# TorchIO-project/torchio

Hardware: NVIDIA H100
Metric: augmented voxels/sec on 256^3 fp32 Compose pipeline (higher is better)
Workload: dtype f32

## Files before the change

### include/tio_b200.h

```cpp
#ifndef TIO_B200_H
#define TIO_B200_H

#include <stddef.h>
#include <stdint.h>

#ifdef __cplusplus
extern "C" {
#endif

#define TIO_ABI_VERSION 2

enum tio_dtype {
  TIO_F32 = 0,
  TIO_U8 = 1,
  TIO_I8 = 2,
  TIO_I16 = 3,
  TIO_I32 = 4,
  TIO_I64 = 5,
  TIO_F16 = 6,
  TIO_BF16 = 7,
  TIO_F64 = 8
};

enum tio_interp { TIO_NEAREST = 0, TIO_LINEAR = 1, TIO_LABEL_PV = 2 };
#define TIO_EXACT_COORDS 0x100

#define TIO_FLAG_PASSTHROUGH 1u
#define TIO_FLAG_ELASTIC 2u

const char* tio_last_error(void);
int tio_abi_version(void);

size_t tio_resample_workspace_bytes(int B, int OI, int OJ, int OK);
int tio_resample(const void* src, void* dst, int dtype,
                 int B, int C, int I, int J, int K,
                 int OI, int OJ, int OK,
                 const float* mat, const float* cp, const uint8_t* flags,
                 int ni, int nj, int nk,
                 const float* spacing_in, const float* spacing_out,
                 int affine_first, int mode, const float* fill, int box_hint,
                 void* workspace, size_t workspace_bytes, void* stream);

int tio_onehot(const void* src, int dtype, int B, int64_t vox, const void* labels, int n,
               float* dst, void* stream);
int tio_label_argmax(const float* sampled, int B, int n, int64_t vox, const void* labels,
                     float pad_label, void* dst, int dtype, void* stream);

int tio_crop_patches(const void* src, void* dst, int elem_bytes, int C, int I, int J, int K,
                     int n, const int32_t* corners, int pi, int pj, int pk, void* stream);

int tio_remap(const void* src, void* dst, int elem_bytes, int B, int C, int I, int J, int K,
              int OI, int OJ, int OK, int off_i, int off_j, int off_k, int mode,
              const void* fill, const uint8_t* flip, void* stream);

int tio_permute(const void* src, void* dst, int elem_bytes, int B, int C, int I, int J, int K,
                int perm0, int perm1, int perm2, int flip_bits, void* stream);

int tio_upload(const void* host_pinned, void* dst_device, size_t bytes, void* stream);

int tio_min_sample0(const float* src, int C, int64_t n, float* fill, void* stream);

int tio_blur(const float* src, float* dst, float* scratch,
             int B, int C, int I, int J, int K,
             const float* taps, const int32_t* radius, int R, int axes_mask,
             const uint8_t* identity, void* stream);

size_t tio_mt19937_table_bytes(void);
int tio_mt19937_build_table(void* host_blob, size_t bytes);
size_t tio_randn_mt19937_workspace_bytes(uint64_t offset, uint64_t n);
int tio_randn_mt19937(uint64_t seed, uint64_t offset, uint64_t n, float* z,
                      const void* table, void* workspace, size_t workspace_bytes,
                      void* stream);

int tio_moments(const float* src, const uint8_t* mask, int64_t n, double* out3, void* stream);
size_t tio_quantiles_workspace_bytes(void);
int tio_quantiles(const float* src, const uint8_t* mask, int64_t n, const double* q_host, int m,
                  float* values, double* weights, double* count, void* workspace,
                  size_t workspace_bytes, void* stream);
int tio_rescale(const float* src, float* dst, int B, int64_t per_elem, float lo, float hi,
                const float* sub, const float* div, const float* mul, const float* add,
                const uint8_t* keep, int flags, void* stream);

size_t tio_quantiles_batched_workspace_bytes(int B, int m);
int tio_quantiles_batched(const void* src, int dtype, const uint8_t* mask, int B, int64_t per_elem,
                          const double* q_host, int m, float* values, double* weights, double* count,
                          uint8_t* has_nan, void* workspace, size_t workspace_bytes, void* stream);
int tio_histogram_tables(const float* values, const double* weights, const uint8_t* has_nan,
                         const float* landmarks, int B, int m, float* tables, void* stream);
int tio_histogram_map(const void* src, void* dst, int dtype, int B, int64_t per_elem,
                      const float* tables, int m, void* stream);

int tio_intensity_fused(const float* src, float* dst, float* scratch,
                        int B, int C, int I, int J, int K,
                        const float* coarse, int si, int sj, int sk,
                        const uint8_t* bias_identity, int bias_divide,
                        const float* taps, const int32_t* radius, int R, int axes_mask,
                        const float* mean, const float* std, const uint8_t* keep,
                        const float* z, const float* z2,
                        uint64_t philox_seed, int noise_mode, int rician,
                        const float* gamma, void* stream);

int tio_labels_to_image(const void* labels, int dtype, int C, int B, int64_t vox,
                        const int64_t* label_values, int n, const float* mean, const float* std,
                        const uint64_t* draw_offset, uint64_t seed, int grid_x, float* dst,
                        void* stream);

int tio_label_lut(const void* src, void* dst, int dtype, int64_t count, const void* keys,
                  const void* values, int n, int identity, void* stream);
int tio_label_contour(const void* src, int dtype, int volumes, int I, int J, int K, float* dst,
                      void* stream);
int tio_onehot_classes(const void* src, int dtype, int B, int C, int64_t vox, int num_classes,
                       float* dst, void* stream);
int tio_label_range(const void* src, int dtype, int B, int C, int64_t vox, int64_t* range,
                    void* stream);
int tio_channel_argmax(const void* src, int dtype, int B, int C, int64_t vox, float* dst,
                       void* stream);

int tio_interpolate(const void* src, void* dst, int dtype, int volumes, int I, int J, int K, int OI,
                    int OJ, int OK, const int32_t* idx, const float* lam, int linear, void* stream);
int tio_axis_resample(const void* src, void* dst, int dtype, int B, int C, int I, int J, int K,
                      const int32_t* axis, const int32_t* lo, const int32_t* hi, const float* w, int L,
                      int linear, void* stream);

int tio_clamp(const void* src, void* dst, int dtype, int dst_dtype, int64_t count, const void* lo,
              const void* hi, void* stream);
int tio_mask(const void* mask, int mask_dtype, int mask_channels, const void* keys, int n_keys,
             const void* src, int dtype, void* dst, int dst_dtype, int B, int C, int64_t vox,
             const void* outside, void* stream);
int tio_swap_patches(void* data, int elem_size, int B, int C, int I, int J, int K, int pi, int pj,
                     int pk, const int32_t* swaps, int lists, int steps, int32_t* swaps_device,
                     void* stage, void* stream);

int tio_components(const void* src, int dtype, int B, int I, int J, int K, int mode, const void* keys,
                   int n_keys, int64_t background, int has_background, int fully_connected,
                   uint32_t* parent, uint32_t* count, uint32_t* flags, void* stream);
int tio_component_roots(const void* src, int dtype, int B, int64_t vox, const uint32_t* parent,
                        void* values, uint32_t* n_values, void* stream);
int tio_keep_largest(void* data, int dtype, int B, int64_t vox, int mode, const void* keys,
                     int n_keys, int64_t background, int has_background, const uint32_t* parent,
                     const uint32_t* count, uint64_t* winner, const void* fill, void* stream);

size_t tio_spike_stats_workspace_bytes(int rows);
int tio_spike_stats(const void* src, int dtype, int B, int C, int64_t vox, const float* intensity,
                    double* sum, uint32_t* flags, void* workspace, size_t workspace_bytes,
                    void* stream);
int tio_spectrum_peak(const void* src, int dtype, int B, int C, int I, int J, int K,
                      const float* intensity, const uint32_t* flags, float* peak, void* workspace,
                      size_t workspace_bytes, void* stream);
int tio_spike(void* data, int dtype, int B, int C, int I, int J, int K, const int32_t* spikes, int S,
              const float* intensity, const double* sum, const uint32_t* flags, const float* peak,
              void* tables, size_t tables_bytes, void* stream);

int tio_ghosting(void* data, int dtype, int B, int C, int I, int J, int K, const float* table, int n_max,
                 const int32_t* axis, const uint8_t* active, int axes, uint32_t* flags, void* stream);

#ifdef __cplusplus
}
#endif
#endif
```

### torchio_b200/_native.py

```python

from __future__ import annotations

import ctypes
from ctypes import c_char_p, c_float, c_int, c_int64, c_size_t, c_uint64, c_void_p
from pathlib import Path

LIB_PATH = Path(__file__).resolve().parent / "csrc" / "libtio_b200.so"

_SIGNATURES = {
    "tio_abi_version": [],
    "tio_resample": [c_void_p, c_void_p, c_int] + [c_int] * 8
    + [c_void_p, c_void_p, c_void_p] + [c_int] * 3
    + [c_void_p, c_void_p, c_int, c_int, c_void_p, c_int, c_void_p, c_size_t, c_void_p],
    "tio_resample_workspace_bytes": [c_int, c_int, c_int, c_int],
    "tio_min_sample0": [c_void_p, c_int, c_int64, c_void_p, c_void_p],
    "tio_upload": [c_void_p, c_void_p, c_size_t, c_void_p],
    "tio_remap": [c_void_p, c_void_p, c_int] + [c_int] * 8 + [c_int] * 3 + [c_int, c_void_p, c_void_p, c_void_p],
    "tio_crop_patches": [c_void_p, c_void_p, c_int] + [c_int] * 5 + [c_void_p, c_int, c_int, c_int, c_void_p],
    "tio_blur": [c_void_p, c_void_p, c_void_p] + [c_int] * 5
    + [c_void_p, c_void_p, c_int, c_int, c_void_p, c_void_p],
    "tio_moments": [c_void_p, c_void_p, c_int64, c_void_p, c_void_p],
    "tio_quantiles_workspace_bytes": [],
    "tio_quantiles": [c_void_p, c_void_p, c_int64, c_void_p, c_int, c_void_p, c_void_p, c_void_p, c_void_p,
                      c_size_t, c_void_p],
    "tio_quantiles_batched_workspace_bytes": [c_int, c_int],
    "tio_quantiles_batched": [c_void_p, c_int, c_void_p, c_int, c_int64, c_void_p, c_int, c_void_p, c_void_p,
                              c_void_p, c_void_p, c_void_p, c_size_t, c_void_p],
    "tio_histogram_tables": [c_void_p, c_void_p, c_void_p, c_void_p, c_int, c_int, c_void_p, c_void_p],
    "tio_histogram_map": [c_void_p, c_void_p, c_int, c_int, c_int64, c_void_p, c_int, c_void_p],
    "tio_rescale": [c_void_p, c_void_p, c_int, c_int64, c_float, c_float, c_void_p, c_void_p, c_void_p, c_void_p,
                    c_void_p, c_int, c_void_p],
    "tio_onehot": [c_void_p, c_int, c_int, c_int64, c_void_p, c_int, c_void_p, c_void_p],
    "tio_label_argmax": [c_void_p, c_int, c_int, c_int64, c_void_p, c_float, c_void_p, c_int, c_void_p],
    "tio_mt19937_table_bytes": [],
    "tio_mt19937_build_table": [c_void_p, c_size_t],
    "tio_randn_mt19937_workspace_bytes": [c_uint64, c_uint64],
    "tio_randn_mt19937": [c_uint64, c_uint64, c_uint64, c_void_p, c_void_p, c_void_p, c_size_t,
                          c_void_p],
    "tio_intensity_fused": [c_void_p, c_void_p, c_void_p] + [c_int] * 5
    + [c_void_p, c_int, c_int, c_int, c_void_p, c_int]
    + [c_void_p, c_void_p, c_int, c_int]
    + [c_void_p] * 5 + [c_uint64, c_int, c_int, c_void_p, c_void_p],
    "tio_labels_to_image": [c_void_p, c_int, c_int, c_int, c_int64, c_void_p, c_int, c_void_p, c_void_p, c_void_p,
                            c_uint64, c_int, c_void_p, c_void_p],
    "tio_label_lut": [c_void_p, c_void_p, c_int, c_int64, c_void_p, c_void_p, c_int, c_int, c_void_p],
    "tio_label_contour": [c_void_p, c_int, c_int, c_int, c_int, c_int, c_void_p, c_void_p],
    "tio_onehot_classes": [c_void_p, c_int, c_int, c_int, c_int64, c_int, c_void_p, c_void_p],
    "tio_label_range": [c_void_p, c_int, c_int, c_int, c_int64, c_void_p, c_void_p],
    "tio_channel_argmax": [c_void_p, c_int, c_int, c_int, c_int64, c_void_p, c_void_p],
    "tio_interpolate": [c_void_p, c_void_p, c_int, c_int, c_int, c_int, c_int, c_int, c_int, c_int, c_void_p,
                        c_void_p, c_int, c_void_p],
    "tio_axis_resample": [c_void_p, c_void_p, c_int, c_int, c_int, c_int, c_int, c_int, c_void_p, c_void_p,
                          c_void_p, c_void_p, c_int, c_int, c_void_p],
    "tio_clamp": [c_void_p, c_void_p, c_int, c_int, c_int64, c_void_p, c_void_p, c_void_p],
    "tio_mask": [c_void_p, c_int, c_int, c_void_p, c_int, c_void_p, c_int, c_void_p, c_int, c_int, c_int, c_int64,
                 c_void_p, c_void_p],
    "tio_swap_patches": [c_void_p] + [c_int] * 9 + [c_void_p, c_int, c_int, c_void_p, c_void_p, c_void_p],
    "tio_components": [c_void_p] + [c_int] * 6 + [c_void_p, c_int, c_int64, c_int, c_int] + [c_void_p] * 4,
    "tio_component_roots": [c_void_p, c_int, c_int, c_int64] + [c_void_p] * 4,
    "tio_keep_largest": [c_void_p, c_int, c_int, c_int64, c_int, c_void_p, c_int, c_int64, c_int] + [c_void_p] * 5,
    "tio_permute": [c_void_p, c_void_p] + [c_int] * 10 + [c_void_p],
    "tio_spike_stats_workspace_bytes": [c_int],
    "tio_spike_stats": [c_void_p, c_int, c_int, c_int, c_int64] + [c_void_p] * 4 + [c_size_t, c_void_p],
    "tio_spectrum_peak": [c_void_p] + [c_int] * 6 + [c_void_p] * 4 + [c_size_t, c_void_p],
    "tio_spike": [c_void_p] + [c_int] * 6 + [c_void_p, c_int] + [c_void_p] * 5 + [c_size_t, c_void_p],
    "tio_ghosting": [c_void_p] + [c_int] * 6 + [c_void_p, c_int, c_void_p, c_void_p, c_int, c_void_p, c_void_p],
}

_lib = None


def lib() -> ctypes.CDLL:
    global _lib
    if _lib is None:
        if not LIB_PATH.exists():
            raise RuntimeError(
                f"torchio_b200: CUDA library not built ({LIB_PATH} is missing)."
                " Run `python -c 'import __graft_entry__ as g; g.build()'` at the"
                " repo root (needs nvcc). There is no CPU fallback."
            )
        handle = ctypes.CDLL(str(LIB_PATH))
        handle.tio_last_error.restype = c_char_p
        handle.tio_last_error.argtypes = []
        for name, argtypes in _SIGNATURES.items():
            fn = getattr(handle, name)
            fn.argtypes = argtypes
            fn.restype = c_size_t if name.endswith("_bytes") else c_int
        _lib = handle
    return _lib


def exported_symbols() -> list[str]:
    return ["tio_last_error", *_SIGNATURES]


def call(name: str, *args) -> None:
    handle = lib()
    rc = getattr(handle, name)(*args)
    if rc != 0:
        msg = handle.tio_last_error().decode(errors="replace")
        raise RuntimeError(f"{name} failed (code {rc}): {msg}")
```

### torchio_b200/csrc/build.py

```python

from __future__ import annotations

import os
import subprocess
import sys
from concurrent.futures import ThreadPoolExecutor
from pathlib import Path

HERE = Path(__file__).resolve().parent
ROOT = HERE.parent.parent
SOURCES = ["error.cu", "resample.cu", "resample_tile.cu", "resample_fast.cu", "upload.cu", "fused_intensity.cu",
           "mt19937_jump.cpp", "mt19937.cu", "patches.cu", "stats.cu", "labels.cu", "labels_to_image.cu",
           "label_maps.cu", "interpolate.cu", "clamp_mask_swap.cu", "components.cu", "permute.cu", "spike.cu",
           "ghosting.cu"]
HEADERS = [HERE / "common.cuh", HERE / "resample_common.cuh", HERE / "resample_tile.cuh", HERE / "tma.cuh",
           HERE / "mt19937_layout.h", HERE / "label_lookup.cuh", HERE / "image_dtype.cuh",
           HERE / "fft_lines.cuh",
           ROOT / "include" / "tio_b200.h",
           Path(__file__).resolve()]
OBJ = HERE / "_obj"
OUT = HERE / "libtio_b200.so"

ARCH = ["-gencode", "arch=compute_90a,code=sm_90a"]
NVCC_FLAGS = [
    *ARCH,
    "-O3", "-std=c++17", "-lineinfo",
    "-Xcompiler", "-fPIC",
    "-Xptxas", "-v",
]


def needs_build() -> bool:
    if not OUT.exists():
        return True
    newest = max(p.stat().st_mtime for p in [*(HERE / s for s in SOURCES), *HEADERS])
    return OUT.stat().st_mtime < newest


def _compile(source: str) -> tuple[str, int, str]:
    src = HERE / source
    obj = OBJ / (Path(source).stem + ".o")
    newest = max(p.stat().st_mtime for p in [src, *HEADERS])
    if obj.exists() and obj.stat().st_mtime >= newest:
        return source, 0, ""
    proc = subprocess.run(["nvcc", *NVCC_FLAGS, "-c", str(src), "-o", str(obj)],
                          capture_output=True, text=True)
    return source, proc.returncode, proc.stdout + proc.stderr


def build(force: bool = False, verbose: bool = False) -> Path:
    if not force and not needs_build():
        return OUT
    OBJ.mkdir(exist_ok=True)
    if force:
        for stale in OBJ.glob("*.o"):
            stale.unlink()
    with ThreadPoolExecutor(max_workers=min(len(SOURCES), os.cpu_count() or 1)) as pool:
        results = list(pool.map(_compile, SOURCES))
    log = "".join(f"==== {name}\n{text}" for name, _, text in results)
    failed = [name for name, code, _ in results if code != 0]
    if verbose or failed:
        sys.stderr.write(log)
    if failed:
        raise RuntimeError(f"nvcc failed for {failed}")
    objects = [str(OBJ / (Path(s).stem + ".o")) for s in SOURCES]
    proc = subprocess.run(["nvcc", *ARCH, "-shared", "-o", str(OUT),
                           *objects], capture_output=True, text=True)
    if proc.returncode != 0:
        sys.stderr.write(proc.stdout + proc.stderr)
        raise RuntimeError(f"nvcc link failed with exit code {proc.returncode}")
    previous = (HERE / "ptxas.log").read_text() if (HERE / "ptxas.log").exists() and not force else ""
    (HERE / "ptxas.log").write_text(log if all(t for _, _, t in results) else previous + log)
    return OUT


if __name__ == "__main__":
    path = build(force="--force" in sys.argv, verbose="--verbose" in sys.argv)
    print(path)
```

### torchio_b200/csrc/fused_intensity.cu

```cuda
#include "common.cuh"
#include "tma.cuh"

namespace tio {

__device__ __forceinline__ float rician(float x, float n1, float n2) {
  float s = __fadd_rn(x, n1);
  return sqrtf(__fadd_rn(__fmul_rn(s, s), __fmul_rn(n2, n2)));
}


__device__ __forceinline__ uint4 philox4x32_10(uint4 ctr, uint2 key) {
  const uint32_t M0 = 0xD2511F53u, M1 = 0xCD9E8D57u, W0 = 0x9E3779B9u, W1 = 0xBB67AE85u;
#pragma unroll
  for (int r = 0; r < 7; ++r) {
    uint32_t hi0 = __umulhi(M0, ctr.x), lo0 = M0 * ctr.x;
    uint32_t hi1 = __umulhi(M1, ctr.z), lo1 = M1 * ctr.z;
    ctr = make_uint4(hi1 ^ ctr.y ^ key.x, lo1, hi0 ^ ctr.w ^ key.y, lo0);
    key.x += W0;
    key.y += W1;
  }
  return ctr;
}

__device__ __forceinline__ void box_muller(uint32_t a, uint32_t b, float& n0, float& n1) {
  float u1 = ((float)(a >> 8) + 0.5f) * (1.0f / 16777216.0f);
  float u2 = ((float)(b >> 8)) * (1.0f / 16777216.0f);
  float rad;
  asm("sqrt.approx.ftz.f32 %0, %1;" : "=f"(rad) : "f"(-2.0f * __logf(u1)));
  float s, c;
  __sincosf(6.283185307179586f * u2, &s, &c);
  n0 = rad * c;
  n1 = rad * s;
}


__device__ __forceinline__ float abs_pow(float ax, float g) {
  float l, p;
  asm("lg2.approx.f32 %0, %1;" : "=f"(l) : "f"(ax));
  asm("ex2.approx.f32 %0, %1;" : "=f"(p) : "f"(__fmul_rn(g, l)));
  return p;
}

__device__ __forceinline__ float signed_pow(float x, float gam) {
  if (gam == 1.0f) return x;
  float ax = fabsf(x);
  float p = abs_pow(ax, gam);
  p = ax == 0.0f ? 0.0f : p;
  return x < 0.0f ? -p : p;
}

constexpr int A_TJ = 32;
constexpr int A_TK = 64;
constexpr int A_PLANES = 16;

struct BiasArgs {
  const float* coarse;
  const uint8_t* identity;
  int si, sj, sk;
  float sc_i, sc_j, sc_k;
  int divide;
};

struct BlurArgs {
  const float* taps;
  const int32_t* radius;
  int R;
};

struct NoiseArgs {
  const float* mean;
  const float* std;
  const uint8_t* keep;
  const float* z;
  const float* z2;
  uint64_t philox_seed;
  int mode;
  int rician;
};

template <int RMAX, bool HAS_EPI>
__global__ void __launch_bounds__(256)
jk_kernel(const float* __restrict__ src, float* __restrict__ dst, int B, int C, int I, int J,
          int K, BlurArgs bl, NoiseArgs nz, const float* __restrict__ gamma) {
  constexpr int ROWS = A_TJ + 2 * RMAX;
  constexpr int COLS = A_TK + 2 * RMAX;
  constexpr int PITCH = (COLS + 3) / 4 * 4 + 4;
  extern __shared__ __align__(16) float smem[];
  float* A = smem;
  float* Bm = A + ROWS * PITCH;
  float* tapk = Bm + ROWS * A_TK;
  float* tapj = tapk + (2 * RMAX + 1);

  const int tiles_i = (I + A_PLANES - 1) / A_PLANES;
  const int bc = blockIdx.z / tiles_i;
  const int i_begin = (blockIdx.z % tiles_i) * A_PLANES;
  const int i_end = min(i_begin + A_PLANES, I);
  const int b = bc / C;
  const int j0 = blockIdx.y * A_TJ, k0 = blockIdx.x * A_TK;
  const int tid = threadIdx.x;
  const int64_t n = (int64_t)I * J * K;
  const float* x = src + (int64_t)bc * n;
  float* y = dst + (int64_t)bc * n;

  const int R = bl.taps ? bl.R : 0;
  const int rj = bl.taps ? bl.radius[1 * B + b] : 0;
  const int rk = bl.taps ? bl.radius[2 * B + b] : 0;
  const bool noise_on = HAS_EPI && nz.mode != 0 && (!nz.keep || nz.keep[b]);
  const float mu = (HAS_EPI && nz.mode) ? nz.mean[b] : 0.0f, sd = (HAS_EPI && nz.mode) ? nz.std[b] : 0.0f;
  const float gam = (HAS_EPI && gamma) ? gamma[b] : 1.0f;

  if (tid < 2 * (2 * RMAX + 1)) {
    const bool is_k = tid < (2 * RMAX + 1);
    const int sft = is_k ? tid : tid - (2 * RMAX + 1);
    const int rr = is_k ? rk : rj;
    float v = 0.0f;
    if (bl.taps && rr > 0 && sft <= 2 * rr)
      v = bl.taps[((int64_t)(is_k ? 2 : 1) * B + b) * (2 * R + 1) + R - rr + sft];
    (is_k ? tapk : tapj)[sft] = v;
  }
  __syncthreads();

  float tk[2 * RMAX + 1], tj[2 * RMAX + 1];
#pragma unroll
  for (int t = 0; t < 2 * RMAX + 1; ++t) { tk[t] = tapk[t]; tj[t] = tapj[t]; }

  const int rows = A_TJ + 2 * rj, cols = A_TK + 2 * rk;
  const int lx = tid & 31, ly = tid >> 5;

  for (int i = i_begin; i < i_end; ++i) {
    const float* xp = x + (int64_t)i * J * K;
    for (int r = ly; r < rows; r += 8) {
      const int jj = min(max(j0 - rj + r, 0), J - 1);
      const float* xr = xp + (int64_t)jj * K;
      for (int c = lx; c < cols; c += 32) {
        const int kk = min(max(k0 - rk + c, 0), K - 1);
        A[r * PITCH + c] = __ldg(xr + kk);
      }
    }
    __syncthreads();
    {
      const int k4 = (tid & 15) * 4;
      for (int r = tid >> 4; r < rows; r += 16) {
        const float* row = A + r * PITCH + k4;
        float acc[4];
        if (rk == 0) {
#pragma unroll
          for (int o = 0; o < 4; ++o) acc[o] = row[o];
        } else {
          float win[4 + 2 * RMAX];
#pragma unroll
          for (int m = 0; m < (4 + 2 * RMAX) / 4; ++m) {
            if (4 * m < 4 + 2 * rk) {
              float4 q = *(const float4*)(row + 4 * m);
              win[4 * m] = q.x; win[4 * m + 1] = q.y; win[4 * m + 2] = q.z; win[4 * m + 3] = q.w;
            } else {
              win[4 * m] = win[4 * m + 1] = win[4 * m + 2] = win[4 * m + 3] = 0.0f;
            }
          }
#pragma unroll
          for (int o = 0; o < 4; ++o) acc[o] = 0.0f;
#pragma unroll
          for (int s = 0; s < 2 * RMAX + 1; ++s) {
            if (s <= 2 * rk) {
#pragma unroll
              for (int o = 0; o < 4; ++o) acc[o] = __fmaf_rn(tk[s], win[o + s], acc[o]);
            }
          }
        }
        *(float4*)(Bm + r * A_TK + k4) = make_float4(acc[0], acc[1], acc[2], acc[3]);
      }
    }
    __syncthreads();
    {
      const int kx = tid & 63, jy = (tid >> 6) * 8;
      const int k = k0 + kx;
      float acc[8];
      if (rj == 0) {
#pragma unroll
        for (int o = 0; o < 8; ++o) acc[o] = Bm[(jy + o) * A_TK + kx];
      } else {
        float win[8 + 2 * RMAX];
#pragma unroll
        for (int w = 0; w < 8 + 2 * RMAX; ++w)
          win[w] = (w < 8 + 2 * rj) ? Bm[(jy + w) * A_TK + kx] : 0.0f;
#pragma unroll
        for (int o = 0; o < 8; ++o) acc[o] = 0.0f;
#pragma unroll
        for (int s = 0; s < 2 * RMAX + 1; ++s) {
          if (s <= 2 * rj) {
#pragma unroll
            for (int o = 0; o < 8; ++o) acc[o] = __fmaf_rn(tj[s], win[o + s], acc[o]);
          }
        }
      }
      if (k < K) {
        const int64_t plane_off = (int64_t)i * J * K + k;
        if (HAS_EPI && noise_on) {
          float z1[8], z2[8];
          if (nz.mode == 1) {
#pragma unroll
            for (int o = 0; o < 8; ++o)
              if (j0 + jy + o < J) {
                const int64_t flat = (int64_t)bc * n + plane_off + (int64_t)(j0 + jy + o) * K;
                z1[o] = __ldcs(nz.z + flat);
                if (nz.rician) z2[o] = __ldcs(nz.z2 + flat);
              }
          } else {
            const uint2 key = make_uint2((uint32_t)nz.philox_seed, (uint32_t)(nz.philox_seed >> 32));
            const uint64_t gidx = (uint64_t)((int64_t)bc * n + plane_off + (int64_t)(j0 + jy) * K);
#pragma unroll
            for (int h = 0; h < 2; ++h) {
              uint4 rr = philox4x32_10(make_uint4((uint32_t)gidx, (uint32_t)(gidx >> 32), (uint32_t)h, 0x6a6bu), key);
              box_muller(rr.x, rr.y, z1[4 * h], z1[4 * h + 1]);
              box_muller(rr.z, rr.w, z1[4 * h + 2], z1[4 * h + 3]);
              if (nz.rician) {
                uint4 r2 = philox4x32_10(make_uint4((uint32_t)gidx, (uint32_t)(gidx >> 32), (uint32_t)(2 + h), 0x6a6bu), key);
                box_muller(r2.x, r2.y, z2[4 * h], z2[4 * h + 1]);
                box_muller(r2.z, r2.w, z2[4 * h + 2], z2[4 * h + 3]);
              }
            }
          }
#pragma unroll
          for (int o = 0; o < 8; ++o) {
            const float n1 = __fadd_rn(mu, __fmul_rn(sd, z1[o]));
            if (nz.rician) acc[o] = rician(acc[o], n1, __fadd_rn(mu, __fmul_rn(sd, z2[o])));
            else acc[o] = __fadd_rn(acc[o], n1);
          }
        }
        if (HAS_EPI && gamma) {
#pragma unroll
          for (int o = 0; o < 8; ++o) acc[o] = signed_pow(acc[o], gam);
        }
        float* yp = y + plane_off;
#pragma unroll
        for (int o = 0; o < 8; ++o)
          if (j0 + jy + o < J) yp[(int64_t)(j0 + jy + o) * K] = acc[o];
      }
    }
    __syncthreads();
  }
}

constexpr int F_R = 6;
constexpr int F_HK = 8;
constexpr int F_ROWS = A_TJ + 2 * F_R;
constexpr int F_COLS = A_TK + 2 * F_HK;
constexpr int F_ABUF = F_ROWS * F_COLS;
constexpr int F_BBUF = F_ROWS * A_TK;
constexpr size_t F_SMEM = (size_t)(2 * F_ABUF + 2 * F_BBUF + 32) * sizeof(float) + 2 * sizeof(uint64_t);

template <int RK>
__device__ __forceinline__ float4 kconv4(const float* __restrict__ row, const int k4, const float* tk) {
  if (RK == 0) return *(const float4*)(row + F_HK + k4);
  constexpr int M0 = RK <= 4 ? 1 : 0, M1 = RK <= 4 ? 4 : 5;
  float win[20];
#pragma unroll
  for (int m = M0; m < M1; ++m) {
    const float4 q = *(const float4*)(row + k4 + 4 * m);
    win[4 * m] = q.x; win[4 * m + 1] = q.y; win[4 * m + 2] = q.z; win[4 * m + 3] = q.w;
  }
  float acc[4] = {0.0f, 0.0f, 0.0f, 0.0f};
#pragma unroll
  for (int t = -RK; t <= RK; ++t)
#pragma unroll
    for (int o = 0; o < 4; ++o) acc[o] = __fmaf_rn(tk[F_R + t], win[F_HK + o + t], acc[o]);
  return make_float4(acc[0], acc[1], acc[2], acc[3]);
}

template <int RJ>
__device__ __forceinline__ void jconv8(const float* __restrict__ Bw, const int jy, const int kx,
                                       const float* tj, float* acc) {
  float win[8 + 2 * RJ];
#pragma unroll
  for (int w = 0; w < 8 + 2 * RJ; ++w) win[w] = Bw[(F_R - RJ + jy + w) * A_TK + kx];
  if (RJ == 0) {
#pragma unroll
    for (int o = 0; o < 8; ++o) acc[o] = win[o];
    return;
  }
#pragma unroll
  for (int o = 0; o < 8; ++o) acc[o] = 0.0f;
#pragma unroll
  for (int t = -RJ; t <= RJ; ++t)
#pragma unroll
    for (int o = 0; o < 8; ++o) acc[o] = __fmaf_rn(tj[F_R + t], win[o + t + RJ], acc[o]);
}

__device__ __forceinline__ float signed_pow_pos(float x, float g) {
  const float p = abs_pow(fabsf(x), g);
  return x < 0.0f ? -p : p;
}

template <bool HAS_EPI>
__global__ void __launch_bounds__(256, 3)
jk6_kernel(const __grid_constant__ CUtensorMap tmap, float* __restrict__ dst, int B, int C, int I,
           int J, int K, BlurArgs bl, NoiseArgs nz, const float* __restrict__ gamma) {
  extern __shared__ __align__(128) float smem[];
  float* Abuf = smem;
  float* Bbuf = smem + 2 * F_ABUF;
  float* taps_s = Bbuf + 2 * F_BBUF;
  uint64_t* bars = reinterpret_cast<uint64_t*>(taps_s + 32);

  const int tiles_i = (I + A_PLANES - 1) / A_PLANES;
  const int bc = blockIdx.z / tiles_i;
  const int i_begin = (blockIdx.z % tiles_i) * A_PLANES;
  const int i_end = min(i_begin + A_PLANES, I);
  const int b = bc / C;
  const int j0 = blockIdx.y * A_TJ, k0 = blockIdx.x * A_TK;
  const int tid = threadIdx.x;
  const int64_t n = (int64_t)I * J * K;

  auto issue = [&](int i, int s) {
    const uint32_t bar = smem_u32(bars + s);
    mbar_expect_tx(bar, (uint32_t)(F_ABUF * sizeof(float)));
    tma_load_3d(smem_u32(Abuf + s * F_ABUF), &tmap, k0 - F_HK, j0 - F_R, bc * I + i, bar);
  };
  if (tid == 0) {
    mbar_init(smem_u32(bars + 0), 1);
    mbar_init(smem_u32(bars + 1), 1);
    mbar_fence_init();
    issue(i_begin, 0);
  }

  const int R = bl.R;
  const int rj = bl.radius[1 * B + b], rk = bl.radius[2 * B + b];
  const bool noise_on = HAS_EPI && nz.mode != 0 && (!nz.keep || nz.keep[b]);
  const float mu = (HAS_EPI && nz.mode) ? nz.mean[b] : 0.0f, sd = (HAS_EPI && nz.mode) ? nz.std[b] : 0.0f;
  const float gam = (HAS_EPI && gamma) ? gamma[b] : 1.0f;
  const int gamma_mode = !(HAS_EPI && gamma) || gam == 1.0f ? 0 : (gam > 0.0f ? 1 : 2);

  if (tid < 2 * (2 * F_R + 1)) {
    const int axis = tid < (2 * F_R + 1) ? 2 : 1;
    const int s = tid < (2 * F_R + 1) ? tid : tid - (2 * F_R + 1);
    const int off = s - F_R, rr = axis == 2 ? rk : rj;
    float v = 0.0f;
    if (rr > 0 && off >= -rr && off <= rr) v = bl.taps[((int64_t)axis * B + b) * (2 * R + 1) + R + off];
    taps_s[(axis == 2 ? 0 : 13) + s] = v;
  }
  __syncthreads();
  float tk[2 * F_R + 1], tj[2 * F_R + 1];
#pragma unroll
  for (int t = 0; t < 2 * F_R + 1; ++t) { tk[t] = taps_s[t]; tj[t] = taps_s[13 + t]; }

  const int row_lo = F_R - rj, row_hi = F_R + A_TJ + rj;
  const int rsrc_lo = max(0, F_R - j0), rsrc_hi = min(F_ROWS - 1, J - 1 - j0 + F_R);
  const int clo = max(0, F_HK - k0), chi = min(F_COLS - 1, K - 1 - k0 + F_HK);
  const bool kfix = (clo > F_HK - rk) || (chi < F_HK + A_TK + rk - 1);

  const int k4 = (tid & 15) * 4;
  const int kx = tid & 63, jy = (tid >> 6) * 8;
  const int k = k0 + kx;
  const int valid = (k < K) ? min(8, J - (j0 + jy)) : 0;
  const int plane_off = (j0 + jy) * K + k;

  auto kpass = [&](int i) {
    const int it = i - i_begin, s = it & 1;
    mbar_wait(smem_u32(bars + s), (uint32_t)((it >> 1) & 1));
    float* A = Abuf + s * F_ABUF;
    float* Bw = Bbuf + s * F_BBUF;
#pragma unroll 1
    for (int r = row_lo + (tid >> 4); r < row_hi; r += 16) {
      float* row = A + min(max(r, rsrc_lo), rsrc_hi) * F_COLS;
      if (kfix) {
        const int c_lo = (F_HK - F_R) + (tid & 15);
        if (c_lo < clo) row[c_lo] = row[clo];
#pragma unroll 1
        for (int c = chi + 1 + (tid & 15); c < F_HK + A_TK + F_R; c += 16) row[c] = row[chi];
        __syncwarp();
      }
      float4 o4;
      switch (rk) {
        case 0: o4 = kconv4<0>(row, k4, tk); break;
        case 1: o4 = kconv4<1>(row, k4, tk); break;
        case 2: o4 = kconv4<2>(row, k4, tk); break;
        case 3: o4 = kconv4<3>(row, k4, tk); break;
        case 4: o4 = kconv4<4>(row, k4, tk); break;
        case 5: o4 = kconv4<5>(row, k4, tk); break;
        default: o4 = kconv4<6>(row, k4, tk); break;
      }
      *(float4*)(Bw + r * A_TK + k4) = o4;
    }
  };

  if (tid == 0 && i_begin + 1 < i_end) issue(i_begin + 1, 1);
  kpass(i_begin);
  __syncthreads();
  for (int i = i_begin; i < i_end; ++i) {
    const int it = i - i_begin, s = it & 1;
    if (tid == 0 && i + 2 < i_end) issue(i + 2, s);
    float* Bw = Bbuf + s * F_BBUF;
    float z1[8], z2[8];
    const int64_t flat0 = (int64_t)bc * n + (int64_t)i * J * K + plane_off;
    if (HAS_EPI && noise_on && nz.mode == 1) {
      const float* zp = nz.z + flat0;
      if (valid == 8) {
#pragma unroll
        for (int o = 0; o < 8; ++o, zp += K) z1[o] = __ldcs(zp);
      } else {
#pragma unroll
        for (int o = 0; o < 8; ++o, zp += K)
          if (o < valid) z1[o] = __ldcs(zp);
      }
      if (nz.rician) {
        const float* zq = nz.z2 + flat0;
#pragma unroll
        for (int o = 0; o < 8; ++o, zq += K)
          if (o < valid) z2[o] = __ldcs(zq);
      }
    }
    if (i + 1 < i_end) kpass(i + 1);
    float acc[8];
    switch (rj) {
      case 0: jconv8<0>(Bw, jy, kx, tj, acc); break;
      case 1: jconv8<1>(Bw, jy, kx, tj, acc); break;
      case 2: jconv8<2>(Bw, jy, kx, tj, acc); break;
      case 3: jconv8<3>(Bw, jy, kx, tj, acc); break;
      case 4: jconv8<4>(Bw, jy, kx, tj, acc); break;
      case 5: jconv8<5>(Bw, jy, kx, tj, acc); break;
      default: jconv8<6>(Bw, jy, kx, tj, acc); break;
    }
    if (valid > 0) {
      if (HAS_EPI && noise_on) {
        if (nz.mode == 2) {
          const uint2 key = make_uint2((uint32_t)nz.philox_seed, (uint32_t)(nz.philox_seed >> 32));
#pragma unroll
          for (int h = 0; h < 2; ++h) {
            const uint64_t gidx = (uint64_t)(flat0 + (int64_t)(4 * h) * K);
            uint4 rr = philox4x32_10(make_uint4((uint32_t)gidx, (uint32_t)(gidx >> 32), 0u, 0x6a6bu), key);
            box_muller(rr.x, rr.y, z1[4 * h], z1[4 * h + 1]);
            box_muller(rr.z, rr.w, z1[4 * h + 2], z1[4 * h + 3]);
            if (nz.rician) {
              uint4 r2 = philox4x32_10(make_uint4((uint32_t)gidx, (uint32_t)(gidx >> 32), 1u, 0x6a6bu), key);
              box_muller(r2.x, r2.y, z2[4 * h], z2[4 * h + 1]);
              box_muller(r2.z, r2.w, z2[4 * h + 2], z2[4 * h + 3]);
            }
          }
        }
        if (nz.rician) {
#pragma unroll
          for (int o = 0; o < 8; ++o)
            acc[o] = rician(acc[o], __fadd_rn(mu, __fmul_rn(sd, z1[o])), __fadd_rn(mu, __fmul_rn(sd, z2[o])));
        } else {
#pragma unroll
          for (int o = 0; o < 8; ++o) acc[o] = __fadd_rn(acc[o], __fadd_rn(mu, __fmul_rn(sd, z1[o])));
        }
      }
      if (gamma_mode == 1) {
#pragma unroll
        for (int o = 0; o < 8; ++o) acc[o] = signed_pow_pos(acc[o], gam);
      } else if (gamma_mode == 2) {
#pragma unroll
        for (int o = 0; o < 8; ++o) acc[o] = signed_pow(acc[o], gam);
      }
      float* yp = dst + flat0;
      if (valid == 8) {
#pragma unroll
        for (int o = 0; o < 8; ++o, yp += K) *yp = acc[o];
      } else {
#pragma unroll
        for (int o = 0; o < 8; ++o, yp += K)
          if (o < valid) *yp = acc[o];
      }
    }
    __syncthreads();
  }
}

template <int V, bool HAS_BIAS>
__global__ void __launch_bounds__(256)
march_kernel(const float* __restrict__ src, float* __restrict__ dst, int B, int C, int I, int J,
             int K, BlurArgs bl, BiasArgs bi, NoiseArgs nz, const float* __restrict__ gamma) {
  extern __shared__ __align__(16) float smem[];
  const int bc = blockIdx.z;
  const int b = bc / C;
  const int tid = threadIdx.y * blockDim.x + threadIdx.x;
  const int k = (blockIdx.x * blockDim.x + threadIdx.x) * V;
  const int j = blockIdx.y * blockDim.y + threadIdx.y;
  const int64_t n = (int64_t)I * J * K;
  const float* x = src + (int64_t)bc * n;
  float* y = dst + (int64_t)bc * n;

  const int r = bl.taps ? bl.radius[0 * B + b] : 0;
  const int R = bl.taps ? bl.R : 0;
  const int W = 2 * r + 1;
  float* tapi = smem;
  float* g = smem + ((2 * R + 1 + 3) / 4) * 4;
  const int ns = HAS_BIAS ? bi.si * bi.sj * bi.sk : 0;
  float* ring = g + ((ns + 3) / 4) * 4;
  const bool bias_on = HAS_BIAS && !(bi.identity && bi.identity[b]);
  if (r > 0)
    for (int t = tid; t < 2 * R + 1; t += 256) tapi[t] = bl.taps[((int64_t)0 * B + b) * (2 * R + 1) + t];
  if (bias_on) {
    const float* gs = bi.coarse + (int64_t)bc * ns;
    for (int t = tid; t < ns; t += 256) g[t] = gs[t];
  }
  __syncthreads();
  if (k >= K || j >= J) return;

  const bool noise_on = nz.mode != 0 && (!nz.keep || nz.keep[b]);
  const float mu = nz.mode ? nz.mean[b] : 0.0f, sd = nz.mode ? nz.std[b] : 0.0f;
  const float gam = gamma ? gamma[b] : 1.0f;

  LerpAxis lj, lk[V];
  int cur0 = -1, cur1 = -1;
  float r_lo[V], r_hi[V];
  if (bias_on) {
    lj = lerp_axis(bi.sc_j, bi.sj, j);
#pragma unroll
    for (int v = 0; v < V; ++v) lk[v] = lerp_axis(bi.sc_k, bi.sk, k + v);
  }

  auto load_plane = [&](int i, float* out) {
    const int64_t o = ((int64_t)i * J + j) * K + k;
    if (V == 4) {
      float4 t = *(const float4*)(x + o);
      out[0] = t.x; out[1] = t.y; out[2] = t.z; out[3] = t.w;
    } else {
      out[0] = x[o];
    }
    if (bias_on) {
      const LerpAxis li = lerp_axis(bi.sc_i, bi.si, i);
      if (li.i0 != cur0 || li.i1 != cur1) {
        const float* p0 = g + (li.i0 * bi.sj) * bi.sk;
        const float* p1 = g + (li.i1 * bi.sj) * bi.sk;
#pragma unroll
        for (int v = 0; v < V; ++v) {
          float a0 = lerp2(lk[v].l0, p0[lj.i0 * bi.sk + lk[v].i0], lk[v].l1, p0[lj.i0 * bi.sk + lk[v].i1]);
          float a1 = lerp2(lk[v].l0, p0[lj.i1 * bi.sk + lk[v].i0], lk[v].l1, p0[lj.i1 * bi.sk + lk[v].i1]);
          r_lo[v] = lerp2(lj.l0, a0, lj.l1, a1);
          float b0 = lerp2(lk[v].l0, p1[lj.i0 * bi.sk + lk[v].i0], lk[v].l1, p1[lj.i0 * bi.sk + lk[v].i1]);
          float b1 = lerp2(lk[v].l0, p1[lj.i1 * bi.sk + lk[v].i0], lk[v].l1, p1[lj.i1 * bi.sk + lk[v].i1]);
          r_hi[v] = lerp2(lj.l0, b0, lj.l1, b1);
        }
        cur0 = li.i0; cur1 = li.i1;
      }
#pragma unroll
      for (int v = 0; v < V; ++v) {
        float f = expf(lerp2(li.l0, r_lo[v], li.l1, r_hi[v]));
        out[v] = bi.divide ? __fdiv_rn(out[v], f) : __fmul_rn(out[v], f);
      }
    }
  };

  auto finish = [&](int i, float* v) {
    const int64_t o = ((int64_t)i * J + j) * K + k;
    if (noise_on) {
      const int64_t flat = (int64_t)bc * n + o;
      float z1[V], z2[V];
      if (nz.mode == 1) {
        if (V == 4) {
          float4 t = __ldcs((const float4*)(nz.z + flat));
          z1[0] = t.x; z1[1] = t.y; z1[2] = t.z; z1[3] = t.w;
          if (nz.rician) {
            float4 u = __ldcs((const float4*)(nz.z2 + flat));
            z2[0] = u.x; z2[1] = u.y; z2[2] = u.z; z2[3] = u.w;
          }
        } else {
          z1[0] = nz.z[flat];
          if (nz.rician) z2[0] = nz.z2[flat];
        }
      } else {
        const uint2 key = make_uint2((uint32_t)nz.philox_seed, (uint32_t)(nz.philox_seed >> 32));
        const uint64_t gidx = (uint64_t)(flat / V);
        uint4 rr = philox4x32_10(make_uint4((uint32_t)gidx, (uint32_t)(gidx >> 32), 0u, 0x5eedu), key);
        float nn[4];
        box_muller(rr.x, rr.y, nn[0], nn[1]);
        box_muller(rr.z, rr.w, nn[2], nn[3]);
#pragma unroll
        for (int q = 0; q < V; ++q) z1[q] = nn[q];
        if (nz.rician) {
          uint4 r2 = philox4x32_10(make_uint4((uint32_t)gidx, (uint32_t)(gidx >> 32), 1u, 0x5eedu), key);
          box_muller(r2.x, r2.y, nn[0], nn[1]);
          box_muller(r2.z, r2.w, nn[2], nn[3]);
#pragma unroll
          for (int q = 0; q < V; ++q) z2[q] = nn[q];
        }
      }
#pragma unroll
      for (int q = 0; q < V; ++q) {
        float n1 = __fadd_rn(mu, __fmul_rn(sd, z1[q]));
        if (nz.rician) v[q] = rician(v[q], n1, __fadd_rn(mu, __fmul_rn(sd, z2[q])));
        else v[q] = __fadd_rn(v[q], n1);
      }
    }
    if (gamma) {
#pragma unroll
      for (int q = 0; q < V; ++q) v[q] = signed_pow(v[q], gam);
    }
    if (V == 4) *(float4*)(y + o) = make_float4(v[0], v[1], v[2], v[3]);
    else y[o] = v[0];
  };

  if (r == 0) {
    for (int i = 0; i < I; ++i) {
      float v[V];
      load_plane(i, v);
      finish(i, v);
    }
    return;
  }

  float* mine = ring + tid * V;
  const int slot_stride = 256 * V;
  auto put = [&](int pos, const float* v) {
    int s = pos % W; if (s < 0) s += W;
    if (V == 4) *(float4*)(mine + s * slot_stride) = make_float4(v[0], v[1], v[2], v[3]);
    else mine[s * slot_stride] = v[0];
  };
  float first[V];
  load_plane(0, first);
  for (int p = -r; p <= 0; ++p) put(p, first);
  float last[V];
#pragma unroll
  for (int q = 0; q < V; ++q) last[q] = first[q];
  for (int p = 1; p < I + r; ++p) {
    if (p < I) load_plane(p, last);
    put(p, last);
    const int o = p - r;
    if (o < 0) continue;
    float acc[V];
#pragma unroll
    for (int q = 0; q < V; ++q) acc[q] = 0.0f;
    int s = (o - r) % W; if (s < 0) s += W;
    for (int t = 0; t < W; ++t) {
      const float tp = tapi[R - r + t];
      if (V == 4) {
        float4 w4 = *(const float4*)(mine + s * slot_stride);
        acc[0] = __fmaf_rn(tp, w4.x, acc[0]); acc[1] = __fmaf_rn(tp, w4.y, acc[1]);
        acc[2] = __fmaf_rn(tp, w4.z, acc[2]); acc[3] = __fmaf_rn(tp, w4.w, acc[3]);
      } else {
        acc[0] = __fmaf_rn(tp, mine[s * slot_stride], acc[0]);
      }
      if (++s == W) s = 0;
    }
    finish(o, acc);
  }
}

constexpr int M6_PF = 8;

template <bool HAS_BIAS, bool EPI>
__global__ void __launch_bounds__(256, EPI ? 1 : 2)
march6_kernel(const float* __restrict__ src, float* __restrict__ dst, int B, int C, int I, int J,
              int K, BlurArgs bl, BiasArgs bi, NoiseArgs nz, const float* __restrict__ gamma) {
  extern __shared__ __align__(16) float smem[];
  constexpr int W = 2 * F_R + 1;
  const int bc = blockIdx.z;
  const int b = bc / C;
  const int tid = threadIdx.y * blockDim.x + threadIdx.x;
  const int k = (blockIdx.x * blockDim.x + threadIdx.x) * 4;
  const int j = blockIdx.y * blockDim.y + threadIdx.y;
  const int64_t n = (int64_t)I * J * K;
  const float* x = src + (int64_t)bc * n;
  float* y = dst + (int64_t)bc * n;

  const int r = bl.taps ? bl.radius[0 * B + b] : 0;
  float* tapi = smem;
  float* g = smem + 16;
  const int ns = HAS_BIAS ? bi.si * bi.sj * bi.sk : 0;
  const bool bias_on = HAS_BIAS && !(bi.identity && bi.identity[b]);
  if (tid < W) {
    const int off = tid - F_R;
    tapi[tid] = (r > 0 && off >= -r && off <= r) ? bl.taps[((int64_t)0 * B + b) * (2 * bl.R + 1) + bl.R + off] : 0.0f;
  }
  if (bias_on) {
    const float* gs = bi.coarse + (int64_t)bc * ns;
    for (int t = tid; t < ns; t += 256) g[t] = gs[t];
  }
  __syncthreads();
  if (k >= K || j >= J) return;

  const bool noise_on = EPI && nz.mode != 0 && (!nz.keep || nz.keep[b]);
  const float mu = (EPI && nz.mode) ? nz.mean[b] : 0.0f, sd = (EPI && nz.mode) ? nz.std[b] : 0.0f;
  const float gam = (EPI && gamma) ? gamma[b] : 1.0f;
  const int gamma_mode = !(EPI && gamma) || gam == 1.0f ? 0 : (gam > 0.0f ? 1 : 2);

  LerpAxis lj, lk[4];
  int o00[4], o01[4], o10[4], o11[4];
  int cur0 = -1, cur1 = -1;
  float r_lo[4], r_hi[4];
  if (bias_on) {
    lj = lerp_axis(bi.sc_j, bi.sj, j);
#pragma unroll
    for (int v = 0; v < 4; ++v) {
      lk[v] = lerp_axis(bi.sc_k, bi.sk, k + v);
      o00[v] = lj.i0 * bi.sk + lk[v].i0; o01[v] = lj.i0 * bi.sk + lk[v].i1;
      o10[v] = lj.i1 * bi.sk + lk[v].i0; o11[v] = lj.i1 * bi.sk + lk[v].i1;
    }
  }
  const int col = j * K + k;
  const int plane = J * K;

  float4* fifo = reinterpret_cast<float4*>(g + ((ns + 3) / 4) * 4) + tid;
  auto fifo_issue = [&](int pl) {
    if (pl < I) {
      const uint32_t sa = (uint32_t)__cvta_generic_to_shared(fifo + (pl & (M6_PF - 1)) * 256);
      asm volatile("cp.async.cg.shared.global [%0], [%1], 16;" ::"r"(sa), "l"(x + (int64_t)pl * plane + col) : "memory");
    }
    asm volatile("cp.async.commit_group;" ::: "memory");
  };
#pragma unroll
  for (int pl = 0; pl < M6_PF - 1; ++pl) fifo_issue(pl);

  auto load_plane = [&](int i, float* out) {
    fifo_issue(i + M6_PF - 1);
    asm volatile("cp.async.wait_group %0;" ::"n"(M6_PF - 1) : "memory");
    const float4 t = fifo[(i & (M6_PF - 1)) * 256];
    out[0] = t.x; out[1] = t.y; out[2] = t.z; out[3] = t.w;
    if (bias_on) {
      const LerpAxis li = lerp_axis(bi.sc_i, bi.si, i);
      if (li.i0 != cur0 || li.i1 != cur1) {
        const float* p0 = g + (li.i0 * bi.sj) * bi.sk;
        const float* p1 = g + (li.i1 * bi.sj) * bi.sk;
#pragma unroll
        for (int v = 0; v < 4; ++v) {
          const float a0 = lerp2(lk[v].l0, p0[o00[v]], lk[v].l1, p0[o01[v]]);
          const float a1 = lerp2(lk[v].l0, p0[o10[v]], lk[v].l1, p0[o11[v]]);
          r_lo[v] = lerp2(lj.l0, a0, lj.l1, a1);
          const float b0 = lerp2(lk[v].l0, p1[o00[v]], lk[v].l1, p1[o01[v]]);
          const float b1 = lerp2(lk[v].l0, p1[o10[v]], lk[v].l1, p1[o11[v]]);
          r_hi[v] = lerp2(lj.l0, b0, lj.l1, b1);
        }
        cur0 = li.i0; cur1 = li.i1;
      }
#pragma unroll
      for (int v = 0; v < 4; ++v) {
        const float f = expf(lerp2(li.l0, r_lo[v], li.l1, r_hi[v]));
        out[v] = bi.divide ? __fdiv_rn(out[v], f) : __fmul_rn(out[v], f);
      }
    }
  };

  auto finish = [&](int i, float* v) {
    const int64_t o = (int64_t)i * plane + col;
    if (EPI) {
      if (noise_on) {
        const int64_t flat = (int64_t)bc * n + o;
        float z1[4], z2[4];
        if (nz.mode == 1) {
          const float4 t = __ldcs((const float4*)(nz.z + flat));
          z1[0] = t.x; z1[1] = t.y; z1[2] = t.z; z1[3] = t.w;
          if (nz.rician) {
            const float4 u = __ldcs((const float4*)(nz.z2 + flat));
            z2[0] = u.x; z2[1] = u.y; z2[2] = u.z; z2[3] = u.w;
          }
        } else {
          const uint2 key = make_uint2((uint32_t)nz.philox_seed, (uint32_t)(nz.philox_seed >> 32));
          const uint64_t gidx = (uint64_t)(flat / 4);
          uint4 rr = philox4x32_10(make_uint4((uint32_t)gidx, (uint32_t)(gidx >> 32), 0u, 0x5eedu), key);
          box_muller(rr.x, rr.y, z1[0], z1[1]);
          box_muller(rr.z, rr.w, z1[2], z1[3]);
          if (nz.rician) {
            uint4 r2 = philox4x32_10(make_uint4((uint32_t)gidx, (uint32_t)(gidx >> 32), 1u, 0x5eedu), key);
            box_muller(r2.x, r2.y, z2[0], z2[1]);
            box_muller(r2.z, r2.w, z2[2], z2[3]);
          }
        }
#pragma unroll
        for (int q = 0; q < 4; ++q) {
          const float n1 = __fadd_rn(mu, __fmul_rn(sd, z1[q]));
          if (nz.rician) v[q] = rician(v[q], n1, __fadd_rn(mu, __fmul_rn(sd, z2[q])));
          else v[q] = __fadd_rn(v[q], n1);
        }
      }
      if (gamma_mode == 1) {
#pragma unroll
        for (int q = 0; q < 4; ++q) v[q] = signed_pow_pos(v[q], gam);
      } else if (gamma_mode == 2) {
#pragma unroll
        for (int q = 0; q < 4; ++q) v[q] = signed_pow(v[q], gam);
      }
    }
    *(float4*)(y + o) = make_float4(v[0], v[1], v[2], v[3]);
  };

  if (r == 0) {
    for (int i = 0; i < I; ++i) {
      float v[4];
      load_plane(i, v);
      finish(i, v);
    }
    return;
  }

  float tp[W];
#pragma unroll
  for (int t = 0; t < W; ++t) tp[t] = tapi[t];
  float ring[W][4];
  {
    float first[4];
    load_plane(0, first);
#pragma unroll
    for (int sl = 0; sl < W; ++sl)
#pragma unroll
      for (int q = 0; q < 4; ++q) ring[sl][q] = first[q];
  }
  for (int base = 0; base < I + F_R; base += W) {
#pragma unroll
    for (int ph = 0; ph < W; ++ph) {
      const int p = base + ph;
      if (p >= I + F_R) break;
      if (p > 0 && p < I) load_plane(p, ring[ph]);
      else if (p >= I) {
#pragma unroll
        for (int q = 0; q < 4; ++q) ring[ph][q] = ring[(ph + W - 1) % W][q];
      }
      const int o = p - F_R;
      if (o >= 0) {
        float acc[4] = {0.0f, 0.0f, 0.0f, 0.0f};
#pragma unroll
        for (int t = 0; t < W; ++t) {
          if (t < F_R - r || t > F_R + r) continue;
          const int sl = (ph + 1 + t) % W;
#pragma unroll
          for (int q = 0; q < 4; ++q) acc[q] = __fmaf_rn(tp[t], ring[sl][q], acc[q]);
        }
        finish(o, acc);
      }
    }
  }
}

constexpr int WIDE_RMAX = 6143;

template <bool HAS_EPI>
__global__ void __launch_bounds__(256)
axis_kernel(const float* __restrict__ src, float* __restrict__ dst, int B, int C, int I, int J,
            int K, int axis, BlurArgs bl, NoiseArgs nz, const float* __restrict__ gamma) {
  extern __shared__ float taps_s[];
  const int bc = blockIdx.y;
  const int b = bc / C;
  const int tid = threadIdx.x;
  const int64_t n = (int64_t)I * J * K;
  const int r = bl.radius[axis * B + b];
  for (int t = tid; t < 2 * r + 1; t += 256)
    taps_s[t] = bl.taps[((int64_t)axis * B + b) * (2 * bl.R + 1) + bl.R - r + t];
  __syncthreads();
  const int64_t e = (int64_t)blockIdx.x * 256 + tid;
  if (e >= n) return;
  const int L = axis == 0 ? I : (axis == 1 ? J : K);
  const int64_t s = axis == 0 ? (int64_t)J * K : (axis == 1 ? K : 1);
  const int pos = (int)((e / s) % L);
  const float* x = src + (int64_t)bc * n + (e - pos * s);
  float acc;
  if (r == 0) {
    acc = x[pos * s];
  } else {
    acc = 0.0f;
    for (int t = 0; t <= 2 * r; ++t) {
      const int q = min(max(pos - r + t, 0), L - 1);
      acc = __fmaf_rn(taps_s[t], __ldg(x + q * s), acc);
    }
  }
  const int64_t flat = (int64_t)bc * n + e;
  if (HAS_EPI) {
    if (nz.mode != 0 && (!nz.keep || nz.keep[b])) {
      const float mu = nz.mean[b], sd = nz.std[b];
      float z1, z2 = 0.0f;
      if (nz.mode == 1) {
        z1 = nz.z[flat];
        if (nz.rician) z2 = nz.z2[flat];
      } else {
        const uint2 key = make_uint2((uint32_t)nz.philox_seed, (uint32_t)(nz.philox_seed >> 32));
        float unused;
        uint4 rr = philox4x32_10(make_uint4((uint32_t)flat, (uint32_t)((uint64_t)flat >> 32), 0u, 0x77ffu), key);
        box_muller(rr.x, rr.y, z1, unused);
        if (nz.rician) box_muller(rr.z, rr.w, z2, unused);
      }
      const float n1 = __fadd_rn(mu, __fmul_rn(sd, z1));
      acc = nz.rician ? rician(acc, n1, __fadd_rn(mu, __fmul_rn(sd, z2))) : __fadd_rn(acc, n1);
    }
    if (gamma) acc = signed_pow(acc, gamma[b]);
  }
  dst[flat] = acc;
}

static inline bool aligned16f(const void* p) { return ((uintptr_t)p & 15) == 0; }

static float up_scale(int n_in, int n_out) {
  if (n_in == n_out) return 1.0f;
  return n_out > 1 ? (float)(n_in - 1) / (float)(n_out - 1) : 0.0f;
}

template <int RMAX>
static int launch_jk(const float* src, float* dst, int B, int C, int I, int J, int K,
                     const BlurArgs& bl, const NoiseArgs& nz, const float* gamma, cudaStream_t st) {
  constexpr int ROWS = A_TJ + 2 * RMAX, COLS = A_TK + 2 * RMAX, PITCH = (COLS + 3) / 4 * 4 + 4;
  const size_t smem = (size_t)(ROWS * PITCH + ROWS * A_TK + 2 * (2 * RMAX + 1)) * sizeof(float);
  const int tiles_i = (I + A_PLANES - 1) / A_PLANES;
  dim3 grid((K + A_TK - 1) / A_TK, (J + A_TJ - 1) / A_TJ, B * C * tiles_i);
  if (nz.mode != 0 || gamma) {
    if (smem > 48 * 1024)
      cudaFuncSetAttribute(jk_kernel<RMAX, true>, cudaFuncAttributeMaxDynamicSharedMemorySize, (int)smem);
    jk_kernel<RMAX, true><<<grid, 256, smem, st>>>(src, dst, B, C, I, J, K, bl, nz, gamma);
  } else {
    if (smem > 48 * 1024)
      cudaFuncSetAttribute(jk_kernel<RMAX, false>, cudaFuncAttributeMaxDynamicSharedMemorySize, (int)smem);
    jk_kernel<RMAX, false><<<grid, 256, smem, st>>>(src, dst, B, C, I, J, K, bl, nz, gamma);
  }
  return 0;
}

static int launch_march(const float* cur, float* out, int B, int C, int I, int J, int K,
                        const BiasArgs& bi, const BlurArgs& ib, const NoiseArgs& nz1,
                        const float* gamma1, cudaStream_t st, const char* who) {
  {
    const bool vec = (K % 4 == 0) && aligned16f(cur) && aligned16f(out) &&
                     (nz1.mode != 1 || (aligned16f(nz1.z) && (!nz1.z2 || aligned16f(nz1.z2))));
    const int V = vec ? 4 : 1;
    dim3 block(64, 4);
    dim3 grid((K + 64 * V - 1) / (64 * V), (J + 3) / 4, B * C);
    TIO_CHECK_ARG(grid.y <= 65535, "%s: J too large", who);
    const int R = ib.taps ? ib.R : 0;
    const int ns = bi.coarse ? bi.si * bi.sj * bi.sk : 0;
    const size_t smem = ((size_t)((2 * R + 1 + 3) / 4 * 4) + (size_t)((ns + 3) / 4 * 4) +
                         (ib.taps ? (size_t)(2 * R + 1) * 256 * V : 0)) * sizeof(float);
#define TIO_LAUNCH_MARCH(VV, BB)                                                              \
  do {                                                                                        \
    if (smem > 48 * 1024)                                                                     \
      cudaFuncSetAttribute(march_kernel<VV, BB>, cudaFuncAttributeMaxDynamicSharedMemorySize, \
                           (int)smem);                                                        \
    march_kernel<VV, BB><<<grid, block, smem, st>>>(cur, out, B, C, I, J, K, ib, bi, nz1, gamma1); \
  } while (0)
    if (vec && R <= F_R) {
      const size_t smem6 = (size_t)(16 + (ns + 3) / 4 * 4) * sizeof(float) + (size_t)M6_PF * 256 * 16;
#define TIO_LAUNCH_MARCH6(BB, EE)                                                              \
  do {                                                                                         \
    if (smem6 > 48 * 1024)                                                                     \
      cudaFuncSetAttribute(march6_kernel<BB, EE>, cudaFuncAttributeMaxDynamicSharedMemorySize, \
                           (int)smem6);                                                        \
    march6_kernel<BB, EE><<<grid, block, smem6, st>>>(cur, out, B, C, I, J, K, ib, bi, nz1, gamma1); \
  } while (0)
      const bool epi = nz1.mode != 0 || gamma1 != nullptr;
      if (bi.coarse) { if (epi) TIO_LAUNCH_MARCH6(true, true); else TIO_LAUNCH_MARCH6(true, false); }
      else { if (epi) TIO_LAUNCH_MARCH6(false, true); else TIO_LAUNCH_MARCH6(false, false); }
#undef TIO_LAUNCH_MARCH6
    } else if (vec) { if (bi.coarse) TIO_LAUNCH_MARCH(4, true); else TIO_LAUNCH_MARCH(4, false); }
    else { if (bi.coarse) TIO_LAUNCH_MARCH(1, true); else TIO_LAUNCH_MARCH(1, false); }
#undef TIO_LAUNCH_MARCH
  }
  return 0;
}

static int wide_impl(const float* src, float* dst, float* scratch, int B, int C, int I, int J,
                     int K, const BiasArgs& bi, const BlurArgs& bl, int axes_mask,
                     const NoiseArgs& nz, const float* gamma, cudaStream_t st, const char* who) {
  TIO_CHECK_ARG(bl.R <= WIDE_RMAX, "%s: blur radius R=%d > %d unsupported", who, bl.R, WIDE_RMAX);
  int axes[3], na = 0;
  for (int a : {0, 2, 1})
    if (axes_mask & (1 << a)) axes[na++] = a;
  const int steps = na + (bi.coarse ? 1 : 0);
  TIO_CHECK_ARG(src != dst && (steps < 2 || (scratch && scratch != src && scratch != dst)),
                "%s: blur radius R=%d > 16 needs src != dst and a scratch buffer", who, bl.R);
  const int64_t n = (int64_t)I * J * K;
  TIO_CHECK_ARG((n + 255) / 256 <= 0x7fffffff, "%s: volume too large", who);
  const float* cur = src;
  int left = steps;
  auto next_out = [&]() { return (--left % 2 == 0) ? dst : scratch; };
  if (bi.coarse) {
    BlurArgs none = bl;
    none.taps = nullptr;
    float* out = next_out();
    if (launch_march(cur, out, B, C, I, J, K, bi, none, NoiseArgs{}, nullptr, st, who)) return 1;
    cur = out;
  }
  const size_t smem = (size_t)(2 * bl.R + 1) * sizeof(float);
  dim3 grid((unsigned)((n + 255) / 256), B * C);
  for (int s = 0; s < na; ++s) {
    float* out = next_out();
    if (s == na - 1 && (nz.mode != 0 || gamma))
      axis_kernel<true><<<grid, 256, smem, st>>>(cur, out, B, C, I, J, K, axes[s], bl, nz, gamma);
    else
      axis_kernel<false><<<grid, 256, smem, st>>>(cur, out, B, C, I, J, K, axes[s], bl, nz, gamma);
    cur = out;
  }
  TIO_CHECK_LAUNCH();
  return 0;
}

static int fused_impl(const float* src, float* dst, float* scratch, int B, int C, int I, int J,
                      int K, BiasArgs bi, BlurArgs bl, int axes_mask, NoiseArgs nz,
                      const float* gamma, cudaStream_t st, const char* who) {
  TIO_CHECK_ARG(src && dst, "%s: null src/dst", who);
  TIO_CHECK_ARG(B > 0 && C > 0 && I > 0 && J > 0 && K > 0, "%s: bad shape", who);
  TIO_CHECK_ARG((int64_t)B * C <= 65535, "%s: B*C must be <= 65535", who);
  if (!bl.taps) axes_mask = 0;
  TIO_CHECK_ARG(!bl.taps || (bl.radius && bl.R >= 0), "%s: blur radius table missing or R=%d < 0", who, bl.R);
  if (bi.coarse) {
    bi.sc_i = up_scale(bi.si, I); bi.sc_j = up_scale(bi.sj, J); bi.sc_k = up_scale(bi.sk, K);
    TIO_CHECK_ARG((size_t)bi.si * bi.sj * bi.sk * 4 <= 64 * 1024, "%s: coarse bias grid too large", who);
  }
  if (axes_mask != 0 && bl.R > 16)
    return wide_impl(src, dst, scratch, B, C, I, J, K, bi, bl, axes_mask, nz, gamma, st, who);
  const bool need_jk = (axes_mask & 6) != 0;
  TIO_CHECK_ARG(!need_jk || (scratch && src != dst && scratch != src && scratch != dst),
                "%s: blur along J/K needs a scratch buffer and src != dst", who);
  TIO_CHECK_ARG(!((axes_mask & 1) && src == dst && !need_jk), "%s: blur along I needs src != dst", who);
  const bool need_i = (axes_mask & 1) != 0;
  const bool need_march = !need_jk || need_i || bi.coarse != nullptr;
  const float* cur = src;
  if (need_jk) {
    const int64_t tiles = (int64_t)B * C * ((I + A_PLANES - 1) / A_PLANES);
    TIO_CHECK_ARG(tiles <= 65535, "%s: batch too large for the blur grid", who);
  }
  if (need_march) {
    BlurArgs ib = bl;
    if (!need_i) ib.taps = nullptr;
    float* out = need_jk ? scratch : dst;
    if (launch_march(cur, out, B, C, I, J, K, bi, ib, need_jk ? NoiseArgs{} : nz,
                     need_jk ? nullptr : gamma, st, who))
      return 1;
    cur = out;
  }
  if (need_jk) {
    const bool tma_ok = bl.R <= F_R && (K % 4 == 0) && aligned16f(cur) && (int64_t)B * C * I < (1ll << 31);
    EncodeTiledFn encode = tma_ok ? encode_tiled_fn() : nullptr;
    CUtensorMap tm;
    bool have_map = false;
    if (encode) {
      const cuuint64_t gdim[3] = {(cuuint64_t)K, (cuuint64_t)J, (cuuint64_t)B * C * I};
      const cuuint64_t gstride[2] = {(cuuint64_t)K * 4, (cuuint64_t)J * K * 4};
      const cuuint32_t bdim[3] = {(cuuint32_t)F_COLS, (cuuint32_t)F_ROWS, 1};
      const cuuint32_t estr[3] = {1, 1, 1};
      have_map = encode(&tm, CU_TENSOR_MAP_DATA_TYPE_FLOAT32, 3, const_cast<float*>(cur), gdim, gstride,
                        bdim, estr, CU_TENSOR_MAP_INTERLEAVE_NONE, CU_TENSOR_MAP_SWIZZLE_NONE,
                        CU_TENSOR_MAP_L2_PROMOTION_L2_128B, CU_TENSOR_MAP_FLOAT_OOB_FILL_NONE) == CUDA_SUCCESS;
    }
    if (have_map) {
      const int tiles_i = (I + A_PLANES - 1) / A_PLANES;
      dim3 grid((K + A_TK - 1) / A_TK, (J + A_TJ - 1) / A_TJ, B * C * tiles_i);
      if (nz.mode != 0 || gamma) {
        cudaFuncSetAttribute(jk6_kernel<true>, cudaFuncAttributeMaxDynamicSharedMemorySize, (int)F_SMEM);
        jk6_kernel<true><<<grid, 256, F_SMEM, st>>>(tm, dst, B, C, I, J, K, bl, nz, gamma);
      } else {
        cudaFuncSetAttribute(jk6_kernel<false>, cudaFuncAttributeMaxDynamicSharedMemorySize, (int)F_SMEM);
        jk6_kernel<false><<<grid, 256, F_SMEM, st>>>(tm, dst, B, C, I, J, K, bl, nz, gamma);
      }
    } else if (bl.R <= F_R) {
      launch_jk<6>(cur, dst, B, C, I, J, K, bl, nz, gamma, st);
    } else {
      launch_jk<16>(cur, dst, B, C, I, J, K, bl, nz, gamma, st);
    }
  }
  TIO_CHECK_LAUNCH();
  return 0;
}

}

using namespace tio;

extern "C" int tio_blur(const float* src, float* dst, float* scratch, int B, int C, int I, int J,
                        int K, const float* taps, const int32_t* radius, int R, int axes_mask,
                        const uint8_t* identity, void* stream) {
  (void)identity;
  TIO_CHECK_ARG(taps && radius, "tio_blur: null taps/radius");
  TIO_CHECK_ARG(src != dst, "tio_blur: src and dst must not alias");
  BiasArgs bi{};
  BlurArgs bl{taps, radius, R};
  NoiseArgs nz{};
  return fused_impl(src, dst, scratch, B, C, I, J, K, bi, bl, axes_mask & 7, nz, nullptr,
                    (cudaStream_t)stream, "tio_blur");
}

extern "C" int tio_intensity_fused(const float* src, float* dst, float* scratch, int B, int C,
                                   int I, int J, int K, const float* coarse, int si, int sj,
                                   int sk, const uint8_t* bias_identity, int bias_divide,
                                   const float* taps, const int32_t* radius, int R,
                                   int axes_mask, const float* mean, const float* std,
                                   const uint8_t* keep, const float* z, const float* z2,
                                   uint64_t philox_seed, int noise_mode, int rician_flag,
                                   const float* gamma, void* stream) {
  BiasArgs bi{};
  bi.coarse = coarse; bi.identity = bias_identity; bi.si = si; bi.sj = sj; bi.sk = sk;
  bi.divide = bias_divide;
  BlurArgs bl{taps, radius, R};
  NoiseArgs nz{};
  nz.mode = noise_mode;
  TIO_CHECK_ARG(noise_mode >= 0 && noise_mode <= 2, "tio_intensity_fused: bad noise_mode");
  if (noise_mode) {
    TIO_CHECK_ARG(mean && std, "tio_intensity_fused: noise needs mean/std");
    TIO_CHECK_ARG(noise_mode != 1 || (z && (!rician_flag || z2)), "tio_intensity_fused: normals missing");
    nz.mean = mean; nz.std = std; nz.keep = keep; nz.z = z; nz.z2 = z2;
    nz.philox_seed = philox_seed; nz.rician = rician_flag;
  }
  return fused_impl(src, dst, scratch, B, C, I, J, K, bi, bl, taps ? (axes_mask & 7) : 0, nz,
                    gamma, (cudaStream_t)stream, "tio_intensity_fused");
}
```

### torchio_b200/csrc/mt19937.cu

```cuda
#include "common.cuh"
#include "mt19937_layout.h"

namespace tio {

constexpr int MT_N = 624, MT_M = 397, MT_DEG = 19937;
constexpr int MT_SEQ = MT_DEG + MT_N;
constexpr int MT_OFFS = (MT_SEQ + 7) / 4 * 4;

__device__ __forceinline__ uint32_t mt_twist(uint32_t a, uint32_t b, uint32_t c) {
  const uint32_t y = (a & 0x80000000u) | (b & 0x7fffffffu);
  return c ^ (y >> 1) ^ ((y & 1u) ? 0x9908b0dfu : 0u);
}

__device__ __forceinline__ uint32_t mt_temper(uint32_t y) {
  y ^= y >> 11;
  y ^= (y << 7) & 0x9d2c5680u;
  y ^= (y << 15) & 0xefc60000u;
  y ^= y >> 18;
  return y;
}

__global__ void mt_seed_kernel(uint32_t seed, uint32_t* __restrict__ states) {
  if (threadIdx.x == 0) {
    uint32_t v = seed;
    states[0] = v;
    for (int j = 1; j < MT_N; ++j) {
      v = 1812433253u * (v ^ (v >> 30)) + (uint32_t)j;
      states[j] = v;
    }
  }
}

struct MtJob { int src, dst, slot; };

__global__ void __launch_bounds__(640)
mt_jump_kernel(uint32_t* __restrict__ states, const uint16_t* __restrict__ polys, int stride,
               int first, int S2, int fine, int parts) {
  extern __shared__ __align__(16) uint32_t seq[];
  uint32_t* offs = seq + MT_OFFS;
  const int job_idx = (int)blockIdx.x / parts, part = (int)blockIdx.x % parts;
  MtJob job;
  if (fine) {
    const int q = first + job_idx, r = q % S2;
    if (r == 0) return;
    job = MtJob{q - r, q, r - 1};
  } else {
    const int m = first + job_idx;
    job = MtJob{0, m * S2, (S2 - 1) + (m - 1)};
  }
  const int tid = threadIdx.x;
  const uint32_t* src = states + (size_t)job.src * MT_N;
  for (int t = tid; t < MT_N; t += blockDim.x) seq[t] = src[t];
  __syncthreads();
  for (int base = 0; base + MT_N < MT_SEQ; base += MT_N - MT_M) {
    const int k = base + tid;
    if (tid < MT_N - MT_M && k + MT_N < MT_SEQ)
      seq[k + MT_N] = mt_twist(seq[k], seq[k + 1], seq[k + MT_M]);
    __syncthreads();
  }
  const uint16_t* p = polys + (size_t)job.slot * stride;
  const uint32_t count = p[0] | ((uint32_t)p[1] << 16);
  const uint32_t t_begin = (uint32_t)((uint64_t)count * part / parts);
  const uint32_t t_end = (uint32_t)((uint64_t)count * (part + 1) / parts);
  const char* mine = reinterpret_cast<const char*>(seq + (tid < MT_N ? tid : 0));
  uint32_t acc = 0;
  for (uint32_t c0 = t_begin; c0 < t_end; c0 += 2048) {
    const uint32_t chunk = min(2048u, t_end - c0);
    for (uint32_t t = tid; t < chunk; t += blockDim.x) offs[t] = (uint32_t)p[2 + c0 + t] << 2;
    __syncthreads();
    if (tid < MT_N) {
      const uint4* o4 = reinterpret_cast<const uint4*>(offs);
      const uint32_t quads = chunk >> 2;
#pragma unroll 4
      for (uint32_t t = 0; t < quads; ++t) {
        const uint4 o = o4[t];
        acc ^= *reinterpret_cast<const uint32_t*>(mine + o.x) ^ *reinterpret_cast<const uint32_t*>(mine + o.y);
        acc ^= *reinterpret_cast<const uint32_t*>(mine + o.z) ^ *reinterpret_cast<const uint32_t*>(mine + o.w);
      }
      for (uint32_t t = quads << 2; t < chunk; ++t) acc ^= *reinterpret_cast<const uint32_t*>(mine + offs[t]);
    }
    __syncthreads();
  }
  if (tid < MT_N) {
    uint32_t* dst = states + (size_t)job.dst * MT_N + tid;
    if (parts == 1) *dst = acc;
    else atomicXor(dst, acc);
  }
}

__device__ __forceinline__ void sincos_0_2pi(float theta, float& sn, float& cs) {
  const float t = __fmaf_rn(theta, 0.6366197723675814f, 12582912.0f);
  const int j = __float_as_int(t);
  const float jf = __fsub_rn(t, 12582912.0f);
  float r = __fmaf_rn(jf, -1.5707962512969971f, theta);
  r = __fmaf_rn(jf, -7.549789415861596e-08f, r);
  const float r2 = __fmul_rn(r, r);
  float ps = __fmaf_rn(r2, -1.9515295891e-4f, 8.3321608736e-3f);
  ps = __fmaf_rn(ps, r2, -1.6666654611e-1f);
  const float s = __fmaf_rn(__fmul_rn(ps, r2), r, r);
  float pc = __fmaf_rn(r2, 2.443315711809948e-5f, -1.388731625493765e-3f);
  pc = __fmaf_rn(pc, r2, 4.166664568298827e-2f);
  const float c = __fmaf_rn(__fmul_rn(pc, r2), r2, __fmaf_rn(r2, -0.5f, 1.0f));
  const bool swap = j & 1;
  const float a = swap ? c : s, b = swap ? s : c;
  sn = (j & 2) ? -a : a;
  cs = ((j + 1) & 2) ? -b : b;
}

__device__ __forceinline__ void mt_box_muller(uint32_t a, uint32_t b, float& zc, float& zs) {
  const float u1 = (float)(mt_temper(a) & 0xffffffu) * (1.0f / 16777216.0f);
  const float u2 = (float)(mt_temper(b) & 0xffffffu) * (1.0f / 16777216.0f);
  float radius;
  asm("sqrt.approx.ftz.f32 %0, %1;" : "=f"(radius) : "f"(-2.0f * logf(1.0f - u1)));
  const float theta = (float)(6.283185307179586 * (double)u2);
  float sn, cs;
  sincos_0_2pi(theta, sn, cs);
  zc = radius * cs;
  zs = radius * sn;
}

template <int ID, int COUNT>
__device__ __forceinline__ void mt_bar_sync() {
  asm volatile("bar.sync %0, %1;" ::"n"(ID), "n"(COUNT) : "memory");
}
template <int ID, int COUNT>
__device__ __forceinline__ void mt_bar_arrive() {
  asm volatile("bar.arrive %0, %1;" ::"n"(ID), "n"(COUNT) : "memory");
}

constexpr int MT_ROUND = 4;
constexpr int MT_RING = 2 * MT_ROUND;
constexpr int MT_ITEMS = MT_ROUND * MT_N / 8;
constexpr int MT_PRODUCERS = 256;
constexpr int MT_CONSUMERS = (MT_ITEMS + 31) / 32 * 32;
constexpr int MT_THREADS = MT_PRODUCERS + MT_CONSUMERS;
constexpr int MT_BAR_PROD = 1, MT_BAR_FULL = 2, MT_BAR_EMPTY = 4;

__global__ void __launch_bounds__(MT_THREADS, 2)
mt_normal_kernel(const uint32_t* __restrict__ states, int q_first, unsigned long long L,
                 unsigned long long offset, unsigned long long n, float* __restrict__ z) {
  __shared__ __align__(16) uint32_t ring[MT_RING * MT_N];
  const int tid = threadIdx.x;
  const int q = q_first + blockIdx.x;
  const unsigned long long seg_begin = (unsigned long long)q * L;
  const unsigned long long lo = max(seg_begin, offset);
  const unsigned long long hi = min(seg_begin + L, offset + n);
  if (lo >= hi) return;
  const int lo_rel = (int)(lo - seg_begin), hi_rel = (int)(hi - seg_begin);
  const int rounds = ((hi_rel + MT_N - 1) / MT_N + MT_ROUND - 1) / MT_ROUND;
  if (tid < MT_PRODUCERS) {
    constexpr int W = MT_N - MT_M;
    const uint32_t* w = states + (size_t)q * MT_N;
    uint32_t* start = ring + (MT_RING - 1) * MT_N;
    for (int t = tid; t < MT_N; t += MT_PRODUCERS) start[t] = w[t];
    mt_bar_sync<MT_BAR_PROD, MT_PRODUCERS>();
    for (int r = 0; r < rounds; ++r) {
      if (r >= 2) {
        if (r & 1) mt_bar_sync<MT_BAR_EMPTY + 1, MT_THREADS>();
        else mt_bar_sync<MT_BAR_EMPTY, MT_THREADS>();
      }
      for (int i = 0; i < MT_ROUND; ++i) {
        const int b = r * MT_ROUND + i;
        const uint32_t* cur = ring + ((b + MT_RING - 1) % MT_RING) * MT_N;
        uint32_t* nxt = ring + (b % MT_RING) * MT_N;
        if (tid < W) nxt[tid] = mt_twist(cur[tid], cur[tid + 1], cur[tid + MT_M]);
        mt_bar_sync<MT_BAR_PROD, MT_PRODUCERS>();
        if (tid < W) nxt[W + tid] = mt_twist(cur[W + tid], cur[W + tid + 1], nxt[tid]);
        mt_bar_sync<MT_BAR_PROD, MT_PRODUCERS>();
        if (tid < MT_N - 2 * W) {
          const int k = 2 * W + tid;
          const uint32_t c = (k + 1 < MT_N) ? cur[k + 1] : nxt[0];
          nxt[k] = mt_twist(cur[k], c, nxt[k - W]);
        }
        mt_bar_sync<MT_BAR_PROD, MT_PRODUCERS>();
      }
      if (r & 1) mt_bar_arrive<MT_BAR_FULL + 1, MT_THREADS>();
      else mt_bar_arrive<MT_BAR_FULL, MT_THREADS>();
    }
  } else {
    const int c = tid - MT_PRODUCERS;
    const int blk = c / (MT_N / 8), item = c % (MT_N / 8);
    const int word = 16 * (item >> 1) + 4 * (item & 1);
    const long long seg_to_z = (long long)seg_begin - (long long)offset;
    const bool vec = ((reinterpret_cast<uintptr_t>(z) & 15) == 0);
    for (int r = 0; r < rounds; ++r) {
      if (r & 1) mt_bar_sync<MT_BAR_FULL + 1, MT_THREADS>();
      else mt_bar_sync<MT_BAR_FULL, MT_THREADS>();
      const int b = r * MT_ROUND + blk;
      const int group = b * MT_N + (word & ~15);
      if (c < MT_ITEMS && group >= lo_rel && group < hi_rel) {
        const uint32_t* x = ring + (b % MT_RING) * MT_N + word;
        const uint4 a = *reinterpret_cast<const uint4*>(x);
        const uint4 s = *reinterpret_cast<const uint4*>(x + 8);
        float4 zc, zs;
        mt_box_muller(a.x, s.x, zc.x, zs.x);
        mt_box_muller(a.y, s.y, zc.y, zs.y);
        mt_box_muller(a.z, s.z, zc.z, zs.z);
        mt_box_muller(a.w, s.w, zc.w, zs.w);
        float* zp = z + (seg_to_z + b * MT_N + word);
        if (vec) {
          *reinterpret_cast<float4*>(zp) = zc;
          *reinterpret_cast<float4*>(zp + 8) = zs;
        } else {
          zp[0] = zc.x; zp[1] = zc.y; zp[2] = zc.z; zp[3] = zc.w;
          zp[8] = zs.x; zp[9] = zs.y; zp[10] = zs.z; zp[11] = zs.w;
        }
      }
      if (r + 2 < rounds) {
        if (r & 1) mt_bar_arrive<MT_BAR_EMPTY + 1, MT_THREADS>();
        else mt_bar_arrive<MT_BAR_EMPTY, MT_THREADS>();
      }
    }
  }
}

}

using namespace tio;

constexpr uint64_t MT_L = 1ull << tio_mt::kLog2L;

extern "C" size_t tio_randn_mt19937_workspace_bytes(uint64_t offset, uint64_t n) {
  const uint64_t q_hi = (offset + n + MT_L - 1) / MT_L;
  return (size_t)(q_hi + tio_mt::kS1) * MT_N * 4;
}

extern "C" int tio_randn_mt19937(uint64_t seed, uint64_t offset, uint64_t n, float* z,
                                 const void* table, void* workspace, size_t workspace_bytes,
                                 void* stream) {
  TIO_CHECK_ARG(z && table && workspace, "tio_randn_mt19937: null pointer");
  TIO_CHECK_ARG(n >= 16 && (n % 16) == 0 && (offset % 16) == 0,
                "tio_randn_mt19937: n and offset must be multiples of 16 (n >= 16)");
  const int S2 = tio_mt::kS2, S1 = tio_mt::kS1, stride = tio_mt::kStride;
  const uint64_t q_lo = offset / MT_L, q_hi = (offset + n + MT_L - 1) / MT_L;
  TIO_CHECK_ARG(q_hi <= (uint64_t)S1 * S2, "tio_randn_mt19937: stream position beyond %d segments", S1 * S2);
  TIO_CHECK_ARG(workspace_bytes >= tio_randn_mt19937_workspace_bytes(offset, n),
                "tio_randn_mt19937: workspace too small");
  cudaStream_t st = (cudaStream_t)stream;
  uint32_t* states = (uint32_t*)workspace;
  const uint16_t* polys = (const uint16_t*)((const char*)table + tio_mt::kHeaderBytes);
  mt_seed_kernel<<<1, 32, 0, st>>>((uint32_t)seed, states);
  const size_t jump_smem = (size_t)(MT_OFFS + 2048) * 4;
  cudaFuncSetAttribute(mt_jump_kernel, cudaFuncAttributeMaxDynamicSharedMemorySize, (int)jump_smem);
  const int m_lo = (int)(q_lo / S2), m_hi = (int)((q_hi - 1) / S2);
  const int m_first = m_lo > 1 ? m_lo : 1;
  if (m_hi >= m_first) {
    constexpr int kCoarseParts = 8;
    const size_t pitch = (size_t)S2 * MT_N * 4;
    cudaMemset2DAsync(states + (size_t)m_first * S2 * MT_N, pitch, 0, MT_N * 4, m_hi - m_first + 1, st);
    mt_jump_kernel<<<(m_hi - m_first + 1) * kCoarseParts, 640, jump_smem, st>>>(states, polys, stride, m_first,
                                                                             S2, 0, kCoarseParts);
  }
  mt_jump_kernel<<<(unsigned)(q_hi - q_lo), 640, jump_smem, st>>>(states, polys, stride, (int)q_lo, S2, 1, 1);
  mt_normal_kernel<<<(unsigned)(q_hi - q_lo), MT_THREADS, 0, st>>>(states, (int)q_lo, MT_L, offset, n, z);
  TIO_CHECK_LAUNCH();
  return 0;
}
```

### torchio_b200/ops.py

```python

from __future__ import annotations

import os
import threading

import numpy as np
import torch
from torch import Tensor

from . import _native, tables

DTYPE_CODES = {
    torch.float32: 0, torch.uint8: 1, torch.int8: 2,
    torch.int16: 3, torch.int32: 4, torch.int64: 5,
}
NEAREST, LINEAR, LABEL_PV = 0, 1, 2
FLAG_PASSTHROUGH, FLAG_ELASTIC = 1, 2

_counter = threading.local()


def launches() -> int:
    return getattr(_counter, "n", 0)


def _count(n: int) -> None:
    _counter.n = getattr(_counter, "n", 0) + n


def _stream(t: Tensor) -> int:
    return torch.cuda.current_stream(t.device).cuda_stream


def _ptr(t: Tensor | None):
    return None if t is None else t.data_ptr()


def _require_cuda(t: Tensor, name: str) -> None:
    if not t.is_cuda:
        raise RuntimeError(
            f"torchio_b200.ops.{name}: expected a CUDA tensor (got {t.device});"
            " the kernels have no CPU fallback"
        )
    if t.requires_grad:
        raise NotImplementedError(
            f"torchio_b200.ops.{name}: kernels are forward-only; detach() the input"
        )


class _StagingRing:

    SLOTS = 64
    SLOT_BYTES = 1 << 20

    def __init__(self) -> None:
        self.buffers = [torch.empty(self.SLOT_BYTES, dtype=torch.uint8, pin_memory=True)
                        for _ in range(self.SLOTS)]
        self.events: list = [None] * self.SLOTS
        self.index = 0
        self.lock = threading.Lock()

    def take(self):
        with self.lock:
            i = self.index
            self.index = (i + 1) % self.SLOTS
            pending, self.events[i] = self.events[i], None
        if pending is not None:
            pending.synchronize()
        return i, self.buffers[i]

    def release(self, i: int, device: torch.device) -> None:
        ev = torch.cuda.Event()
        ev.record(torch.cuda.current_stream(device))
        with self.lock:
            self.events[i] = ev


_ring: _StagingRing | None = None
_init_lock = threading.Lock()


def upload(device: torch.device, *arrays):
    global _ring
    specs, offset = [], 0
    for a in arrays:
        if a is None:
            specs.append(None)
            continue
        t = torch.as_tensor(a)
        t = t.contiguous()
        nbytes = t.numel() * t.element_size()
        specs.append((t, offset, nbytes))
        offset += (nbytes + 15) // 16 * 16
    if offset == 0:
        return [None] * len(arrays)
    slot = None
    if torch.cuda.is_available() and offset <= _StagingRing.SLOT_BYTES:
        if _ring is None:
            with _init_lock:
                if _ring is None:
                    _ring = _StagingRing()
        slot, stage = _ring.take()
        stage = stage[:offset]
    else:
        stage = torch.empty(offset, dtype=torch.uint8, pin_memory=torch.cuda.is_available())
    stage_np = stage.numpy()
    for s in specs:
        if s is None:
            continue
        t, off, nbytes = s
        stage_np[off:off + nbytes] = t.reshape(-1).numpy().view(np.uint8)
    if slot is not None:
        dev = torch.empty(offset, dtype=torch.uint8, device=device)
        _native.call("tio_upload", stage.data_ptr(), dev.data_ptr(), offset,
                     torch.cuda.current_stream(dev.device).cuda_stream)
        _count(1)
        _ring.release(slot, torch.device(device))
    else:
        dev = stage.to(device, non_blocking=True)
    out = []
    for s in specs:
        if s is None:
            out.append(None)
            continue
        t, off, nbytes = s
        out.append(dev[off:off + nbytes].view(t.dtype).reshape(t.shape))
    return out


EXACT_COORDS = 0x100
_exact_default = os.environ.get("TIO_B200_EXACT_COORDS", "0") not in ("", "0")


def set_exact_coords(enabled: bool) -> bool:
    global _exact_default
    previous, _exact_default = _exact_default, bool(enabled)
    return previous


def exact_coords_default() -> bool:
    return _exact_default


def resample(
    src: Tensor, mat: Tensor, cp: Tensor | None, flags: Tensor | None,
    spacing_in, spacing_out, *, affine_first: bool, mode: int,
    fill: Tensor | None, out_shape=None, box_hint: int = 0, exact_coords: bool | None = None,
) -> Tensor:
    _require_cuda(src, "resample")
    if src.dtype not in DTYPE_CODES:
        raise TypeError(f"resample: unsupported dtype {src.dtype}")
    src = src.contiguous()
    b, c, i, j, k = src.shape
    oi, oj, ok = (i, j, k) if out_shape is None else out_shape
    dst = torch.empty((b, c, oi, oj, ok), dtype=src.dtype, device=src.device)
    ni = nj = nk = 0
    if cp is not None:
        ni, nj, nk = cp.shape[1:4]
    sp_in = np.asarray(spacing_in, dtype=np.float32)
    sp_out = np.asarray(spacing_out, dtype=np.float32)
    workspace, ws_bytes = None, 0
    tiled = (src.dtype == torch.float32 and mode == LINEAR) or (
        mode in (NEAREST, LABEL_PV) and src.dtype in (torch.uint8, torch.int16, torch.int32))
    if box_hint >= 0 and tiled:
        ws_bytes = _native.lib().tio_resample_workspace_bytes(b, oi, oj, ok)
        workspace = torch.empty(ws_bytes, dtype=torch.uint8, device=src.device)
    with torch.cuda.device(src.device):
        _native.call(
            "tio_resample", _ptr(src), _ptr(dst), DTYPE_CODES[src.dtype],
            b, c, i, j, k, oi, oj, ok, _ptr(mat), _ptr(cp), _ptr(flags), ni, nj, nk,
            sp_in.ctypes.data, sp_out.ctypes.data, int(bool(affine_first)),
            int(mode) | (EXACT_COORDS if (_exact_default if exact_coords is None else exact_coords) else 0),
            _ptr(fill), int(box_hint), _ptr(workspace), ws_bytes, _stream(src),
        )
    _count(2 if workspace is not None else 1)
    return dst


def _label_table(labels: Tensor, dtype: torch.dtype) -> Tensor:
    return labels.to(torch.float32 if dtype == torch.float32 else torch.int64).contiguous()


def onehot(src: Tensor, labels: Tensor) -> Tensor:
    _require_cuda(src, "onehot")
    if src.dtype not in DTYPE_CODES:
        raise TypeError(f"onehot: unsupported dtype {src.dtype}")
    src = src.contiguous()
    b, n = src.shape[0], int(labels.numel())
    vox = src[0].numel()
    table = _label_table(labels, src.dtype)
    dst = torch.empty((b, n, *src.shape[2:]), dtype=torch.float32, device=src.device)
    with torch.cuda.device(src.device):
        _native.call("tio_onehot", _ptr(src), DTYPE_CODES[src.dtype], b, vox, _ptr(table), n, _ptr(dst),
                     _stream(src))
    _count(1)
    return dst


def label_argmax(sampled: Tensor, labels: Tensor, pad_label: float, dtype: torch.dtype) -> Tensor:
    _require_cuda(sampled, "label_argmax")
    if dtype not in DTYPE_CODES:
        raise TypeError(f"label_argmax: unsupported dtype {dtype}")
    sampled = sampled.contiguous()
    b, n = sampled.shape[:2]
    vox = sampled[0, 0].numel()
    table = _label_table(labels, dtype)
    dst = torch.empty((b, 1, *sampled.shape[2:]), dtype=dtype, device=sampled.device)
    with torch.cuda.device(sampled.device):
        _native.call("tio_label_argmax", _ptr(sampled), b, n, vox, _ptr(table), float(pad_label), _ptr(dst),
                     DTYPE_CODES[dtype], _stream(sampled))
    _count(1)
    return dst


def min_sample0(src: Tensor) -> Tensor:
    _require_cuda(src, "min_sample0")
    src = src.contiguous()
    c = src.shape[1]
    n = src[0, 0].numel()
    fill = torch.empty(c, dtype=torch.float32, device=src.device)
    with torch.cuda.device(src.device):
        _native.call("tio_min_sample0", _ptr(src), c, n, _ptr(fill), _stream(src))
    _count(2)
    return fill


def crop_patches(volume: Tensor, corners, size, out: Tensor | None = None) -> Tensor:
    _require_cuda(volume, "crop_patches")
    if volume.ndim != 4:
        raise ValueError(f"crop_patches expects a (C, I, J, K) volume, got {tuple(volume.shape)}")
    volume = volume.contiguous()
    corners = np.ascontiguousarray(np.asarray(corners, dtype=np.int32).reshape(-1, 3))
    n = corners.shape[0]
    c, i, j, k = (int(v) for v in volume.shape)
    pi, pj, pk = (int(v) for v in size)
    if n == 0:
        return volume.new_empty((0, c, pi, pj, pk))
    if corners.min() < 0 or np.any(corners + np.asarray([pi, pj, pk]) > np.asarray([i, j, k])):
        raise ValueError("crop_patches: a patch extends beyond the volume")
    (corners_d,) = upload(volume.device, corners)
    if out is None:
        dst = torch.empty((n, c, pi, pj, pk), dtype=volume.dtype, device=volume.device)
    else:
        dst = out
        if (tuple(dst.shape) != (n, c, pi, pj, pk) or dst.dtype != volume.dtype or dst.device != volume.device
                or not dst.is_contiguous()):
            raise ValueError("crop_patches: `out` must be a contiguous (n, C, *size) block of the volume's dtype/device")
    with torch.cuda.device(volume.device):
        _native.call(
            "tio_crop_patches", _ptr(volume), _ptr(dst), volume.element_size(), c, i, j, k, n,
            _ptr(corners_d), pi, pj, pk, _stream(volume),
        )
    _count(1)
    return dst


PAD_MODES = {"constant": 0, "replicate": 1, "reflect": 2, "circular": 3}


def remap(src: Tensor, out_shape, offsets, *, mode: str = "constant", fill=0, flip: Tensor | None = None,
          out: Tensor | None = None) -> Tensor:
    _require_cuda(src, "remap")
    if src.ndim != 5:
        raise ValueError(f"remap expects (B, C, I, J, K), got {tuple(src.shape)}")
    src = src.contiguous()
    b, c, i, j, k = (int(v) for v in src.shape)
    oi, oj, ok = (int(v) for v in out_shape)
    if out is None:
        dst = torch.empty((b, c, oi, oj, ok), dtype=src.dtype, device=src.device)
    else:
        dst = out
        if (tuple(dst.shape) != (b, c, oi, oj, ok) or dst.dtype != src.dtype or dst.device != src.device
                or not dst.is_contiguous()):
            raise ValueError("remap: `out` must be a contiguous (B, C, *out_shape) block of the source's dtype/device")
    fill_host = torch.tensor([fill]).to(src.dtype)
    with torch.cuda.device(src.device):
        _native.call(
            "tio_remap", _ptr(src), _ptr(dst), src.element_size(), b, c, i, j, k, oi, oj, ok,
            int(offsets[0]), int(offsets[1]), int(offsets[2]), PAD_MODES[mode],
            fill_host.data_ptr(), _ptr(flip), _stream(src),
        )
    _count(1)
    return dst


def permute(src: Tensor, perm, flip_bits: int = 0) -> Tensor:
    _require_cuda(src, "permute")
    if src.ndim != 5:
        raise ValueError(f"permute expects (B, C, I, J, K), got {tuple(src.shape)}")
    perm = tuple(int(p) for p in perm)
    if sorted(perm) != [0, 1, 2]:
        raise ValueError(f"permute: {perm} is not a permutation of (0, 1, 2)")
    flip_bits = int(flip_bits)
    if perm == (0, 1, 2):
        if flip_bits == 0:
            return src
        (flags,) = upload(src.device, np.full(src.shape[0], flip_bits, dtype=np.uint8))
        return remap(src, src.shape[2:], (0, 0, 0), flip=flags)
    src = src.contiguous()
    b, c, i, j, k = (int(v) for v in src.shape)
    n = (i, j, k)
    dst = torch.empty((b, c, *(n[p] for p in perm)), dtype=src.dtype, device=src.device)
    with torch.cuda.device(src.device):
        _native.call("tio_permute", _ptr(src), _ptr(dst), src.element_size(), b, c, i, j, k, *perm, flip_bits,
                     _stream(src))
    _count(1)
    return dst


def blur(src: Tensor, taps: Tensor, radius: Tensor, big_r: int, axes_mask: int,
         identity: Tensor | None) -> Tensor:
    _require_cuda(src, "blur")
    src = src.contiguous()
    b, c, i, j, k = src.shape
    dst = torch.empty_like(src)
    scratch = torch.empty_like(src) if (axes_mask & 6) or big_r > WIDE_R else None
    with torch.cuda.device(src.device):
        _native.call(
            "tio_blur", _ptr(src), _ptr(dst), _ptr(scratch), b, c, i, j, k, _ptr(taps),
            _ptr(radius), int(big_r), int(axes_mask), _ptr(identity), _stream(src),
        )
    _count(_fused_launches(axes_mask, False, big_r))
    return dst


WIDE_R = 16


def _fused_launches(axes_mask: int, has_bias: bool, big_r: int = 0) -> int:
    if axes_mask & 7 and big_r > WIDE_R:
        return bin(axes_mask & 7).count("1") + int(has_bias)
    jk = bool(axes_mask & 6)
    march = (not jk) or bool(axes_mask & 1) or has_bias
    return int(jk) + int(march)


def moments(values: Tensor, mask: Tensor | None = None) -> tuple[float, float, float]:
    _require_cuda(values, "moments")
    values = values.contiguous()
    m8 = None if mask is None else mask.expand_as(values).contiguous().to(torch.uint8)
    out = torch.empty(3, dtype=torch.float64, device=values.device)
    with torch.cuda.device(values.device):
        _native.call("tio_moments", _ptr(values), _ptr(m8), values.numel(), _ptr(out), _stream(values))
    _count(1)
    s, ss, n = out.tolist()
    return s, ss, n


def quantile_neighbours(values: Tensor, qs, mask: Tensor | None = None):
    _require_cuda(values, "quantile_neighbours")
    values = values.contiguous()
    m8 = None if mask is None else mask.expand_as(values).contiguous().to(torch.uint8)
    qs = np.ascontiguousarray(np.asarray(qs, dtype=np.float64).reshape(-1))
    m = int(qs.shape[0])
    dev = values.device
    vals = torch.empty(2 * m, dtype=torch.float32, device=dev)
    out = torch.empty(m + 1, dtype=torch.float64, device=dev)
    ws_bytes = _native.lib().tio_quantiles_workspace_bytes()
    ws = torch.empty(ws_bytes, dtype=torch.uint8, device=dev)
    with torch.cuda.device(dev):
        _native.call("tio_quantiles", _ptr(values), _ptr(m8), values.numel(), qs.ctypes.data, m, _ptr(vals),
                     _ptr(out), out[m:].data_ptr(), _ptr(ws), ws_bytes, _stream(values))
    _count(7)
    host = out.tolist()
    return vals.tolist(), host[:m], int(host[m])


def quantiles_batched(values: Tensor, qs, mask: Tensor | None = None):
    _require_cuda(values, "quantiles_batched")
    if values.dtype not in RESOLUTION_DTYPE_CODES:
        raise TypeError(f"quantiles_batched: unsupported dtype {values.dtype}")
    values = values.contiguous()
    b = values.shape[0]
    per_elem = values[0].numel()
    m8 = None if mask is None else mask.expand_as(values).contiguous().to(torch.uint8)
    qs = np.ascontiguousarray(np.asarray(qs, dtype=np.float64).reshape(-1))
    m = int(qs.shape[0])
    dev = values.device
    vals = torch.empty((b, 2 * m), dtype=torch.float32, device=dev)
    weights = torch.empty((b, m), dtype=torch.float64, device=dev)
    count = torch.empty(b, dtype=torch.float64, device=dev)
    has_nan = torch.empty(b, dtype=torch.uint8, device=dev)
    ws_bytes = _native.lib().tio_quantiles_batched_workspace_bytes(b, m)
    ws = torch.empty(ws_bytes, dtype=torch.uint8, device=dev)
    with torch.cuda.device(dev):
        _native.call("tio_quantiles_batched", _ptr(values), RESOLUTION_DTYPE_CODES[values.dtype], _ptr(m8), b,
                     per_elem, qs.ctypes.data, m, _ptr(vals), _ptr(weights), _ptr(count), _ptr(has_nan), _ptr(ws),
                     ws_bytes, _stream(values))
    _count(2 + 5 * ((m + 12) // 13))
    return vals, weights, count, has_nan


def histogram_tables(values: Tensor, weights: Tensor, has_nan: Tensor, landmarks: Tensor) -> Tensor:
    b, m = weights.shape
    landmarks = landmarks.to(device=values.device, dtype=torch.float32).contiguous()
    tables = torch.empty((b, 3 * (m - 1)), dtype=torch.float32, device=values.device)
    with torch.cuda.device(values.device):
        _native.call("tio_histogram_tables", _ptr(values), _ptr(weights), _ptr(has_nan), _ptr(landmarks), b, m,
                     _ptr(tables), _stream(values))
    _count(1)
    return tables


def histogram_map(data: Tensor, tables: Tensor, m: int) -> None:
    _require_cuda(data, "histogram_map")
    if data.dtype not in RESOLUTION_DTYPE_CODES:
        raise TypeError(f"histogram_map: unsupported dtype {data.dtype}")
    if not data.is_contiguous():
        raise ValueError("histogram_map: data must be contiguous")
    if data.numel() == 0:
        return
    with torch.cuda.device(data.device):
        _native.call("tio_histogram_map", _ptr(data), _ptr(data), RESOLUTION_DTYPE_CODES[data.dtype], data.shape[0],
                     data[0].numel(), _ptr(tables), int(m), _stream(data))
    _count(1)


def rescale(src: Tensor, *, lo: float | None = None, hi: float | None = None, sub=None, div=None, mul=None,
            add=None, keep=None) -> Tensor:
    _require_cuda(src, "rescale")
    src = src.contiguous()
    b = src.shape[0]
    flags = (1 if lo is not None else 0)
    tabs = []
    for bit, table in ((2, sub), (4, div), (8, mul), (16, add)):
        if table is None:
            tabs.append(None)
            continue
        flags |= bit
        arr = np.asarray(table, dtype=np.float32).reshape(-1)
        tabs.append(np.ascontiguousarray(np.broadcast_to(arr, (b,)) if arr.size == 1 else arr))
    keep_np = None if keep is None else np.ascontiguousarray(np.asarray(keep, dtype=np.uint8))
    sub_d, div_d, mul_d, add_d, keep_d = upload(src.device, *tabs, keep_np)
    dst = torch.empty_like(src)
    with torch.cuda.device(src.device):
        _native.call("tio_rescale", _ptr(src), _ptr(dst), b, src[0].numel(),
                     float(lo if lo is not None else 0.0), float(hi if hi is not None else 0.0),
                     _ptr(sub_d), _ptr(div_d), _ptr(mul_d), _ptr(add_d), _ptr(keep_d), flags, _stream(src))
    _count(2)
    return dst


def intensity_fused(
    src: Tensor, *, coarse: Tensor | None = None, bias_identity: Tensor | None = None,
    bias_divide: bool = False, taps: Tensor | None = None, radius: Tensor | None = None,
    big_r: int = 0, axes_mask: int = 0, mean: Tensor | None = None, std: Tensor | None = None,
    keep: Tensor | None = None, z: Tensor | None = None, z2: Tensor | None = None,
    philox_seed: int = 0, noise_mode: int = 0, rician: bool = False,
    gamma: Tensor | None = None,
) -> Tensor:
    _require_cuda(src, "intensity_fused")
    src = src.contiguous()
    b, c, i, j, k = src.shape
    dst = torch.empty_like(src)
    jk = taps is not None and ((axes_mask & 6) or (axes_mask & 7 and big_r > WIDE_R))
    scratch = torch.empty_like(src) if jk else None
    si = sj = sk = 0
    if coarse is not None:
        si, sj, sk = coarse.shape[2:]
    with torch.cuda.device(src.device):
        _native.call(
            "tio_intensity_fused", _ptr(src), _ptr(dst), _ptr(scratch), b, c, i, j, k,
            _ptr(coarse), si, sj, sk, _ptr(bias_identity), int(bool(bias_divide)),
            _ptr(taps), _ptr(radius), int(big_r), int(axes_mask),
            _ptr(mean), _ptr(std), _ptr(keep), _ptr(z), _ptr(z2),
            int(philox_seed) & (2**64 - 1), int(noise_mode), int(bool(rician)),
            _ptr(gamma), _stream(src),
        )
    _count(_fused_launches(axes_mask if taps is not None else 0, coarse is not None, big_r))
    return dst



_MT_TABLE_FILE = _native.LIB_PATH.parent / "mt19937_jump.bin"
_mt_host_table: Tensor | None = None
_mt_device_tables: dict = {}
_mt_lock = threading.Lock()
MT_MAX_WORDS = 1 << 31
MT_TABLE_HEADER = (0x4D544A31, 21, 16, 64, 78, 10496)


def mt19937_host_table() -> Tensor:
    global _mt_host_table
    with _mt_lock:
        if _mt_host_table is None:
            lib = _native.lib()
            nbytes = lib.tio_mt19937_table_bytes()
            blob = None
            if _MT_TABLE_FILE.exists() and _MT_TABLE_FILE.stat().st_size == nbytes:
                cached = np.fromfile(_MT_TABLE_FILE, dtype=np.uint8)
                if tuple(int(v) for v in cached[:24].view(np.uint32)) == MT_TABLE_HEADER:
                    blob = torch.from_numpy(cached)
            if blob is None:
                blob = torch.zeros(nbytes, dtype=torch.uint8)
                _native.call("tio_mt19937_build_table", blob.data_ptr(), nbytes)
                try:
                    blob.numpy().tofile(_MT_TABLE_FILE)
                except OSError:
                    pass
            _mt_host_table = blob
        return _mt_host_table


def _mt_table(device: torch.device) -> Tensor:
    key = (device.type, device.index)
    table = _mt_device_tables.get(key)
    if table is None:
        with _init_lock:
            table = _mt_device_tables.get(key)
            if table is None:
                table = mt19937_host_table().to(device)
                torch.cuda.synchronize(device)
                _mt_device_tables[key] = table
    return table


def randn_mt19937(seed: int, offset: int, n: int, device, out: Tensor | None = None) -> Tensor:
    device = torch.device(device)
    if n < 16 or n % 16 or offset % 16 or offset + n > MT_MAX_WORDS:
        raise ValueError("randn_mt19937: offset and n must be multiples of 16, n >= 16,"
                         " offset + n <= 2**31")
    z = torch.empty(n, dtype=torch.float32, device=device) if out is None else out
    lib = _native.lib()
    ws_bytes = lib.tio_randn_mt19937_workspace_bytes(offset, n)
    workspace = torch.empty(ws_bytes, dtype=torch.uint8, device=device)
    table = _mt_table(device)
    with torch.cuda.device(device):
        _native.call("tio_randn_mt19937", int(seed) & 0xFFFFFFFF, offset, n, _ptr(z), _ptr(table),
                     _ptr(workspace), ws_bytes, torch.cuda.current_stream(device).cuda_stream)
    _count(4)
    return z



_cuda_rng_lock = threading.Lock()


def labels_to_image(labels: Tensor, label_values, means, stds, draw=None) -> Tensor:
    if labels.dtype not in DTYPE_CODES:
        raise TypeError(f"labels_to_image: unsupported label dtype {labels.dtype}")
    if labels.ndim != 5:
        raise ValueError(f"labels_to_image expects (B, C, I, J, K), got {tuple(labels.shape)}")
    b, c = int(labels.shape[0]), int(labels.shape[1])
    vox = int(np.prod(labels.shape[2:]))
    numel = b * vox
    tables.check_randn_numel(numel)
    _require_cuda(labels, "labels_to_image")
    if torch.cuda.is_current_stream_capturing():
        raise RuntimeError("labels_to_image: CUDA-graph capture is not supported (the generator offsets are"
                           " reserved on the host)")
    values = np.ascontiguousarray(np.asarray(label_values, dtype=np.int64).reshape(-1))
    n = int(values.shape[0])
    if n and np.any(np.diff(values) <= 0):
        raise ValueError("labels_to_image: label_values must be strictly ascending")
    mean = np.array(np.broadcast_to(np.asarray(means, dtype=np.float32).reshape(-1, n), (b, n)))
    std = np.array(np.broadcast_to(np.asarray(stds, dtype=np.float32).reshape(-1, n), (b, n)))
    if draw is None:
        active = np.any(mean != 0, axis=0) | np.any(std != 0, axis=0)
        draw = np.where(active, np.cumsum(active) - 1, -1)
    draw = np.asarray(draw, dtype=np.int64).reshape(n)
    n_draws = int((draw >= 0).sum())
    out = torch.empty((b, 1, *labels.shape[2:]), dtype=torch.float32, device=labels.device)
    if numel == 0:
        return out
    device = labels.device
    props = torch.cuda.get_device_properties(device)
    grid_x, counter_offset = tables.randn_cuda_layout(numel, props.multi_processor_count,
                                                      props.max_threads_per_multi_processor)
    gen = torch.cuda.default_generators[device.index]
    with _cuda_rng_lock:
        seed = int(gen.initial_seed())
        base = int(gen.get_offset())
        if n_draws:
            gen.set_offset(base + n_draws * counter_offset)
    offsets = np.where(draw >= 0, base + draw * counter_offset, -1).astype(np.int64)
    labels = labels.contiguous()
    values_d, mean_d, std_d, offsets_d = upload(device, values, mean, std, offsets) if n else (None,) * 4
    with torch.cuda.device(device):
        _native.call("tio_labels_to_image", _ptr(labels), DTYPE_CODES[labels.dtype], c, b, vox, _ptr(values_d), n,
                     _ptr(mean_d), _ptr(std_d), _ptr(offsets_d), seed & (2**64 - 1), grid_x, _ptr(out),
                     _stream(labels))
    _count(2 if n else 1)
    return out




def _label_map(src: Tensor, name: str) -> Tensor:
    _require_cuda(src, name)
    if src.dtype not in DTYPE_CODES:
        raise TypeError(f"{name}: unsupported label dtype {src.dtype}")
    if src.ndim != 5:
        raise ValueError(f"{name} expects (B, C, I, J, K), got {tuple(src.shape)}")
    return src.contiguous()


def label_lut(src: Tensor, keys: np.ndarray, values: np.ndarray, *, identity: bool) -> Tensor:
    src = _label_map(src, "label_lut")
    dst = torch.empty_like(src)
    n = int(keys.shape[0])
    keys_d, values_d = upload(src.device, keys, values) if n else (None, None)
    with torch.cuda.device(src.device):
        _native.call("tio_label_lut", _ptr(src), _ptr(dst), DTYPE_CODES[src.dtype], src.numel(), _ptr(keys_d),
                     _ptr(values_d), n, int(bool(identity)), _stream(src))
    _count(2 if n else 1)
    return dst


def label_contour(src: Tensor) -> Tensor:
    src = _label_map(src, "label_contour")
    dst = torch.empty(src.shape, dtype=torch.float32, device=src.device)
    if src.numel():
        b, c, i, j, k = src.shape
        with torch.cuda.device(src.device):
            _native.call("tio_label_contour", _ptr(src), DTYPE_CODES[src.dtype], b * c, i, j, k, _ptr(dst),
                         _stream(src))
        _count(1)
    return dst


def label_range(src: Tensor) -> tuple[int, int]:
    src = _label_map(src, "label_range")
    b, c = src.shape[:2]
    out = torch.empty(2, dtype=torch.int64, device=src.device)
    with torch.cuda.device(src.device):
        _native.call("tio_label_range", _ptr(src), DTYPE_CODES[src.dtype], b, c, src[0, 0].numel(), _ptr(out),
                     _stream(src))
    _count(2)
    lo, hi = out.tolist()
    return lo, hi


def onehot_classes(src: Tensor, num_classes: int) -> Tensor:
    src = _label_map(src, "onehot_classes")
    b, c = src.shape[:2]
    dst = torch.empty((b, num_classes, *src.shape[2:]), dtype=torch.float32, device=src.device)
    with torch.cuda.device(src.device):
        _native.call("tio_onehot_classes", _ptr(src), DTYPE_CODES[src.dtype], b, c, src[0, 0].numel(),
                     int(num_classes), _ptr(dst), _stream(src))
    _count(1)
    return dst


def channel_argmax(src: Tensor) -> Tensor:
    src = _label_map(src, "channel_argmax")
    b, c = src.shape[:2]
    dst = torch.empty((b, 1, *src.shape[2:]), dtype=torch.float32, device=src.device)
    with torch.cuda.device(src.device):
        _native.call("tio_channel_argmax", _ptr(src), DTYPE_CODES[src.dtype], b, c, src[0, 0].numel(), _ptr(dst),
                     _stream(src))
    _count(1)
    return dst



RESOLUTION_DTYPE_CODES = {**DTYPE_CODES, torch.float16: 6, torch.bfloat16: 7, torch.float64: 8}


def _volume_batch(src: Tensor, name: str) -> Tensor:
    _require_cuda(src, name)
    if src.dtype not in RESOLUTION_DTYPE_CODES:
        raise TypeError(f"{name}: unsupported dtype {src.dtype}")
    if src.ndim != 5:
        raise ValueError(f"{name} expects (B, C, I, J, K), got {tuple(src.shape)}")
    return src.contiguous()


def interpolate(src: Tensor, out_shape, idx: np.ndarray, lam: np.ndarray | None) -> Tensor:
    src = _volume_batch(src, "interpolate")
    b, c, i, j, k = src.shape
    oi, oj, ok = (int(s) for s in out_shape)
    dst = torch.empty((b, c, oi, oj, ok), dtype=src.dtype, device=src.device)
    if src.numel() and dst.numel():
        idx_d, lam_d = upload(src.device, idx, lam)
        with torch.cuda.device(src.device):
            _native.call("tio_interpolate", _ptr(src), _ptr(dst), RESOLUTION_DTYPE_CODES[src.dtype], b * c, i, j, k, oi, oj,
                         ok, _ptr(idx_d), _ptr(lam_d), int(lam is not None), _stream(src))
        _count(1)
    return dst


def axis_resample(src: Tensor, axis: np.ndarray, lo: np.ndarray, hi: np.ndarray, w: np.ndarray, *,
                  linear: bool) -> Tensor:
    src = _volume_batch(src, "axis_resample")
    b, c, i, j, k = src.shape
    dst = torch.empty_like(src)
    if src.numel():
        if linear:
            axis_d, lo_d, hi_d, w_d = upload(src.device, axis, lo, hi, w)
        else:
            (axis_d, lo_d), hi_d, w_d = upload(src.device, axis, lo), None, None
        with torch.cuda.device(src.device):
            _native.call("tio_axis_resample", _ptr(src), _ptr(dst), RESOLUTION_DTYPE_CODES[src.dtype], b, c, i, j, k,
                         _ptr(axis_d), _ptr(lo_d), _ptr(hi_d), _ptr(w_d), int(lo.shape[1]), int(bool(linear)),
                         _stream(src))
        _count(1)
    return dst




def _scalar_bytes(value: Tensor | None):
    if value is None:
        return None, None
    raw = value.reshape(1).contiguous().view(torch.uint8).numpy()
    return raw, raw.ctypes.data


def clamp(src: Tensor, lo: Tensor | None, hi: Tensor | None) -> Tensor:
    _require_cuda(src, "clamp")
    if src.dtype not in RESOLUTION_DTYPE_CODES:
        raise TypeError(f"clamp: unsupported dtype {src.dtype}")
    bound = lo if lo is not None else hi
    if bound is None:
        raise ValueError("clamp: no bound")
    src = src.contiguous()
    dst = torch.empty(src.shape, dtype=bound.dtype, device=src.device)
    (lo_keep, lo_ptr), (hi_keep, hi_ptr) = _scalar_bytes(lo), _scalar_bytes(hi)
    with torch.cuda.device(src.device):
        _native.call("tio_clamp", _ptr(src), _ptr(dst), RESOLUTION_DTYPE_CODES[src.dtype],
                     RESOLUTION_DTYPE_CODES[dst.dtype], src.numel(), lo_ptr, hi_ptr, _stream(src))
    _count(1)
    del lo_keep, hi_keep
    return dst


def mask(data: Tensor, mask: Tensor, keys: np.ndarray | None, outside: Tensor) -> Tensor:
    _require_cuda(data, "mask")
    _require_cuda(mask, "mask")
    if data.dtype not in RESOLUTION_DTYPE_CODES:
        raise TypeError(f"mask: unsupported dtype {data.dtype}")
    if mask.dtype == torch.bool:
        mask = mask.view(torch.uint8)
    if mask.dtype not in DTYPE_CODES:
        raise TypeError(f"mask: unsupported mask dtype {mask.dtype}")
    if data.ndim != 5 or mask.ndim != 4 or mask.shape[0] not in (1, data.shape[1]) or mask.shape[1:] != data.shape[2:]:
        raise ValueError(f"mask: a {tuple(mask.shape)} mask for a {tuple(data.shape)} batch")
    if not data.is_contiguous():
        raise ValueError("mask: data must be contiguous")
    mask = mask.contiguous()
    b, c = data.shape[:2]
    promote = outside.dtype != data.dtype
    dst = torch.empty(data.shape, dtype=outside.dtype, device=data.device) if promote else data
    n = -1 if keys is None else int(keys.shape[0])
    (keys_d,) = upload(data.device, keys) if n > 0 else (None,)
    keep, outside_ptr = _scalar_bytes(outside)
    if data.numel():
        with torch.cuda.device(data.device):
            _native.call("tio_mask", _ptr(mask), DTYPE_CODES[mask.dtype], mask.shape[0], _ptr(keys_d), n,
                         _ptr(data), RESOLUTION_DTYPE_CODES[data.dtype], _ptr(dst), RESOLUTION_DTYPE_CODES[dst.dtype],
                         b, c, data[0, 0].numel(), outside_ptr, _stream(data))
        _count(2 if n > 0 else 1)
    del keep
    return dst


SWAP_EXCHANGE, SWAP_STAGED, SWAP_NOOP = 0, 1, 2


def swap_patches(data: Tensor, swaps: np.ndarray, patch_size) -> None:
    _require_cuda(data, "swap_patches")
    if data.ndim != 5 or not data.is_contiguous():
        raise ValueError(f"swap_patches expects a contiguous (B, C, I, J, K) batch, got {tuple(data.shape)}")
    swaps = np.ascontiguousarray(swaps, dtype=np.int32)
    lists, steps = swaps.shape[:2]
    if steps == 0 or data.numel() == 0:
        return
    b, c, i, j, k = data.shape
    pi, pj, pk = (int(p) for p in patch_size)
    device_list = torch.empty(swaps.size, dtype=torch.int32, device=data.device)
    stage = None
    if bool((swaps[..., 6] == SWAP_STAGED).any()):
        stage = torch.empty(b * 2 * c * pi * pj * pk * data.element_size(), dtype=torch.uint8, device=data.device)
    with torch.cuda.device(data.device):
        _native.call("tio_swap_patches", _ptr(data), data.element_size(), b, c, i, j, k, pi, pj, pk,
                     swaps.ctypes.data, lists, steps, _ptr(device_list), _ptr(stage), _stream(data))
    _count(2)



KEEP_KEYS, KEEP_VALUE, KEEP_SEARCH = 0, 1, 2
KEEP_PRESENT, KEEP_NAN, KEEP_INF = 1, 2, 4


def _background_key(background_label, dtype: torch.dtype) -> tuple[int, int]:
    if isinstance(background_label, float) and not background_label.is_integer():
        return 0, 0
    key = int(background_label)
    if not -2**63 <= key < 2**63:
        return 0, 0
    if dtype == torch.float32 and int(np.float32(key)) != key:
        return 0, 0
    return key, 1


def keep_largest(data: Tensor, labels, background_label, fully_connected: bool) -> tuple[Tensor, Tensor]:
    if data.ndim != 5:
        raise ValueError(f"keep_largest expects (B, 1, I, J, K), got {tuple(data.shape)}")
    b, c, i, j, k = (int(s) for s in data.shape)
    if c != 1:
        raise ValueError(f"keep_largest expects single-channel label maps, got {c} channels")
    vox = i * j * k
    if vox >= 2**32:
        raise ValueError(f"keep_largest: {vox} voxels per element; component roots are 32-bit (at most 2**32 - 1)")
    if b > 65535:
        raise ValueError(f"keep_largest: {b} elements, at most 65535")
    data = _label_map(data, "keep_largest")
    dtype, dev = data.dtype, data.device
    fill, fill_error = None, None
    try:
        _, fill = tables.label_lut([(0, background_label)], dtype, dev)
    except (RuntimeError, ValueError, OverflowError, TypeError) as exc:
        fill_error = exc
    key, has_key = _background_key(background_label, dtype)
    if labels is not None:
        mode = KEEP_KEYS
        keys, _ = tables.label_lut([(label, 0) for label in labels], dtype, dev)
        n = int(keys.shape[0])
        (keys_d,) = upload(dev, keys) if n else (None,)
    else:
        mode = KEEP_VALUE if data.element_size() <= 2 else KEEP_SEARCH
        keys_d, n = None, 0
    roots = torch.empty((b, i, j, k), dtype=torch.int32, device=dev)
    count = torch.empty_like(roots)
    flags = torch.empty(b, dtype=torch.int32, device=dev)
    code = DTYPE_CODES[dtype]
    with torch.cuda.device(dev):
        _native.call("tio_components", _ptr(data), code, b, i, j, k, mode, _ptr(keys_d), n, key, has_key,
                     int(bool(fully_connected)), _ptr(roots), _ptr(count), _ptr(flags), _stream(data))
        _count(3)
        if mode == KEEP_SEARCH and b * vox:
            values = torch.empty(b * vox, dtype=dtype, device=dev)
            n_values = torch.empty(1, dtype=torch.int32, device=dev)
            _native.call("tio_component_roots", _ptr(data), code, b, vox, _ptr(roots), _ptr(values),
                         _ptr(n_values), _stream(data))
            _count(1)
            found = values[:int(n_values.item())]
            keys_d = torch.unique(found).to(torch.float32 if dtype == torch.float32 else torch.int64).contiguous()
            n = int(keys_d.numel())
            del values
    if (labels is None and dtype == torch.float32) or fill_error is not None:
        for bits in flags.tolist():
            if labels is None and bits & KEEP_INF:
                raise OverflowError("cannot convert float infinity to integer")
            if labels is None and bits & KEEP_NAN:
                raise ValueError("cannot convert float NaN to integer")
            if fill_error is not None and bits & KEEP_PRESENT:
                raise fill_error
    if fill_error is not None or not b * vox or (mode != KEEP_VALUE and n == 0):
        return data, roots
    slots = n if mode != KEEP_VALUE else (65536 if data.element_size() == 2 else 256)
    winner = torch.empty(b * slots, dtype=torch.int64, device=dev)
    keep, fill_ptr = _scalar_bytes(torch.from_numpy(np.ascontiguousarray(fill[:1])))
    with torch.cuda.device(dev):
        _native.call("tio_keep_largest", _ptr(data), code, b, vox, mode, _ptr(keys_d), n, key, has_key, _ptr(roots),
                     _ptr(count), _ptr(winner), fill_ptr, _stream(data))
    _count(2)
    del keep
    return data, roots



SPIKE_MAX_AXIS = 4096
SPECTRUM_WORKSPACE_BYTES = 512 << 20


def spike(data: Tensor, spikes: np.ndarray, intensity: np.ndarray) -> Tensor:
    _require_cuda(data, "spike")
    if data.dtype not in RESOLUTION_DTYPE_CODES:
        raise TypeError(f"spike: unsupported dtype {data.dtype}")
    if data.ndim != 5 or not data.is_contiguous():
        raise ValueError(f"spike expects a contiguous (B, C, I, J, K) batch, got {tuple(data.shape)}")
    b, c, i, j, k = (int(s) for s in data.shape)
    if max(i, j, k) > SPIKE_MAX_AXIS:
        raise NotImplementedError(
            f"Spike: spatial shape {(i, j, k)} has an axis longer than {SPIKE_MAX_AXIS} points, the"
            f" longest the spectrum peak supports")
    spikes = np.ascontiguousarray(spikes, dtype=np.int32)
    intensity = np.ascontiguousarray(intensity, dtype=np.float32)
    if spikes.ndim != 3 or spikes.shape[0] != b or spikes.shape[2] != 4 or intensity.shape != (b,):
        raise ValueError(f"spike: tables {spikes.shape} / {intensity.shape} for a batch of {b}")
    if data.numel() == 0 or spikes.shape[1] == 0:
        return data
    s = int(spikes.shape[1])
    spikes_d, intensity_d = upload(data.device, spikes, intensity)
    total, flags = spike_stats(data, intensity_d)
    peak = spectrum_peak(data, intensity_d, flags)
    tables_bytes = b * s * (i + j + k) * 8
    tables = torch.empty(tables_bytes, dtype=torch.uint8, device=data.device)
    with torch.cuda.device(data.device):
        _native.call("tio_spike", _ptr(data), RESOLUTION_DTYPE_CODES[data.dtype], b, c, i, j, k, _ptr(spikes_d), s,
                     _ptr(intensity_d), _ptr(total), _ptr(flags), _ptr(peak), _ptr(tables), tables_bytes,
                     _stream(data))
    _count(2)
    return data


def spike_stats(data: Tensor, intensity: Tensor) -> tuple[Tensor, Tensor]:
    b, c = int(data.shape[0]), int(data.shape[1])
    total = torch.empty(b * c, dtype=torch.float64, device=data.device)
    flags = torch.empty(b * c, dtype=torch.int32, device=data.device)
    ws_bytes = _native.lib().tio_spike_stats_workspace_bytes(b * c)
    ws = torch.empty(ws_bytes, dtype=torch.uint8, device=data.device)
    with torch.cuda.device(data.device):
        _native.call("tio_spike_stats", _ptr(data), RESOLUTION_DTYPE_CODES[data.dtype], b, c, data[0, 0].numel(),
                     _ptr(intensity), _ptr(total), _ptr(flags), _ptr(ws), ws_bytes, _stream(data))
    _count(2)
    return total, flags


def spectrum_peak(data: Tensor, intensity: Tensor, flags: Tensor, workspace_bytes: int | None = None) -> Tensor:
    b, c, i, j, k = (int(s) for s in data.shape)
    row_bytes = i * j * (k // 2 + 1) * 8
    if workspace_bytes is None:
        workspace_bytes = min(b * c, max(1, SPECTRUM_WORKSPACE_BYTES // row_bytes)) * row_bytes
    peak = torch.empty(b * c, dtype=torch.float32, device=data.device)
    ws = torch.empty(workspace_bytes, dtype=torch.uint8, device=data.device)
    with torch.cuda.device(data.device):
        _native.call("tio_spectrum_peak", _ptr(data), RESOLUTION_DTYPE_CODES[data.dtype], b, c, i, j, k,
                     _ptr(intensity), _ptr(flags), _ptr(peak), _ptr(ws), workspace_bytes, _stream(data))
    _count(1 + 3 * -(-(b * c) // (workspace_bytes // row_bytes)))
    return peak



GHOSTING_MAX_AXIS = 4096


def ghosting(data: Tensor, table: np.ndarray, axis: np.ndarray, active: np.ndarray) -> Tensor:
    _require_cuda(data, "ghosting")
    if data.dtype not in RESOLUTION_DTYPE_CODES:
        raise TypeError(f"ghosting: unsupported dtype {data.dtype}")
    if data.ndim != 5 or not data.is_contiguous():
        raise ValueError(f"ghosting expects a contiguous (B, C, I, J, K) batch, got {tuple(data.shape)}")
    b, c, i, j, k = (int(s) for s in data.shape)
    table = np.ascontiguousarray(table, dtype=np.float32)
    axis = np.ascontiguousarray(axis, dtype=np.int32)
    active = np.ascontiguousarray(active, dtype=np.uint8)
    if table.ndim != 2 or table.shape[0] != b or axis.shape != (b,) or active.shape != (b,):
        raise ValueError(f"ghosting: tables {table.shape} / {axis.shape} / {active.shape} for a batch of {b}")
    ghosted = sorted({int(a) for a, on in zip(axis, active, strict=True) if on})
    if not ghosted or data.numel() == 0:
        return data
    if ghosted[0] < 0 or ghosted[-1] > 2:
        raise ValueError(f"ghosting: axis {ghosted[0] if ghosted[0] < 0 else ghosted[-1]} outside 0..2")
    longest = max(data.shape[2 + a] for a in ghosted)
    if longest > GHOSTING_MAX_AXIS:
        raise NotImplementedError(
            f"Ghosting: spatial shape {(i, j, k)} is ghosted along an axis longer than {GHOSTING_MAX_AXIS} points,"
            f" the longest the line FFT supports")
    if table.shape[1] < longest:
        raise ValueError(f"ghosting: table rows of {table.shape[1]} entries for an axis of {longest} points")
    table_d, axis_d, active_d = upload(data.device, table, axis, active)
    flags = torch.empty(b * c, dtype=torch.int32, device=data.device)
    with torch.cuda.device(data.device):
        _native.call("tio_ghosting", _ptr(data), RESOLUTION_DTYPE_CODES[data.dtype], b, c, i, j, k, _ptr(table_d),
                     int(table.shape[1]), _ptr(axis_d), _ptr(active_d), sum(1 << a for a in ghosted), _ptr(flags),
                     _stream(data))
    _count(2 + len(ghosted))
    return data
```

### torchio_b200/transforms/intensity.py

```python

from __future__ import annotations

import os
import warnings
from typing import Any

import numpy as np
import torch
from torch import Tensor

from .. import ops, tables
from ..data import ImagesBatch, LabelMap, ScalarImage, SubjectsBatch
from ..params import to_nonneg_range, to_range
from .base import IntensityTransform, Transform, chunk_info, staged_derived


def _as_f32(data: Tensor) -> Tensor:
    return data if data.dtype == torch.float32 else data.float()




class BiasField(IntensityTransform):
    def __init__(self, *, std=0.5, scale: float = 0.025, **kwargs: Any) -> None:
        super().__init__(**kwargs)
        self.std = to_nonneg_range(std)
        if scale <= 0 or scale > 1:
            raise ValueError(f"scale must be in (0, 1], got {scale}")
        self.scale = scale

    @property
    def supports_per_instance_params(self) -> bool:
        return True

    @property
    def supports_per_instance_p(self) -> bool:
        return True

    def supports_chunks(self, batch: SubjectsBatch) -> bool:
        return True

    def make_params(self, batch: SubjectsBatch) -> dict[str, Any]:
        n = self._resolve_n(batch)
        if n is None:
            std = self.std.sample_1d()
            seed = int(torch.randint(0, 2**31, (1,)).item())
            return {"std": std, "seed": seed, "scale": self.scale}
        keep = self._keep_mask(batch, n)
        std = self._mask_identity(self.std.sample_1d(n), keep, identity=0.0)
        seeds = [int(torch.randint(0, 2**31, (1,)).item()) for _ in range(n)]
        params = {"std": self._serialize_param(std), "seed": seeds, "scale": self.scale}
        self._tag_batched(params, batch, n, keep, ["std", "seed"])
        return params

    def apply_transform(self, batch: SubjectsBatch, params: dict[str, Any]) -> SubjectsBatch:
        _apply_bias(self, batch, params["std"], params["seed"], params["scale"], divide=False)
        return batch

    @property
    def invertible(self) -> bool:
        return True

    def inverse(self, params: dict[str, Any]) -> _BiasFieldInverse:
        return _BiasFieldInverse(std=params["std"], seed=params["seed"], scale=params["scale"],
                                 copy=False)


def _bias_stage(data_shape, affines, std, seed, scale, *, divide: bool):
    per_element = isinstance(std, list)
    if (not per_element and std == 0) or (per_element and all(s == 0 for s in std)):
        return None
    b = data_shape[0]
    if per_element and len(std) != b:
        raise RuntimeError(
            f"Per-instance parameters were recorded for {len(std)} elements"
            f" but the batch has {b}"
        )
    info = chunk_info()
    if info is not None and not per_element:
        full = tables.coarse_bias_fields((info.total, *data_shape[1:]), std, seed, scale)
        coarse = full[info.b0:info.b1].contiguous()
    else:
        coarse = tables.coarse_bias_fields(data_shape, std, seed, scale)
    return {
        "coarse": coarse,
        "bias_identity": np.asarray([s == 0 for s in std], dtype=np.uint8) if per_element else None,
        "bias_divide": divide,
    }


def _apply_bias(transform, batch, std, seed, scale, *, divide: bool) -> None:
    run_stages(transform._get_images(batch),
               [lambda ib, index: _bias_stage(ib.data.shape, ib.affines, std, seed, scale,
                                              divide=divide)])


class _BiasFieldInverse(IntensityTransform):
    def __init__(self, *, std, seed, scale: float, **kwargs: Any) -> None:
        super().__init__(**kwargs)
        self._std, self._seed, self._scale = std, seed, scale

    def apply_transform(self, batch: SubjectsBatch, params: dict[str, Any]) -> SubjectsBatch:
        _apply_bias(self, batch, self._std, self._seed, self._scale, divide=True)
        return batch




class Blur(IntensityTransform):
    def __init__(self, *, std=0.0, **kwargs: Any) -> None:
        super().__init__(**kwargs)
        self.std = to_nonneg_range(std)
        self._warn_if_noop(is_noop=self.std.is_constant(0.0), hint="std=(0, 2)")

    @property
    def supports_per_instance_params(self) -> bool:
        return True

    @property
    def supports_per_instance_p(self) -> bool:
        return True

    def supports_chunks(self, batch: SubjectsBatch) -> bool:
        return True

    def make_params(self, batch: SubjectsBatch) -> dict[str, Any]:
        n = self._resolve_n(batch)
        if n is None:
            return {"std": self.std.sample()}
        keep = self._keep_mask(batch, n)
        std = self.std.sample(n)
        if keep is not None:
            std[~keep] = 0.0
        params = {"std": self._serialize_param(std)}
        self._tag_batched(params, batch, n, keep, ["std"])
        return params

    def apply_transform(self, batch: SubjectsBatch, params: dict[str, Any]) -> SubjectsBatch:
        run_stages(self._get_images(batch), [lambda ib, index: _blur_stage(ib, params, index)])
        return batch

    def prepare_stream(self, batch: SubjectsBatch, params: dict[str, Any], cache: dict, step: int) -> None:
        for index, ib in enumerate(self._get_images(batch).values()):
            cache[("blur", step, index)] = {"tables": _blur_stage(ib, params, index, whole=True)}


def _blur_stage(ib, params, index: int = 0, whole: bool = False):
    info = None if whole else chunk_info()
    if info is not None:
        cached = info.cache.get(("blur", info.step, index))
        if cached is not None:
            full = cached["tables"]
            if full is None:
                return None
            return {"taps": full["taps"][:, info.b0:info.b1].contiguous(),
                    "radius": full["radius"][:, info.b0:info.b1].contiguous(),
                    "big_r": full["big_r"], "axes_mask": full["axes_mask"]}
    if "_batched_keys" in params:
        mm = np.asarray(params["std"], dtype=np.float64)
        sp = np.asarray([a.spacing for a in ib.affines], dtype=np.float64)
        vox = np.divide(mm, sp, out=np.zeros_like(mm), where=sp > 0)
    else:
        sp = np.asarray(ib.affines[0].spacing, dtype=np.float64)
        vox = [s / q if q > 0 else 0.0 for s, q in zip(params["std"], sp, strict=True)]
    t = tables.blur_tables(vox, ib.data.shape[0])
    if t is None:
        return None
    return {"taps": t.taps, "radius": t.radius, "big_r": t.big_r, "axes_mask": t.axes_mask}




def _noise_mode() -> str:
    mode = os.environ.get("TIO_B200_NOISE", "exact").lower()
    if mode not in ("exact", "philox"):
        raise ValueError(f"TIO_B200_NOISE must be 'exact' or 'philox', got {mode!r}")
    return mode


class Noise(IntensityTransform):
    def __init__(self, *, mean=0.0, std=0.25, rician: bool = False, **kwargs: Any) -> None:
        super().__init__(**kwargs)
        self.mean = to_range(mean)
        self.std = to_nonneg_range(std)
        self.rician = rician

    @property
    def supports_per_instance_params(self) -> bool:
        return True

    @property
    def supports_per_instance_p(self) -> bool:
        return True

    def supports_chunks(self, batch: SubjectsBatch) -> bool:
        if _noise_mode() != "exact":
            return False
        images = self._get_images(batch).values()
        words = sum(int(np.prod(ib.data.shape)) for ib in images) * (2 if self.rician else 1)
        if words > ops.MT_MAX_WORDS:
            return False
        return all(int(np.prod(ib.data.shape[1:])) % 16 == 0 for ib in images)

    def make_params(self, batch: SubjectsBatch) -> dict[str, Any]:
        seed = int(torch.randint(0, 2**31, (1,)).item())
        n = self._resolve_n(batch)
        keep = self._keep_mask(batch, n)
        mean = self._mask_identity(self.mean.sample_1d(n), keep, identity=0.0)
        std = self._mask_identity(self.std.sample_1d(n), keep, identity=0.0)
        params = {
            "mean": self._serialize_param(mean), "std": self._serialize_param(std),
            "seed": seed, "rician": self.rician,
        }
        self._tag_batched(params, batch, n, keep, ["mean", "std"])
        return params

    def apply_transform(self, batch: SubjectsBatch, params: dict[str, Any]) -> SubjectsBatch:
        run_stages(self._get_images(batch), [_noise_stage_factory(params)])
        return batch


def _noise_stage_factory(params):
    mode = _noise_mode()
    generator = torch.Generator(device="cpu")
    generator.manual_seed(params["seed"])
    rician = bool(params.get("rician", False))
    keep = params.get("_keep")

    consumed = [0]

    def draw(shape, device):
        n = int(np.prod(shape))
        info = chunk_info()
        if info is None:
            start, n_full = consumed[0], n
        else:
            per = n // shape[0]
            start, n_full = consumed[0] + per * info.b0, per * info.total
        on_device = (not ragged[0] and n >= 16 and n % 16 == 0 and start % 16 == 0
                     and n_full % 16 == 0 and start + n <= ops.MT_MAX_WORDS
                     and device.type == "cuda")
        if info is not None and not on_device:
            raise RuntimeError("Noise: this batch cannot be streamed in slices (ragged normal stream)")
        if n_full < 16 or n_full % 16:
            ragged[0] = True
        consumed[0] += n_full + (16 if (n_full >= 16 and n_full % 16) else 0)
        if on_device:
            return ops.randn_mt19937(params["seed"], start, n, device).view(shape), None
        if host_state[0] != start:
            skip = start - host_state[0]
            if skip % 16 == 0 and skip >= 16:
                torch.randn(skip, generator=generator)
            else:
                raise RuntimeError("Noise: cannot realign the host generator (ragged stream)")
        pin = torch.cuda.is_available()
        z = torch.empty(shape, dtype=torch.float32, pin_memory=pin)
        torch.randn(shape, generator=generator, out=z)
        host_state[0] = consumed[0]
        return None, z

    host_state = [0]
    ragged = [False]

    def stage(ib, index):
        shape = ib.data.shape
        b = shape[0]
        out = {
            "mean": tables.per_element_vector(params["mean"], b),
            "std": tables.per_element_vector(params["std"], b),
            "keep": None if keep is None else np.asarray(keep, dtype=np.uint8),
            "rician": rician,
        }
        if mode == "philox":
            out["noise_mode"] = 2
            out["philox_seed"] = (int(params["seed"]) << 8) | (index & 0xFF)
            return out
        out["noise_mode"] = 1
        z_dev, z_host = draw(shape, ib.data.device)
        out["z" if z_dev is not None else "z_host"] = z_dev if z_dev is not None else z_host
        if rician:
            z_dev, z_host = draw(shape, ib.data.device)
            out["z2" if z_dev is not None else "z2_host"] = z_dev if z_dev is not None else z_host
        return out

    return stage




class Gamma(IntensityTransform):
    def __init__(self, *, log_gamma=0.0, **kwargs: Any) -> None:
        super().__init__(**kwargs)
        self.log_gamma = to_range(log_gamma)
        self._warn_if_noop(is_noop=self.log_gamma.is_constant(0.0), hint="log_gamma=(-0.3, 0.3)")

    @property
    def supports_per_instance_params(self) -> bool:
        return True

    @property
    def supports_per_instance_p(self) -> bool:
        return True

    def supports_chunks(self, batch: SubjectsBatch) -> bool:
        return True

    def make_params(self, batch: SubjectsBatch) -> dict[str, Any]:
        n = self._resolve_n(batch)
        keep = self._keep_mask(batch, n)
        log_gamma = self._mask_identity(self.log_gamma.sample_1d(n), keep, identity=0.0)
        params = {"log_gamma": self._serialize_param(log_gamma)}
        self._tag_batched(params, batch, n, keep, ["log_gamma"])
        return params

    def apply_transform(self, batch: SubjectsBatch, params: dict[str, Any]) -> SubjectsBatch:
        _apply_gamma(self, batch, params["log_gamma"])
        return batch

    @property
    def invertible(self) -> bool:
        return True

    def inverse(self, params: dict[str, Any]) -> _GammaInverse:
        return _GammaInverse(log_gamma=params["log_gamma"], copy=False)


def _apply_gamma(transform, batch, log_gamma) -> None:
    run_stages(transform._get_images(batch),
               [lambda ib, index: {"gamma": tables.gamma_values(log_gamma, ib.data.shape[0])}])


class _GammaInverse(IntensityTransform):
    def __init__(self, *, log_gamma, **kwargs: Any) -> None:
        super().__init__(**kwargs)
        self._log_gamma = log_gamma

    def apply_transform(self, batch: SubjectsBatch, params: dict[str, Any]) -> SubjectsBatch:
        lg = self._log_gamma
        _apply_gamma(self, batch, [-v for v in lg] if isinstance(lg, list) else -lg)
        return batch




class LabelsToImage(Transform):

    def __init__(self, label_key: str | None = None, *, image_key: str = "image_from_labels", mean=None,
                 std=None, default_mean=(0.1, 0.9), default_std=(0.01, 0.1), ignore_background: bool = False,
                 **kwargs: Any) -> None:
        super().__init__(**kwargs)
        self.label_key = label_key
        self.image_key = image_key
        self.mean_ranges = [to_range(m) for m in mean] if mean is not None else None
        self.std_ranges = [to_range(s) for s in std] if std is not None else None
        self.default_mean = to_range(default_mean)
        self.default_std = to_range(default_std)
        self.ignore_background = ignore_background

    @property
    def supports_per_instance_params(self) -> bool:
        return True

    def make_params(self, batch: SubjectsBatch) -> dict[str, Any]:
        _, label_batch = self._find_label_batch(batch)
        unique = sorted(int(v) for v in label_batch.data[0].unique().tolist())
        n = self._resolve_n(batch)
        if n is None:
            means, stds = self._sample_label_values(unique)
            return {"means": means, "stds": stds}
        means_list, stds_list = [], []
        for _ in range(n):
            means, stds = self._sample_label_values(unique)
            means_list.append(means)
            stds_list.append(stds)
        params = {"means": means_list, "stds": stds_list}
        self._tag_batched(params, batch, n, None, ["means", "stds"])
        return params

    def _sample_label_values(self, unique: list[int]) -> tuple[dict[int, float], dict[int, float]]:
        means: dict[int, float] = {}
        stds: dict[int, float] = {}
        for idx, label in enumerate(unique):
            if self.ignore_background and label == 0:
                means[label] = 0.0
                stds[label] = 0.0
                continue
            if self.mean_ranges is not None and idx < len(self.mean_ranges):
                means[label] = self.mean_ranges[idx].sample_1d()
            else:
                means[label] = self.default_mean.sample_1d()
            if self.std_ranges is not None and idx < len(self.std_ranges):
                stds[label] = self.std_ranges[idx].sample_1d()
            else:
                stds[label] = abs(self.default_std.sample_1d())
        return means, stds

    def apply_transform(self, batch: SubjectsBatch, params: dict[str, Any]) -> SubjectsBatch:
        name, label_batch = self._find_label_batch(batch)
        data = label_batch.data
        if not data.is_cuda:
            from .base import execution_device

            data = data.to(execution_device())
        values, draw, mean, std = tables.label_synthesis_tables(params["means"], params["stds"], data.shape[0])
        generated = ops.labels_to_image(data, values, mean, std, draw)
        batch.images[self.image_key] = ImagesBatch(generated, label_batch.affines, image_class=ScalarImage)
        staged_derived(self.image_key, name)
        return batch

    def _find_label_batch(self, batch: SubjectsBatch):
        if self.label_key is not None:
            if self.label_key not in batch.images:
                raise KeyError(f"Label key '{self.label_key}' not found. Available: {list(batch.images.keys())}")
            return self.label_key, batch.images[self.label_key]
        for name, img_batch in batch.images.items():
            if issubclass(img_batch._image_class, LabelMap):
                return name, img_batch
        raise KeyError("No LabelMap found in the subject")




def _resolve_mask(masking_method, img_batch, batch) -> Tensor | None:
    if masking_method is None:
        return None
    if callable(masking_method) and not isinstance(masking_method, str):
        return masking_method(img_batch.data[0]).bool()
    if isinstance(masking_method, str):
        return label_map_element0(masking_method, batch).bool()
    raise TypeError(f"masking_method must be None, str, or callable, got {type(masking_method)}")


def label_map_element0(key: str, batch) -> Tensor:
    if key not in batch.images:
        raise KeyError(f'Masking method "{key}" not found in batch images.'
                       f" Available: {list(batch.images.keys())}")
    mask_batch = batch.images[key]
    from ..data import LabelMap

    if not issubclass(mask_batch._image_class, LabelMap):
        raise TypeError(f'Masking method "{key}" must refer to a LabelMap.')
    return mask_batch.data[0]


def _sample0(img_batch, mask, warn_empty: str) -> tuple[Tensor, Tensor | None]:
    tensor = _as_f32(img_batch.data[0]).contiguous()
    if mask is not None:
        mask = mask.to(tensor.device).expand_as(tensor)
        if not bool(mask.any()):
            warnings.warn(warn_empty, RuntimeWarning, stacklevel=4)
            mask = None
    return tensor, mask


class Standardize(IntensityTransform):

    def __init__(self, *, masking_method=None, **kwargs: Any) -> None:
        super().__init__(**kwargs)
        self.masking_method = masking_method

    def make_params(self, batch: SubjectsBatch) -> dict[str, Any]:
        stats: dict[str, tuple[float, float]] = {}
        for name, img_batch in self._get_images(batch).items():
            mask = _resolve_mask(self.masking_method, img_batch, batch)
            with _Staged(img_batch) as staged:
                tensor, mask = _sample0(staged, mask, f'Mask is empty for "{name}". Using all voxels.')
                s, ss, n = ops.moments(tensor, mask)
            mean = s / n
            var = (ss - s * s / n) / (n - 1) if n > 1 else float("nan")
            stats[name] = (float(np.float32(mean)), float(np.float32(np.sqrt(max(var, 0.0)))))
        return {"stats": stats}

    def apply_transform(self, batch: SubjectsBatch, params: dict[str, Any]) -> SubjectsBatch:
        stats = params["stats"]
        for name, img_batch in self._get_images(batch).items():
            if name not in stats:
                continue
            mean, std = stats[name]
            if std == 0:
                raise RuntimeError(f'Standard deviation is zero for masked values in "{name}".'
                                   " Cannot standardize.")
            img_batch.data = ops.rescale(_as_f32(img_batch.data), sub=mean, div=std)
        return batch

    @property
    def invertible(self) -> bool:
        return True

    def inverse(self, params: dict[str, Any]) -> _StandardizeInverse:
        return _StandardizeInverse(stats=params["stats"], copy=False)


class _StandardizeInverse(IntensityTransform):
    def __init__(self, *, stats, **kwargs: Any) -> None:
        super().__init__(**kwargs)
        self._stats = stats

    def make_params(self, batch: SubjectsBatch) -> dict[str, Any]:
        return {}

    def apply_transform(self, batch: SubjectsBatch, params: dict[str, Any]) -> SubjectsBatch:
        for name, img_batch in self._get_images(batch).items():
            if name not in self._stats:
                continue
            mean, std = self._stats[name]
            if std == 0:
                continue
            img_batch.data = ops.rescale(_as_f32(img_batch.data), mul=std, add=mean)
        return batch


def _lerp_f32(a: float, b: float, weight: float) -> float:
    a32, b32, w32 = np.float32(a), np.float32(b), np.float32(weight)
    diff = np.float32(b32 - a32)
    if w32 < np.float32(0.5):
        return float(np.float32(a32 + np.float32(w32 * diff)))
    return float(np.float32(b32 - np.float32(diff * np.float32(np.float32(1.0) - w32))))


class Normalize(IntensityTransform):

    def __init__(self, *, out_min=-1.0, out_max=1.0, in_min=None, in_max=None, percentile_low=0.0,
                 percentile_high=100.0, masking_method=None, **kwargs: Any) -> None:
        super().__init__(**kwargs)
        self.out_min = _value_range(out_min)
        self.out_max = _value_range(out_max)
        self.in_min = _value_range(in_min) if in_min is not None else None
        self.in_max = _value_range(in_max) if in_max is not None else None
        self.percentile_low = _value_range(percentile_low)
        self.percentile_high = _value_range(percentile_high)
        self.masking_method = masking_method

    @property
    def supports_per_instance_params(self) -> bool:
        return True

    def make_params(self, batch: SubjectsBatch) -> dict[str, Any]:
        n = self._resolve_n(batch)
        out_min = self.out_min.sample_1d(n)
        out_max = self.out_max.sample_1d(n)
        pct_low = self.percentile_low.sample_1d()
        pct_high = self.percentile_high.sample_1d()
        params: dict[str, Any] = {"out_min": self._serialize_param(out_min),
                                  "out_max": self._serialize_param(out_max)}
        if self.in_min is not None and self.in_max is not None:
            params["in_min"] = self.in_min.sample_1d()
            params["in_max"] = self.in_max.sample_1d()
        else:
            in_ranges: dict[str, tuple[float, float]] = {}
            for name, img_batch in self._get_images(batch).items():
                mask = _resolve_mask(self.masking_method, img_batch, batch)
                with _Staged(img_batch) as staged:
                    tensor, mask = _sample0(staged, mask, f'Cannot compute percentiles for "{name}": mask is'
                                                          " empty. Using full range.")
                    values, weights, _ = ops.quantile_neighbours(tensor, [pct_low / 100.0, pct_high / 100.0], mask)
                low = values[0] if weights[0] == 0 else _lerp_f32(values[0], values[1], weights[0])
                high = values[2] if weights[1] == 0 else _lerp_f32(values[2], values[3], weights[1])
                in_ranges[name] = (low, high)
            params["in_ranges"] = in_ranges
        if n is not None:
            self._tag_batched(params, batch, n, None, ["out_min", "out_max"])
        return params

    def apply_transform(self, batch: SubjectsBatch, params: dict[str, Any]) -> SubjectsBatch:
        for name, img_batch in self._get_images(batch).items():
            if "in_min" in params:
                in_min, in_max = params["in_min"], params["in_max"]
            else:
                in_ranges = params.get("in_ranges", {})
                if name not in in_ranges:
                    continue
                in_min, in_max = in_ranges[name]
            in_range = in_max - in_min
            if in_range == 0:
                warnings.warn(f'Cannot rescale "{name}": input range is zero.', RuntimeWarning, stacklevel=2)
                continue
            out_min, out_range = _out_min_and_range(params["out_min"], params["out_max"])
            img_batch.data = ops.rescale(_as_f32(img_batch.data), lo=in_min, hi=in_max, sub=in_min, div=in_range,
                                         mul=out_range, add=out_min)
        return batch

    @property
    def invertible(self) -> bool:
        return True

    def inverse(self, params: dict[str, Any]) -> _RescaleInverse:
        return _RescaleInverse(out_min=params["out_min"], out_max=params["out_max"], in_min=params.get("in_min"),
                               in_max=params.get("in_max"), in_ranges=params.get("in_ranges"), copy=False)


RescaleIntensity = Normalize
ZNormalization = Standardize


def _value_range(value):
    if isinstance(value, (int, float)):
        return to_range(float(value))
    if isinstance(value, (tuple, list)):
        return to_range(tuple(float(v) for v in value))
    return to_range(value)


def _out_min_and_range(out_min, out_max):
    if isinstance(out_min, list):
        lo = np.asarray(out_min, dtype=np.float32)
        return lo, (np.asarray(out_max, dtype=np.float32) - lo).astype(np.float32)
    return out_min, out_max - out_min


class _RescaleInverse(IntensityTransform):
    def __init__(self, *, out_min, out_max, in_min, in_max, in_ranges, **kwargs: Any) -> None:
        super().__init__(**kwargs)
        self._out_min, self._out_max = out_min, out_max
        self._in_min, self._in_max, self._in_ranges = in_min, in_max, in_ranges

    def make_params(self, batch: SubjectsBatch) -> dict[str, Any]:
        return {}

    def apply_transform(self, batch: SubjectsBatch, params: dict[str, Any]) -> SubjectsBatch:
        for name, img_batch in self._get_images(batch).items():
            if self._in_min is not None and self._in_max is not None:
                in_min, in_max = self._in_min, self._in_max
            elif self._in_ranges is not None and name in self._in_ranges:
                in_min, in_max = self._in_ranges[name]
            else:
                continue
            in_range = in_max - in_min
            if in_range == 0:
                continue
            out_min, out_range = _out_min_and_range(self._out_min, self._out_max)
            keep = None
            if isinstance(out_range, float):
                if out_range == 0:
                    continue
            else:
                keep = (out_range != 0).astype(np.uint8)
                out_range = np.where(out_range == 0, np.float32(1.0), out_range)
            data = _as_f32(img_batch.data)
            img_batch.data = ops.rescale(data, sub=out_min, div=out_range, mul=in_range, add=in_min, keep=keep)
        return batch


class _Staged:

    def __init__(self, img_batch) -> None:
        self.img_batch = img_batch

    def __enter__(self):
        data = self.img_batch.data
        if data.is_cuda:
            return self.img_batch
        from .base import execution_device

        class _View:
            pass

        view = _View()
        view.data = data[:1].to(execution_device(), non_blocking=True)
        return view

    def __exit__(self, *exc) -> None:
        return None



_TABLE_KEYS = ("coarse", "bias_identity", "taps", "radius", "mean", "std", "keep", "gamma")


def run_stages(images, stage_builders) -> None:
    for index, ib in enumerate(images.values()):
        kwargs: dict[str, Any] = {}
        for build in stage_builders:
            stage = build(ib, index)
            if stage:
                kwargs.update(stage)
        if not kwargs:
            continue
        data = ib.data
        device = data.device
        uploaded = ops.upload(device, *[kwargs.get(k) for k in _TABLE_KEYS])
        for key, value in zip(_TABLE_KEYS, uploaded, strict=True):
            if key in kwargs:
                kwargs[key] = value
        z_host, z2_host = kwargs.pop("z_host", None), kwargs.pop("z2_host", None)
        if z_host is not None:
            kwargs["z"] = z_host.to(device, non_blocking=True)
        if z2_host is not None:
            kwargs["z2"] = z2_host.to(device, non_blocking=True)
        out = ops.intensity_fused(_as_f32(data), **kwargs)
        promotes = ("gamma" in kwargs or "mean" in kwargs) and data.dtype != torch.float64
        ib.data = out if promotes or out.dtype == data.dtype else out.to(data.dtype)
```

Measured before the change: 49.95 billion.

## Co-schedule MT19937 normal generation with first intensity pass via warp-specialized kernel

Adds a persistent kernel that runs the bias/I-blur march in 256 threads while the extra warps generate MT19937 normals concurrently, using named barriers and setmaxnreg to split registers between the two roles. The noise stage now defers normal generation (passing seed/offset as z_replay), and intensity_fused routes eligible cases through this combined pass before the J/K blur+noise pass. The goal is to hide the standalone RNG kernel's cost behind the memory-bound march. It also relaxes the scratch requirement when only J/K blur is needed. This adds complexity and contention for SM resources, and it relies on a dynamic tile counter.

```diff
diff --git a/include/tio_b200.h b/include/tio_b200.h
--- a/include/tio_b200.h
+++ b/include/tio_b200.h
@@ -100,6 +100,16 @@
                         uint64_t philox_seed, int noise_mode, int rician,
                         const float* gamma, void* stream);
 
+size_t tio_intensity_pass1_with_normals_workspace_bytes(uint64_t offset, uint64_t n);
+int tio_intensity_pass1_with_normals(const float* src, float* dst,
+                                     int B, int C, int I, int J, int K,
+                                     const float* coarse, int si, int sj, int sk,
+                                     const uint8_t* bias_identity, int bias_divide,
+                                     const float* taps, const int32_t* radius, int R, int axes_mask,
+                                     uint64_t seed, uint64_t offset, uint64_t n, float* z,
+                                     const void* table, void* workspace, size_t workspace_bytes,
+                                     void* stream);
+
 int tio_labels_to_image(const void* labels, int dtype, int C, int B, int64_t vox,
                         const int64_t* label_values, int n, const float* mean, const float* std,
                         const uint64_t* draw_offset, uint64_t seed, int grid_x, float* dst,
diff --git a/torchio_b200/_native.py b/torchio_b200/_native.py
--- a/torchio_b200/_native.py
+++ b/torchio_b200/_native.py
@@ -41,6 +41,11 @@
     + [c_void_p, c_int, c_int, c_int, c_void_p, c_int]
     + [c_void_p, c_void_p, c_int, c_int]
     + [c_void_p] * 5 + [c_uint64, c_int, c_int, c_void_p, c_void_p],
+    "tio_intensity_pass1_with_normals_workspace_bytes": [c_uint64, c_uint64],
+    "tio_intensity_pass1_with_normals": [c_void_p, c_void_p] + [c_int] * 5
+    + [c_void_p, c_int, c_int, c_int, c_void_p, c_int]
+    + [c_void_p, c_void_p, c_int, c_int]
+    + [c_uint64, c_uint64, c_uint64, c_void_p, c_void_p, c_void_p, c_size_t, c_void_p],
     "tio_labels_to_image": [c_void_p, c_int, c_int, c_int, c_int64, c_void_p, c_int, c_void_p, c_void_p, c_void_p,
                             c_uint64, c_int, c_void_p, c_void_p],
     "tio_label_lut": [c_void_p, c_void_p, c_int, c_int64, c_void_p, c_void_p, c_int, c_int, c_void_p],
diff --git a/torchio_b200/csrc/build.py b/torchio_b200/csrc/build.py
--- a/torchio_b200/csrc/build.py
+++ b/torchio_b200/csrc/build.py
@@ -14,7 +14,7 @@
            "label_maps.cu", "interpolate.cu", "clamp_mask_swap.cu", "components.cu", "permute.cu", "spike.cu",
            "ghosting.cu"]
 HEADERS = [HERE / "common.cuh", HERE / "resample_common.cuh", HERE / "resample_tile.cuh", HERE / "tma.cuh",
-           HERE / "mt19937_layout.h", HERE / "label_lookup.cuh", HERE / "image_dtype.cuh",
+           HERE / "mt19937_layout.h", HERE / "mt19937_normal.cuh", HERE / "label_lookup.cuh", HERE / "image_dtype.cuh",
            HERE / "fft_lines.cuh",
            ROOT / "include" / "tio_b200.h",
            Path(__file__).resolve()]
diff --git a/torchio_b200/csrc/fused_intensity.cu b/torchio_b200/csrc/fused_intensity.cu
--- a/torchio_b200/csrc/fused_intensity.cu
+++ b/torchio_b200/csrc/fused_intensity.cu
@@ -1,4 +1,6 @@
 #include "common.cuh"
+#include "mt19937_layout.h"
+#include "mt19937_normal.cuh"
 #include "tma.cuh"
 
 namespace tio {
@@ -639,17 +641,13 @@
 
 constexpr int M6_PF = 8;
 
-template <bool HAS_BIAS, bool EPI>
-__global__ void __launch_bounds__(256, EPI ? 1 : 2)
-march6_kernel(const float* __restrict__ src, float* __restrict__ dst, int B, int C, int I, int J,
-              int K, BlurArgs bl, BiasArgs bi, NoiseArgs nz, const float* __restrict__ gamma) {
-  extern __shared__ __align__(16) float smem[];
+template <bool HAS_BIAS, bool EPI, int BAR>
+__device__ __forceinline__ void march6_tile(float* smem, const int tid, const int k, const int j, const int bc,
+                                            const float* __restrict__ src, float* __restrict__ dst, int B,
+                                            int C, int I, int J, int K, const BlurArgs& bl, const BiasArgs& bi,
+                                            const NoiseArgs& nz, const float* __restrict__ gamma) {
   constexpr int W = 2 * F_R + 1;
-  const int bc = blockIdx.z;
   const int b = bc / C;
-  const int tid = threadIdx.y * blockDim.x + threadIdx.x;
-  const int k = (blockIdx.x * blockDim.x + threadIdx.x) * 4;
-  const int j = blockIdx.y * blockDim.y + threadIdx.y;
   const int64_t n = (int64_t)I * J * K;
   const float* x = src + (int64_t)bc * n;
   float* y = dst + (int64_t)bc * n;
@@ -667,7 +665,8 @@
     const float* gs = bi.coarse + (int64_t)bc * ns;
     for (int t = tid; t < ns; t += 256) g[t] = gs[t];
   }
-  __syncthreads();
+  if (BAR == 0) __syncthreads();
+  else asm volatile("bar.sync %0, 256;" ::"n"(BAR) : "memory");
   if (k >= K || j >= J) return;
 
   const bool noise_on = EPI && nz.mode != 0 && (!nz.keep || nz.keep[b]);
@@ -817,6 +816,56 @@
         }
         finish(o, acc);
       }
+    }
+  }
+}
+
+template <bool HAS_BIAS, bool EPI>
+__global__ void __launch_bounds__(256, EPI ? 1 : 2)
+march6_kernel(const float* __restrict__ src, float* __restrict__ dst, int B, int C, int I, int J,
+              int K, BlurArgs bl, BiasArgs bi, NoiseArgs nz, const float* __restrict__ gamma) {
+  extern __shared__ __align__(16) float smem[];
+  march6_tile<HAS_BIAS, EPI, 0>(smem, threadIdx.y * blockDim.x + threadIdx.x,
+                                (blockIdx.x * blockDim.x + threadIdx.x) * 4,
+                                blockIdx.y * blockDim.y + threadIdx.y, blockIdx.z, src, dst, B, C, I, J, K,
+                                bl, bi, nz, gamma);
+}
+
+constexpr int P1N_MARCH_THREADS = 256;
+constexpr int P1N_THREADS = P1N_MARCH_THREADS + 5 * 128;
+constexpr int P1N_BAR_SEGMENT = 6, P1N_BAR_MARCH = 7;
+constexpr int P1N_RING_FLOATS = MT_RING * MT_N + 4;
+
+template <bool HAS_BIAS>
+__global__ void __launch_bounds__(P1N_THREADS, 1)
+pass1_normals_kernel(const float* __restrict__ src, float* __restrict__ dst, int B, int C, int I, int J,
+                     int K, BlurArgs bl, BiasArgs bi, unsigned int* __restrict__ tile_counter,
+                     const uint32_t* __restrict__ states, int q_lo, int q_hi, unsigned long long L,
+                     unsigned long long offset, unsigned long long n, float* __restrict__ z) {
+  extern __shared__ __align__(16) float smem[];
+  if (threadIdx.x < P1N_MARCH_THREADS) {
+    asm volatile("setmaxnreg.inc.sync.aligned.u32 152;");
+    const int tid = threadIdx.x;
+    volatile int* next_tile = reinterpret_cast<int*>(smem + MT_RING * MT_N);
+    const int kb_n = (K + 255) / 256, jb_n = (J + 3) / 4;
+    const int tiles = kb_n * jb_n * B * C;
+    for (;;) {
+      if (tid == 0) *next_tile = (int)atomicAdd(tile_counter, 1u);
+      asm volatile("bar.sync %0, 256;" ::"n"(P1N_BAR_MARCH) : "memory");
+      const int tile = *next_tile;
+      if (tile >= tiles) break;
+      const int kb = tile % kb_n, jb = (tile / kb_n) % jb_n, bc = tile / (kb_n * jb_n);
+      march6_tile<HAS_BIAS, false, P1N_BAR_MARCH>(smem + P1N_RING_FLOATS, tid, (kb * 64 + (tid & 63)) * 4,
+                                                  jb * 4 + (tid >> 6), bc, src, dst, B, C, I, J, K, bl, bi,
+                                                  NoiseArgs{}, nullptr);
+    }
+  } else {
+    asm volatile("setmaxnreg.dec.sync.aligned.u32 40;");
+    const int tid = threadIdx.x - P1N_MARCH_THREADS;
+    if (tid >= MT_THREADS) return;
+    for (int q = q_lo + blockIdx.x; q < q_hi; q += gridDim.x) {
+      mt_normal_segment(reinterpret_cast<uint32_t*>(smem), tid, states, q, L, offset, n, z);
+      mt_bar_sync<P1N_BAR_SEGMENT, MT_THREADS>();
     }
   }
 }
@@ -993,11 +1042,12 @@
   if (axes_mask != 0 && bl.R > 16)
     return wide_impl(src, dst, scratch, B, C, I, J, K, bi, bl, axes_mask, nz, gamma, st, who);
   const bool need_jk = (axes_mask & 6) != 0;
-  TIO_CHECK_ARG(!need_jk || (scratch && src != dst && scratch != src && scratch != dst),
-                "%s: blur along J/K needs a scratch buffer and src != dst", who);
-  TIO_CHECK_ARG(!((axes_mask & 1) && src == dst && !need_jk), "%s: blur along I needs src != dst", who);
   const bool need_i = (axes_mask & 1) != 0;
   const bool need_march = !need_jk || need_i || bi.coarse != nullptr;
+  TIO_CHECK_ARG(!need_jk || src != dst, "%s: blur along J/K needs src != dst", who);
+  TIO_CHECK_ARG(!(need_jk && need_march) || (scratch && scratch != src && scratch != dst),
+                "%s: blur along J/K after bias or blur along I needs a scratch buffer", who);
+  TIO_CHECK_ARG(!((axes_mask & 1) && src == dst && !need_jk), "%s: blur along I needs src != dst", who);
   const float* cur = src;
   if (need_jk) {
     const int64_t tiles = (int64_t)B * C * ((I + A_PLANES - 1) / A_PLANES);
@@ -1087,3 +1137,59 @@
   return fused_impl(src, dst, scratch, B, C, I, J, K, bi, bl, taps ? (axes_mask & 7) : 0, nz,
                     gamma, (cudaStream_t)stream, "tio_intensity_fused");
 }
+
+extern "C" size_t tio_intensity_pass1_with_normals_workspace_bytes(uint64_t offset, uint64_t n) {
+  return tio_randn_mt19937_workspace_bytes(offset, n) + 16;
+}
+
+extern "C" int tio_intensity_pass1_with_normals(const float* src, float* dst, int B, int C, int I, int J,
+                                                int K, const float* coarse, int si, int sj, int sk,
+                                                const uint8_t* bias_identity, int bias_divide,
+                                                const float* taps, const int32_t* radius, int R,
+                                                int axes_mask, uint64_t seed, uint64_t offset, uint64_t n,
+                                                float* z, const void* table, void* workspace,
+                                                size_t workspace_bytes, void* stream) {
+  const char* who = "tio_intensity_pass1_with_normals";
+  TIO_CHECK_ARG(src && dst && z, "%s: null src/dst/z", who);
+  TIO_CHECK_ARG(src != dst, "%s: src and dst must not alias", who);
+  TIO_CHECK_ARG(B > 0 && C > 0 && I > 0 && J > 0 && K > 0, "%s: bad shape", who);
+  const bool need_i = taps && (axes_mask & 1);
+  TIO_CHECK_ARG(!need_i || (radius && R >= 0 && R <= F_R), "%s: needs a radius table and R <= %d, got R=%d", who,
+                F_R, R);
+  TIO_CHECK_ARG(K % 4 == 0 && aligned16f(src) && aligned16f(dst) && aligned16f(z),
+                "%s: needs K %% 4 == 0 and 16-byte aligned src, dst and z", who);
+  const int64_t tiles = (int64_t)((K + 255) / 256) * ((J + 3) / 4) * B * C;
+  TIO_CHECK_ARG(tiles < (1ll << 31) - (1 << 20), "%s: batch too large", who);
+  BiasArgs bi{};
+  bi.coarse = coarse; bi.identity = bias_identity; bi.si = si; bi.sj = sj; bi.sk = sk;
+  bi.divide = bias_divide;
+  if (coarse) {
+    bi.sc_i = up_scale(si, I); bi.sc_j = up_scale(sj, J); bi.sc_k = up_scale(sk, K);
+    TIO_CHECK_ARG(si > 0 && sj > 0 && sk > 0 && (size_t)si * sj * sk * 4 <= 64 * 1024,
+                  "%s: coarse bias grid empty or too large", who);
+  }
+  BlurArgs bl{need_i ? taps : nullptr, radius, R};
+  TIO_CHECK_ARG(workspace_bytes >= tio_intensity_pass1_with_normals_workspace_bytes(offset, n),
+                "%s: workspace too small", who);
+  cudaStream_t st = (cudaStream_t)stream;
+  int q_lo, q_hi;
+  const size_t states_bytes = tio_randn_mt19937_workspace_bytes(offset, n);
+  if (int rc = mt_start_states(seed, offset, n, table, workspace, states_bytes, st, who, &q_lo, &q_hi)) return rc;
+  unsigned int* tile_counter = reinterpret_cast<unsigned int*>((char*)workspace + states_bytes);
+  cudaMemsetAsync(tile_counter, 0, sizeof(unsigned int), st);
+  const int ns = coarse ? si * sj * sk : 0;
+  const size_t smem = (size_t)(P1N_RING_FLOATS + 16 + (ns + 3) / 4 * 4) * sizeof(float) + (size_t)M6_PF * 256 * 16;
+  const unsigned long long seg = 1ull << tio_mt::kLog2L;
+  const int grid = num_sms();
+#define TIO_LAUNCH_P1N(BB)                                                                                   \
+  do {                                                                                                       \
+    cudaFuncSetAttribute(pass1_normals_kernel<BB>, cudaFuncAttributeMaxDynamicSharedMemorySize, (int)smem);  \
+    pass1_normals_kernel<BB><<<grid, P1N_THREADS, smem, st>>>(src, dst, B, C, I, J, K, bl, bi, tile_counter, \
+                                                              (const uint32_t*)workspace, q_lo, q_hi, seg,   \
+                                                              offset, n, z);                                 \
+  } while (0)
+  if (coarse) TIO_LAUNCH_P1N(true); else TIO_LAUNCH_P1N(false);
+#undef TIO_LAUNCH_P1N
+  TIO_CHECK_LAUNCH();
+  return 0;
+}
diff --git a/torchio_b200/csrc/mt19937.cu b/torchio_b200/csrc/mt19937.cu
--- a/torchio_b200/csrc/mt19937.cu
+++ b/torchio_b200/csrc/mt19937.cu
@@ -1,24 +1,12 @@
 #include "common.cuh"
 #include "mt19937_layout.h"
+#include "mt19937_normal.cuh"
 
 namespace tio {
 
-constexpr int MT_N = 624, MT_M = 397, MT_DEG = 19937;
+constexpr int MT_DEG = 19937;
 constexpr int MT_SEQ = MT_DEG + MT_N;
 constexpr int MT_OFFS = (MT_SEQ + 7) / 4 * 4;
-
-__device__ __forceinline__ uint32_t mt_twist(uint32_t a, uint32_t b, uint32_t c) {
-  const uint32_t y = (a & 0x80000000u) | (b & 0x7fffffffu);
-  return c ^ (y >> 1) ^ ((y & 1u) ? 0x9908b0dfu : 0u);
-}
-
-__device__ __forceinline__ uint32_t mt_temper(uint32_t y) {
-  y ^= y >> 11;
-  y ^= (y << 7) & 0x9d2c5680u;
-  y ^= (y << 15) & 0xefc60000u;
-  y ^= y >> 18;
-  return y;
-}
 
 __global__ void mt_seed_kernel(uint32_t seed, uint32_t* __restrict__ states) {
   if (threadIdx.x == 0) {
@@ -88,155 +76,24 @@
   }
 }
 
-__device__ __forceinline__ void sincos_0_2pi(float theta, float& sn, float& cs) {
-  const float t = __fmaf_rn(theta, 0.6366197723675814f, 12582912.0f);
-  const int j = __float_as_int(t);
-  const float jf = __fsub_rn(t, 12582912.0f);
-  float r = __fmaf_rn(jf, -1.5707962512969971f, theta);
-  r = __fmaf_rn(jf, -7.549789415861596e-08f, r);
-  const float r2 = __fmul_rn(r, r);
-  float ps = __fmaf_rn(r2, -1.9515295891e-4f, 8.3321608736e-3f);
-  ps = __fmaf_rn(ps, r2, -1.6666654611e-1f);
-  const float s = __fmaf_rn(__fmul_rn(ps, r2), r, r);
-  float pc = __fmaf_rn(r2, 2.443315711809948e-5f, -1.388731625493765e-3f);
-  pc = __fmaf_rn(pc, r2, 4.166664568298827e-2f);
-  const float c = __fmaf_rn(__fmul_rn(pc, r2), r2, __fmaf_rn(r2, -0.5f, 1.0f));
-  const bool swap = j & 1;
-  const float a = swap ? c : s, b = swap ? s : c;
-  sn = (j & 2) ? -a : a;
-  cs = ((j + 1) & 2) ? -b : b;
-}
-
-__device__ __forceinline__ void mt_box_muller(uint32_t a, uint32_t b, float& zc, float& zs) {
-  const float u1 = (float)(mt_temper(a) & 0xffffffu) * (1.0f / 16777216.0f);
-  const float u2 = (float)(mt_temper(b) & 0xffffffu) * (1.0f / 16777216.0f);
-  float radius;
-  asm("sqrt.approx.ftz.f32 %0, %1;" : "=f"(radius) : "f"(-2.0f * logf(1.0f - u1)));
-  const float theta = (float)(6.283185307179586 * (double)u2);
-  float sn, cs;
-  sincos_0_2pi(theta, sn, cs);
-  zc = radius * cs;
-  zs = radius * sn;
-}
-
-template <int ID, int COUNT>
-__device__ __forceinline__ void mt_bar_sync() {
-  asm volatile("bar.sync %0, %1;" ::"n"(ID), "n"(COUNT) : "memory");
-}
-template <int ID, int COUNT>
-__device__ __forceinline__ void mt_bar_arrive() {
-  asm volatile("bar.arrive %0, %1;" ::"n"(ID), "n"(COUNT) : "memory");
-}
-
-constexpr int MT_ROUND = 4;
-constexpr int MT_RING = 2 * MT_ROUND;
-constexpr int MT_ITEMS = MT_ROUND * MT_N / 8;
-constexpr int MT_PRODUCERS = 256;
-constexpr int MT_CONSUMERS = (MT_ITEMS + 31) / 32 * 32;
-constexpr int MT_THREADS = MT_PRODUCERS + MT_CONSUMERS;
-constexpr int MT_BAR_PROD = 1, MT_BAR_FULL = 2, MT_BAR_EMPTY = 4;
-
 __global__ void __launch_bounds__(MT_THREADS, 2)
 mt_normal_kernel(const uint32_t* __restrict__ states, int q_first, unsigned long long L,
                  unsigned long long offset, unsigned long long n, float* __restrict__ z) {
   __shared__ __align__(16) uint32_t ring[MT_RING * MT_N];
-  const int tid = threadIdx.x;
-  const int q = q_first + blockIdx.x;
-  const unsigned long long seg_begin = (unsigned long long)q * L;
-  const unsigned long long lo = max(seg_begin, offset);
-  const unsigned long long hi = min(seg_begin + L, offset + n);
-  if (lo >= hi) return;
-  const int lo_rel = (int)(lo - seg_begin), hi_rel = (int)(hi - seg_begin);
-  const int rounds = ((hi_rel + MT_N - 1) / MT_N + MT_ROUND - 1) / MT_ROUND;
-  if (tid < MT_PRODUCERS) {
-    constexpr int W = MT_N - MT_M;
-    const uint32_t* w = states + (size_t)q * MT_N;
-    uint32_t* start = ring + (MT_RING - 1) * MT_N;
-    for (int t = tid; t < MT_N; t += MT_PRODUCERS) start[t] = w[t];
-    mt_bar_sync<MT_BAR_PROD, MT_PRODUCERS>();
-    for (int r = 0; r < rounds; ++r) {
-      if (r >= 2) {
-        if (r & 1) mt_bar_sync<MT_BAR_EMPTY + 1, MT_THREADS>();
-        else mt_bar_sync<MT_BAR_EMPTY, MT_THREADS>();
-      }
-      for (int i = 0; i < MT_ROUND; ++i) {
-        const int b = r * MT_ROUND + i;
-        const uint32_t* cur = ring + ((b + MT_RING - 1) % MT_RING) * MT_N;
-        uint32_t* nxt = ring + (b % MT_RING) * MT_N;
-        if (tid < W) nxt[tid] = mt_twist(cur[tid], cur[tid + 1], cur[tid + MT_M]);
-        mt_bar_sync<MT_BAR_PROD, MT_PRODUCERS>();
-        if (tid < W) nxt[W + tid] = mt_twist(cur[W + tid], cur[W + tid + 1], nxt[tid]);
-        mt_bar_sync<MT_BAR_PROD, MT_PRODUCERS>();
-        if (tid < MT_N - 2 * W) {
-          const int k = 2 * W + tid;
-          const uint32_t c = (k + 1 < MT_N) ? cur[k + 1] : nxt[0];
-          nxt[k] = mt_twist(cur[k], c, nxt[k - W]);
-        }
-        mt_bar_sync<MT_BAR_PROD, MT_PRODUCERS>();
-      }
-      if (r & 1) mt_bar_arrive<MT_BAR_FULL + 1, MT_THREADS>();
-      else mt_bar_arrive<MT_BAR_FULL, MT_THREADS>();
-    }
-  } else {
-    const int c = tid - MT_PRODUCERS;
-    const int blk = c / (MT_N / 8), item = c % (MT_N / 8);
-    const int word = 16 * (item >> 1) + 4 * (item & 1);
-    const long long seg_to_z = (long long)seg_begin - (long long)offset;
-    const bool vec = ((reinterpret_cast<uintptr_t>(z) & 15) == 0);
-    for (int r = 0; r < rounds; ++r) {
-      if (r & 1) mt_bar_sync<MT_BAR_FULL + 1, MT_THREADS>();
-      else mt_bar_sync<MT_BAR_FULL, MT_THREADS>();
-      const int b = r * MT_ROUND + blk;
-      const int group = b * MT_N + (word & ~15);
-      if (c < MT_ITEMS && group >= lo_rel && group < hi_rel) {
-        const uint32_t* x = ring + (b % MT_RING) * MT_N + word;
-        const uint4 a = *reinterpret_cast<const uint4*>(x);
-        const uint4 s = *reinterpret_cast<const uint4*>(x + 8);
-        float4 zc, zs;
-        mt_box_muller(a.x, s.x, zc.x, zs.x);
-        mt_box_muller(a.y, s.y, zc.y, zs.y);
-        mt_box_muller(a.z, s.z, zc.z, zs.z);
-        mt_box_muller(a.w, s.w, zc.w, zs.w);
-        float* zp = z + (seg_to_z + b * MT_N + word);
-        if (vec) {
-          *reinterpret_cast<float4*>(zp) = zc;
-          *reinterpret_cast<float4*>(zp + 8) = zs;
-        } else {
-          zp[0] = zc.x; zp[1] = zc.y; zp[2] = zc.z; zp[3] = zc.w;
-          zp[8] = zs.x; zp[9] = zs.y; zp[10] = zs.z; zp[11] = zs.w;
-        }
-      }
-      if (r + 2 < rounds) {
-        if (r & 1) mt_bar_arrive<MT_BAR_EMPTY + 1, MT_THREADS>();
-        else mt_bar_arrive<MT_BAR_EMPTY, MT_THREADS>();
-      }
-    }
-  }
+  mt_normal_segment(ring, (int)threadIdx.x, states, q_first + (int)blockIdx.x, L, offset, n, z);
 }
-
-}
-
-using namespace tio;
 
 constexpr uint64_t MT_L = 1ull << tio_mt::kLog2L;
 
-extern "C" size_t tio_randn_mt19937_workspace_bytes(uint64_t offset, uint64_t n) {
-  const uint64_t q_hi = (offset + n + MT_L - 1) / MT_L;
-  return (size_t)(q_hi + tio_mt::kS1) * MT_N * 4;
-}
-
-extern "C" int tio_randn_mt19937(uint64_t seed, uint64_t offset, uint64_t n, float* z,
-                                 const void* table, void* workspace, size_t workspace_bytes,
-                                 void* stream) {
-  TIO_CHECK_ARG(z && table && workspace, "tio_randn_mt19937: null pointer");
+int mt_start_states(uint64_t seed, uint64_t offset, uint64_t n, const void* table, void* workspace,
+                    size_t workspace_bytes, cudaStream_t st, const char* who, int* q_lo_out, int* q_hi_out) {
+  TIO_CHECK_ARG(table && workspace, "%s: null table or workspace", who);
   TIO_CHECK_ARG(n >= 16 && (n % 16) == 0 && (offset % 16) == 0,
-                "tio_randn_mt19937: n and offset must be multiples of 16 (n >= 16)");
+                "%s: n and offset must be multiples of 16 (n >= 16)", who);
   const int S2 = tio_mt::kS2, S1 = tio_mt::kS1, stride = tio_mt::kStride;
   const uint64_t q_lo = offset / MT_L, q_hi = (offset + n + MT_L - 1) / MT_L;
-  TIO_CHECK_ARG(q_hi <= (uint64_t)S1 * S2, "tio_randn_mt19937: stream position beyond %d segments", S1 * S2);
-  TIO_CHECK_ARG(workspace_bytes >= tio_randn_mt19937_workspace_bytes(offset, n),
-                "tio_randn_mt19937: workspace too small");
-  cudaStream_t st = (cudaStream_t)stream;
+  TIO_CHECK_ARG(q_hi <= (uint64_t)S1 * S2, "%s: stream position beyond %d segments", who, S1 * S2);
+  TIO_CHECK_ARG(workspace_bytes >= tio_randn_mt19937_workspace_bytes(offset, n), "%s: workspace too small", who);
   uint32_t* states = (uint32_t*)workspace;
   const uint16_t* polys = (const uint16_t*)((const char*)table + tio_mt::kHeaderBytes);
   mt_seed_kernel<<<1, 32, 0, st>>>((uint32_t)seed, states);
@@ -252,7 +109,31 @@
                                                                              S2, 0, kCoarseParts);
   }
   mt_jump_kernel<<<(unsigned)(q_hi - q_lo), 640, jump_smem, st>>>(states, polys, stride, (int)q_lo, S2, 1, 1);
-  mt_normal_kernel<<<(unsigned)(q_hi - q_lo), MT_THREADS, 0, st>>>(states, (int)q_lo, MT_L, offset, n, z);
+  *q_lo_out = (int)q_lo;
+  *q_hi_out = (int)q_hi;
+  return 0;
+}
+
+}
+
+using namespace tio;
+
+extern "C" size_t tio_randn_mt19937_workspace_bytes(uint64_t offset, uint64_t n) {
+  const uint64_t q_hi = (offset + n + MT_L - 1) / MT_L;
+  return (size_t)(q_hi + tio_mt::kS1) * MT_N * 4;
+}
+
+extern "C" int tio_randn_mt19937(uint64_t seed, uint64_t offset, uint64_t n, float* z,
+                                 const void* table, void* workspace, size_t workspace_bytes,
+                                 void* stream) {
+  TIO_CHECK_ARG(z, "tio_randn_mt19937: null pointer");
+  cudaStream_t st = (cudaStream_t)stream;
+  int q_lo, q_hi;
+  if (int rc = mt_start_states(seed, offset, n, table, workspace, workspace_bytes, st, "tio_randn_mt19937",
+                               &q_lo, &q_hi))
+    return rc;
+  mt_normal_kernel<<<(unsigned)(q_hi - q_lo), MT_THREADS, 0, st>>>((const uint32_t*)workspace, q_lo, MT_L, offset,
+                                                                   n, z);
   TIO_CHECK_LAUNCH();
   return 0;
 }
diff --git a/torchio_b200/csrc/mt19937_normal.cuh b/torchio_b200/csrc/mt19937_normal.cuh
--- /dev/null
+++ b/torchio_b200/csrc/mt19937_normal.cuh
@@ -0,0 +1,149 @@
+#pragma once
+
+#include "common.cuh"
+
+namespace tio {
+
+constexpr int MT_N = 624, MT_M = 397;
+
+__device__ __forceinline__ uint32_t mt_twist(uint32_t a, uint32_t b, uint32_t c) {
+  const uint32_t y = (a & 0x80000000u) | (b & 0x7fffffffu);
+  return c ^ (y >> 1) ^ ((y & 1u) ? 0x9908b0dfu : 0u);
+}
+
+__device__ __forceinline__ uint32_t mt_temper(uint32_t y) {
+  y ^= y >> 11;
+  y ^= (y << 7) & 0x9d2c5680u;
+  y ^= (y << 15) & 0xefc60000u;
+  y ^= y >> 18;
+  return y;
+}
+
+__device__ __forceinline__ void sincos_0_2pi(float theta, float& sn, float& cs) {
+  const float t = __fmaf_rn(theta, 0.6366197723675814f, 12582912.0f);
+  const int j = __float_as_int(t);
+  const float jf = __fsub_rn(t, 12582912.0f);
+  float r = __fmaf_rn(jf, -1.5707962512969971f, theta);
+  r = __fmaf_rn(jf, -7.549789415861596e-08f, r);
+  const float r2 = __fmul_rn(r, r);
+  float ps = __fmaf_rn(r2, -1.9515295891e-4f, 8.3321608736e-3f);
+  ps = __fmaf_rn(ps, r2, -1.6666654611e-1f);
+  const float s = __fmaf_rn(__fmul_rn(ps, r2), r, r);
+  float pc = __fmaf_rn(r2, 2.443315711809948e-5f, -1.388731625493765e-3f);
+  pc = __fmaf_rn(pc, r2, 4.166664568298827e-2f);
+  const float c = __fmaf_rn(__fmul_rn(pc, r2), r2, __fmaf_rn(r2, -0.5f, 1.0f));
+  const bool swap = j & 1;
+  const float a = swap ? c : s, b = swap ? s : c;
+  sn = (j & 2) ? -a : a;
+  cs = ((j + 1) & 2) ? -b : b;
+}
+
+__device__ __forceinline__ void mt_box_muller(uint32_t a, uint32_t b, float& zc, float& zs) {
+  const float u1 = (float)(mt_temper(a) & 0xffffffu) * (1.0f / 16777216.0f);
+  const float u2 = (float)(mt_temper(b) & 0xffffffu) * (1.0f / 16777216.0f);
+  float radius;
+  asm("sqrt.approx.ftz.f32 %0, %1;" : "=f"(radius) : "f"(-2.0f * logf(1.0f - u1)));
+  const float theta = (float)(6.283185307179586 * (double)u2);
+  float sn, cs;
+  sincos_0_2pi(theta, sn, cs);
+  zc = radius * cs;
+  zs = radius * sn;
+}
+
+template <int ID, int COUNT>
+__device__ __forceinline__ void mt_bar_sync() {
+  asm volatile("bar.sync %0, %1;" ::"n"(ID), "n"(COUNT) : "memory");
+}
+template <int ID, int COUNT>
+__device__ __forceinline__ void mt_bar_arrive() {
+  asm volatile("bar.arrive %0, %1;" ::"n"(ID), "n"(COUNT) : "memory");
+}
+
+constexpr int MT_ROUND = 4;
+constexpr int MT_RING = 2 * MT_ROUND;
+constexpr int MT_ITEMS = MT_ROUND * MT_N / 8;
+constexpr int MT_PRODUCERS = 256;
+constexpr int MT_CONSUMERS = (MT_ITEMS + 31) / 32 * 32;
+constexpr int MT_THREADS = MT_PRODUCERS + MT_CONSUMERS;
+constexpr int MT_BAR_PROD = 1, MT_BAR_FULL = 2, MT_BAR_EMPTY = 4;
+
+__device__ __forceinline__ void mt_normal_segment(uint32_t* __restrict__ ring, const int tid,
+                                                  const uint32_t* __restrict__ states, const int q,
+                                                  unsigned long long L, unsigned long long offset,
+                                                  unsigned long long n, float* __restrict__ z) {
+  const unsigned long long seg_begin = (unsigned long long)q * L;
+  const unsigned long long lo = max(seg_begin, offset);
+  const unsigned long long hi = min(seg_begin + L, offset + n);
+  if (lo >= hi) return;
+  const int lo_rel = (int)(lo - seg_begin), hi_rel = (int)(hi - seg_begin);
+  const int rounds = ((hi_rel + MT_N - 1) / MT_N + MT_ROUND - 1) / MT_ROUND;
+  if (tid < MT_PRODUCERS) {
+    constexpr int W = MT_N - MT_M;
+    const uint32_t* w = states + (size_t)q * MT_N;
+    uint32_t* start = ring + (MT_RING - 1) * MT_N;
+    for (int t = tid; t < MT_N; t += MT_PRODUCERS) start[t] = w[t];
+    mt_bar_sync<MT_BAR_PROD, MT_PRODUCERS>();
+    for (int r = 0; r < rounds; ++r) {
+      if (r >= 2) {
+        if (r & 1) mt_bar_sync<MT_BAR_EMPTY + 1, MT_THREADS>();
+        else mt_bar_sync<MT_BAR_EMPTY, MT_THREADS>();
+      }
+      for (int i = 0; i < MT_ROUND; ++i) {
+        const int b = r * MT_ROUND + i;
+        const uint32_t* cur = ring + ((b + MT_RING - 1) % MT_RING) * MT_N;
+        uint32_t* nxt = ring + (b % MT_RING) * MT_N;
+        if (tid < W) nxt[tid] = mt_twist(cur[tid], cur[tid + 1], cur[tid + MT_M]);
+        mt_bar_sync<MT_BAR_PROD, MT_PRODUCERS>();
+        if (tid < W) nxt[W + tid] = mt_twist(cur[W + tid], cur[W + tid + 1], nxt[tid]);
+        mt_bar_sync<MT_BAR_PROD, MT_PRODUCERS>();
+        if (tid < MT_N - 2 * W) {
+          const int k = 2 * W + tid;
+          const uint32_t c = (k + 1 < MT_N) ? cur[k + 1] : nxt[0];
+          nxt[k] = mt_twist(cur[k], c, nxt[k - W]);
+        }
+        mt_bar_sync<MT_BAR_PROD, MT_PRODUCERS>();
+      }
+      if (r & 1) mt_bar_arrive<MT_BAR_FULL + 1, MT_THREADS>();
+      else mt_bar_arrive<MT_BAR_FULL, MT_THREADS>();
+    }
+  } else {
+    const int c = tid - MT_PRODUCERS;
+    const int blk = c / (MT_N / 8), item = c % (MT_N / 8);
+    const int word = 16 * (item >> 1) + 4 * (item & 1);
+    const long long seg_to_z = (long long)seg_begin - (long long)offset;
+    const bool vec = ((reinterpret_cast<uintptr_t>(z) & 15) == 0);
+    for (int r = 0; r < rounds; ++r) {
+      if (r & 1) mt_bar_sync<MT_BAR_FULL + 1, MT_THREADS>();
+      else mt_bar_sync<MT_BAR_FULL, MT_THREADS>();
+      const int b = r * MT_ROUND + blk;
+      const int group = b * MT_N + (word & ~15);
+      if (c < MT_ITEMS && group >= lo_rel && group < hi_rel) {
+        const uint32_t* x = ring + (b % MT_RING) * MT_N + word;
+        const uint4 a = *reinterpret_cast<const uint4*>(x);
+        const uint4 s = *reinterpret_cast<const uint4*>(x + 8);
+        float4 zc, zs;
+        mt_box_muller(a.x, s.x, zc.x, zs.x);
+        mt_box_muller(a.y, s.y, zc.y, zs.y);
+        mt_box_muller(a.z, s.z, zc.z, zs.z);
+        mt_box_muller(a.w, s.w, zc.w, zs.w);
+        float* zp = z + (seg_to_z + b * MT_N + word);
+        if (vec) {
+          *reinterpret_cast<float4*>(zp) = zc;
+          *reinterpret_cast<float4*>(zp + 8) = zs;
+        } else {
+          zp[0] = zc.x; zp[1] = zc.y; zp[2] = zc.z; zp[3] = zc.w;
+          zp[8] = zs.x; zp[9] = zs.y; zp[10] = zs.z; zp[11] = zs.w;
+        }
+      }
+      if (r + 2 < rounds) {
+        if (r & 1) mt_bar_arrive<MT_BAR_EMPTY + 1, MT_THREADS>();
+        else mt_bar_arrive<MT_BAR_EMPTY, MT_THREADS>();
+      }
+    }
+  }
+}
+
+int mt_start_states(uint64_t seed, uint64_t offset, uint64_t n, const void* table, void* workspace,
+                    size_t workspace_bytes, cudaStream_t st, const char* who, int* q_lo, int* q_hi);
+
+}
diff --git a/torchio_b200/ops.py b/torchio_b200/ops.py
--- a/torchio_b200/ops.py
+++ b/torchio_b200/ops.py
@@ -447,14 +447,25 @@
     big_r: int = 0, axes_mask: int = 0, mean: Tensor | None = None, std: Tensor | None = None,
     keep: Tensor | None = None, z: Tensor | None = None, z2: Tensor | None = None,
     philox_seed: int = 0, noise_mode: int = 0, rician: bool = False,
-    gamma: Tensor | None = None,
+    gamma: Tensor | None = None, z_replay: tuple[int, int] | None = None,
 ) -> Tensor:
     _require_cuda(src, "intensity_fused")
     src = src.contiguous()
     b, c, i, j, k = src.shape
+    if z_replay is not None:
+        seed, offset = z_replay
+        blur_jk = taps is not None and bool(axes_mask & 6) and big_r <= 6
+        first_pass = coarse is not None or (taps is not None and bool(axes_mask & 1))
+        if (blur_jk and first_pass and noise_mode == 1 and not rician and k % 4 == 0
+                and src.data_ptr() % 16 == 0 and src.numel() % 16 == 0):
+            return _intensity_fused_pass1_normals(
+                src, coarse, bias_identity, bias_divide, taps, radius, big_r, axes_mask, mean, std,
+                keep, gamma, seed, offset)
+        z = randn_mt19937(seed, offset, src.numel(), src.device).view(src.shape)
     dst = torch.empty_like(src)
-    jk = taps is not None and ((axes_mask & 6) or (axes_mask & 7 and big_r > WIDE_R))
-    scratch = torch.empty_like(src) if jk else None
+    two_pass = taps is not None and axes_mask & 6 and (coarse is not None or axes_mask & 1)
+    wide = taps is not None and axes_mask & 7 and big_r > WIDE_R
+    scratch = torch.empty_like(src) if two_pass or wide else None
     si = sj = sk = 0
     if coarse is not None:
         si, sj, sk = coarse.shape[2:]
@@ -469,6 +480,47 @@
         )
     _count(_fused_launches(axes_mask if taps is not None else 0, coarse is not None, big_r))
     return dst
+
+
+def intensity_pass1_with_normals(
+    src: Tensor, seed: int, offset: int, *, coarse: Tensor | None = None,
+    bias_identity: Tensor | None = None, bias_divide: bool = False, taps: Tensor | None = None,
+    radius: Tensor | None = None, big_r: int = 0, axes_mask: int = 0,
+) -> tuple[Tensor, Tensor]:
+    _require_cuda(src, "intensity_pass1_with_normals")
+    src = src.contiguous()
+    b, c, i, j, k = src.shape
+    n = src.numel()
+    if n < 16 or n % 16 or offset % 16 or offset + n > MT_MAX_WORDS:
+        raise ValueError("intensity_pass1_with_normals: offset and numel must be multiples of 16,"
+                         " numel >= 16, offset + numel <= 2**31")
+    dst = torch.empty_like(src)
+    z = torch.empty_like(src)
+    ws_bytes = _native.lib().tio_intensity_pass1_with_normals_workspace_bytes(offset, n)
+    workspace = torch.empty(ws_bytes, dtype=torch.uint8, device=src.device)
+    table = _mt_table(src.device)
+    si = sj = sk = 0
+    if coarse is not None:
+        si, sj, sk = coarse.shape[2:]
+    with torch.cuda.device(src.device):
+        _native.call(
+            "tio_intensity_pass1_with_normals", _ptr(src), _ptr(dst), b, c, i, j, k,
+            _ptr(coarse), si, sj, sk, _ptr(bias_identity), int(bool(bias_divide)),
+            _ptr(taps), _ptr(radius), int(big_r), int(axes_mask),
+            int(seed) & 0xFFFFFFFF, offset, n, _ptr(z), _ptr(table), _ptr(workspace), ws_bytes,
+            _stream(src),
+        )
+    _count(4)
+    return dst, z
+
+
+def _intensity_fused_pass1_normals(src, coarse, bias_identity, bias_divide, taps, radius, big_r,
+                                   axes_mask, mean, std, keep, gamma, seed, offset) -> Tensor:
+    first, z = intensity_pass1_with_normals(
+        src, seed, offset, coarse=coarse, bias_identity=bias_identity, bias_divide=bias_divide,
+        taps=taps, radius=radius, big_r=big_r, axes_mask=axes_mask)
+    return intensity_fused(first, taps=taps, radius=radius, big_r=big_r, axes_mask=axes_mask & 6,
+                           mean=mean, std=std, keep=keep, z=z, noise_mode=1, gamma=gamma)
 
 
 
diff --git a/torchio_b200/transforms/intensity.py b/torchio_b200/transforms/intensity.py
--- a/torchio_b200/transforms/intensity.py
+++ b/torchio_b200/transforms/intensity.py
@@ -229,7 +229,7 @@
 
     consumed = [0]
 
-    def draw(shape, device):
+    def draw(shape, device, defer=False):
         n = int(np.prod(shape))
         info = chunk_info()
         if info is None:
@@ -246,6 +246,8 @@
             ragged[0] = True
         consumed[0] += n_full + (16 if (n_full >= 16 and n_full % 16) else 0)
         if on_device:
+            if defer:
+                return (params["seed"], start), None
             return ops.randn_mt19937(params["seed"], start, n, device).view(shape), None
         if host_state[0] != start:
             skip = start - host_state[0]
@@ -276,8 +278,11 @@
             out["philox_seed"] = (int(params["seed"]) << 8) | (index & 0xFF)
             return out
         out["noise_mode"] = 1
-        z_dev, z_host = draw(shape, ib.data.device)
-        out["z" if z_dev is not None else "z_host"] = z_dev if z_dev is not None else z_host
+        z_dev, z_host = draw(shape, ib.data.device, defer=not rician)
+        if z_host is not None:
+            out["z_host"] = z_host
+        else:
+            out["z" if rician else "z_replay"] = z_dev
         if rician:
             z_dev, z_host = draw(shape, ib.data.device)
             out["z2" if z_dev is not None else "z2_host"] = z_dev if z_dev is not None else z_host
```

New measurement: 52.05 billion, median of 6. +4.2%, better.
